# dnbaker/dashing

Measured on AMD Instinct MI355X. Metric: genome-pairs/sec, all-pairs HLL Jaccard (Ertl-MLE), N=10000 p=14, higher is better.
Workload: dtype u8/u32 popcount + f64 estimator; 1 GPU; BASELINE configs[2]: 10000 synthetic sketches, p=14 (16384 B each), all-pairs dist on MI355X; n_sketches=10000, p=14, k=31, estimator=ERTL_MLE

## Files before the change

### dashing_amd/csrc/abi.hip

```cpp
#include <algorithm>
#include <cstdlib>
#include <cstring>
#include <new>

#include "ctx.h"

using namespace dsh;

extern "C" {

const char *dsh_backend_name(void) { return "hip:gfx950"; }

int dsh_abi_version(void) { return DSH_ABI_VERSION; }

int dsh_device_count(void)
{
    int n = 0;
    if (hipGetDeviceCount(&n) != hipSuccess) return 0;
    return n;
}

static void release_ctx(dsh_ctx *c)
{
    (void)hipSetDevice(c->device);
// ... 787 lines not shown
{
    if (!c) return DSH_EINVAL;
    if (pair_ms) *pair_ms = c->pair_ms;
    if (fin_ms) *fin_ms = c->fin_ms;
    if (prep_ms) *prep_ms = c->prep_ms;
    if (launches) *launches = c->pair_launches;
    return DSH_OK;
}

int dsh_last_part_info(dsh_ctx *c, double *ready_ms, uint64_t *floats, uint32_t cap, uint32_t *nparts_out)
{
    if (!c || !nparts_out) return DSH_EINVAL;
    const uint32_t k = (uint32_t)c->part_ready_ms.size();
    *nparts_out = k;
    if (k > cap && (ready_ms || floats)) return DSH_EINVAL;
    for (uint32_t q = 0; q < k; ++q) {
        if (ready_ms) ready_ms[q] = c->part_ready_ms[q];
        if (floats) floats[q] = c->part_floats[q];
    }
    return DSH_OK;
}

int dsh_finalize_phase_cycles(dsh_ctx *c, uint64_t *out16)
{
    if (!c || !out16) return DSH_EINVAL;
    int rc = bind(c);
    if (rc) return rc;
    if (!c->phase_cyc.ptr) return fail(c, DSH_ESTATE, "no call with the option finalize_timing yet");
    HIPCHK(c, hipStreamSynchronize(c->stream));
    HIPCHK(c, hipMemcpy(out16, c->phase_cyc.ptr, 16 * sizeof(uint64_t), hipMemcpyDeviceToHost));
    return DSH_OK;
}

int dsh_get_info(dsh_ctx *c, const char *name, int64_t *out)
{
    if (!c || !name || !out) return DSH_EINVAL;
    if (!std::strcmp(name, "planes")) *out = c->lay.P;
    else if (!std::strcmp(name, "vlo")) *out = c->lay.vlo;
    else if (!std::strcmp(name, "vhi")) *out = c->lay.vhi;
    else if (!std::strcmp(name, "threshold")) *out = c->lay.pbase + (int64_t)c->lay.P;
    else if (!std::strcmp(name, "pbase")) *out = c->lay.pbase;
    else if (!std::strcmp(name, "host_layout_us")) *out = (int64_t)c->host_layout_us;
    else if (!std::strcmp(name, "host_lists_us")) *out = (int64_t)c->host_lists_us;
    else if (!std::strcmp(name, "host_keys_wait_us")) *out = (int64_t)c->host_keys_wait_us;
    else if (!std::strcmp(name, "emax")) *out = c->emax;
    else if (!std::strcmp(name, "elow")) *out = c->elow;
    else if (!std::strcmp(name, "kc")) *out = c->kc;
    else if (!std::strcmp(name, "pair_groups")) *out = c->pair_groups;
    else if (!std::strcmp(name, "pair_round")) *out = c->pp.band_round.empty() ? 0 : c->pp.band_round[0];
    else if (!std::strcmp(name, "tile")) *out = kTile;
    else if (!std::strcmp(name, "parts_done")) *out = c->parts_done;
    else if (!std::strcmp(name, "parts_signalled")) *out = c->parts_signalled ? 1 : 0;
    else if (!std::strcmp(name, "sketch_kernel_us")) *out = (int64_t)(c->sketch_ms * 1000.0);
    else if (!std::strcmp(name, "fastx_decode_us")) *out = (int64_t)(c->fastx_ms * 1000.0);
    else if (!std::strcmp(name, "xch_recv_gated")) *out = c->xch.recv_gated ? 1 : 0;
    else if (!std::strcmp(name, "stats_route")) *out = c->gs.route_last;
    else if (!std::strcmp(name, "linkage_route")) *out = c->lk.route_last;
    else if (!std::strcmp(name, "mst_rounds")) *out = c->mst.rounds_last;
    else if (!std::strcmp(name, "mst_band_us")) *out = (int64_t)(c->mst.band_ms * 1000.0);
    else if (!std::strcmp(name, "place_kernel_us")) *out = (int64_t)(c->xch.place_ms * 1000.0);
    else if (!std::strcmp(name, "whatif_mfma")) {
#ifdef DSH_WHATIF_MFMA
        *out = 1;
#else
        *out = 0;
#endif
    }
    else if (!std::strcmp(name, "npad")) *out = c->lay.Npad;
    else if (!std::strcmp(name, "kpad")) *out = c->Kpad;
    else if (!std::strcmp(name, "cum_bytes")) *out = c->cum_bytes;
    else if (!std::strcmp(name, "sorted")) *out = c->lay.sorted;
    else if (!std::strcmp(name, "ncols")) *out = (int64_t)c->lay.ncols;
    else if (!std::strcmp(name, "lockstep")) *out = c->planes_valid && use_lockstep(c) ? 1 : 0;
    else if (!std::strcmp(name, "tiles")) *out = (int64_t)c->pp.T.size();
    else if (!std::strcmp(name, "bands")) *out = (int64_t)c->last_bands;
    else if (!std::strcmp(name, "items")) *out = (int64_t)c->pp.items.size();
    else if (!std::strcmp(name, "frag_items")) {
        uint64_t f = 0;
        for (uint32_t x : c->pp.band_frags) f += x;
        *out = (int64_t)f;
    }
    else if (!std::strcmp(name, "sparse_items")) *out = (int64_t)c->pp.sp_items.size();
    else if (!std::strcmp(name, "sparse_plane_us")) *out = (int64_t)(c->sparse_ms * 1000.0);
    else if (!std::strcmp(name, "sparse_planes")) *out = c->sparse_planes;
    else if (!std::strcmp(name, "sparse_cap")) *out = c->sparse_cap;
    else if (!std::strcmp(name, "words_per_plane")) *out = c->W;
    else if (!std::strcmp(name, "avg_tile_planes_x100")) {
        uint64_t tot = 0;
        for (const auto &t : c->pp.T) tot += t.w - t.z;
        *out = c->pp.T.empty() ? 0 : (int64_t)(tot * 100 / c->pp.T.size());
    }
    else return fail(c, DSH_EINVAL, "unknown info %s", name);
    return DSH_OK;
}

int dsh_set_option(dsh_ctx *c, const char *name, int64_t v)
{
    if (!c || !name) return DSH_EINVAL;
    if (!std::strcmp(name, "kc")) {
        if (v != 0 && v != 16 && v != 32) return fail(c, DSH_EINVAL, "kc must be 0 (auto), 16 or 32");
        c->kc_opt = (int)v;
        c->planes_valid = false;
        return DSH_OK;
    }
    if (!std::strcmp(name, "pair_groups")) {
        if (v != 0 && v != 2 && v != 3) return fail(c, DSH_EINVAL, "pair_groups must be 0 (auto), 2 or 3");
        c->pair_groups_opt = (int)v;
        c->planes_valid = false;
        return DSH_OK;
    }
    if (!std::strcmp(name, "cum_budget_bytes")) {
        if (v < (1 << 20)) return fail(c, DSH_EINVAL, "cum_budget_bytes too small");
        c->cum_budget = (uint64_t)v;
        return DSH_OK;
    }
    if (!std::strcmp(name, "knn_square_budget_bytes")) {
        if (v < 0) return fail(c, DSH_EINVAL, "knn_square_budget_bytes must be >= 0");
        c->knn_square_budget = (uint64_t)v;
        return DSH_OK;
    }
    if (!std::strcmp(name, "threshold_band_bytes")) {
        if (v < 4) return fail(c, DSH_EINVAL, "threshold_band_bytes must be at least 4");
        c->threshold_band_bytes = (uint64_t)v;
        return DSH_OK;
    }
    if (!std::strcmp(name, "pairs_chunk")) {
        if (v < 1 || v > (1 << 24)) return fail(c, DSH_EINVAL, "pairs_chunk must be in [1, 2^24]");
        c->pairs.chunk = (uint64_t)v;
        return DSH_OK;
    }
    if (!std::strcmp(name, "cluster_chunk")) {
        if (v < 1 || v > (1 << 26)) return fail(c, DSH_EINVAL, "cluster_chunk must be in [1, 2^26]");
        c->cc.chunk = (uint64_t)v;
        return DSH_OK;
    }
    if (!std::strcmp(name, "stats_route")) {
        if (v < -1 || v > 1) return fail(c, DSH_EINVAL, "stats_route must be -1 (auto), 0 (dense) or 1 (pairs)");
        c->gs.route = (int)v;
        return DSH_OK;
    }
    if (!std::strcmp(name, "linkage_route")) {
        if (v < -1 || v > 1) return fail(c, DSH_EINVAL, "linkage_route must be -1 (auto), 0 (dense) or 1 (pairs)");
        c->lk.route = (int)v;
        return DSH_OK;
    }
    if (!std::strcmp(name, "linkage_partition")) {
        if (v < 0 || v > 1) return fail(c, DSH_EINVAL, "linkage_partition must be 0 or 1");
        c->lk.partition = (int)v;
        return DSH_OK;
    }
    if (!std::strcmp(name, "linkage_budget_bytes")) {
        if (v < 64) return fail(c, DSH_EINVAL, "linkage_budget_bytes must be at least 64");
        c->lk.budget = (uint64_t)v;
        return DSH_OK;
    }
    if (!std::strcmp(name, "linkage_lds_max")) {
        if (v < 0 || v > 6144) return fail(c, DSH_EINVAL, "linkage_lds_max must be in [0, 6144]");
        c->lk.lds_max = (uint32_t)v;
        return DSH_OK;
    }
    if (!std::strcmp(name, "greedy_band_rows")) {
        if (v < 1 || v > (long long)kGreedyMaxRows) return fail(c, DSH_EINVAL, "greedy_band_rows must be in [1, %u]", kGreedyMaxRows);
        c->gr.band_rows = (uint64_t)v;
        return DSH_OK;
    }
    if (!std::strcmp(name, "derive_chunk_bytes")) {
        if (v < 1) return fail(c, DSH_EINVAL, "derive_chunk_bytes must be at least 1");
        c->derive.chunk_bytes = (uint64_t)v;
        return DSH_OK;
    }
    if (!std::strcmp(name, "sort")) {
        if (v < -1 || v > 1) return fail(c, DSH_EINVAL, "sort must be -1, 0 or 1");
        c->sort_mode = (int)v;
        return DSH_OK;
    }
    if (!std::strcmp(name, "range_sort_min_rows")) {
        if (v < 1) return fail(c, DSH_EINVAL, "range_sort_min_rows must be >= 1");
        c->range_sort_min_rows = (int)std::min<int64_t>(v, 1 << 30);
        return DSH_OK;
    }
#ifdef DSH_WHATIF_MFMA
    if (!std::strcmp(name, "pair_mfma")) {
        c->pair_mfma = v != 0;
        return DSH_OK;
    }
#endif
    if (!std::strcmp(name, "finalize_stop")) {
        if (v < 0 || v > 4) return fail(c, DSH_EINVAL, "finalize_stop must be in [0,4]");
        if (v && !c->profiling) return fail(c, DSH_ESTATE, "finalize_stop needs dsh_set_profiling(ctx, 1)");
        c->finalize_stop = (int)v;
        return DSH_OK;
    }
    if (!std::strcmp(name, "finalize_timing")) {
        if (v && !c->profiling) return fail(c, DSH_ESTATE, "finalize_timing needs dsh_set_profiling(ctx, 1)");
        c->finalize_timing = v != 0;
        return DSH_OK;
    }
    if (!std::strcmp(name, "nsplit")) {
        if (v < 0 || v > 64) return fail(c, DSH_EINVAL, "nsplit must be in [0,64]");
        c->nsplit = (int)v;
        return DSH_OK;
    }
    if (!std::strcmp(name, "emax") || !std::strcmp(name, "elow")) {
        if (v < -1 || v > (int64_t)kMaxListSide) return fail(c, DSH_EINVAL, "%s must be in [-1,%u]", name, kMaxListSide);
        (name[1] == 'm' ? c->emax_opt : c->elow_opt) = (int)v;
        return DSH_OK;
    }
    if (!std::strcmp(name, "part_band_tiles")) {
        if (v < 1 || v > (1 << 30)) return fail(c, DSH_EINVAL, "part_band_tiles out of range");
        c->part_band_tiles = (int)v;
        return DSH_OK;
    }
    if (!std::strcmp(name, "xch_tail_bands")) {
        if (v < 0 || v > 8) return fail(c, DSH_EINVAL, "xch_tail_bands out of range");
        c->tail_bands = (int)v;
        return DSH_OK;
    }
    if (!std::strcmp(name, "overflow_frag_permille")) {
        if (v < 0 || v > 1000) return fail(c, DSH_EINVAL, "overflow_frag_permille out of range");
        c->overflow_frag_permille = (int)v;
        return DSH_OK;
    }
    if (!std::strcmp(name, "sparse_planes")) {
        if (v < -1 || v > 2) return fail(c, DSH_EINVAL, "sparse_planes is -1 (auto), 0 (off), 1 or 2");
        c->sparse_planes = (int)v;
        return DSH_OK;
    }
    if (!std::strcmp(name, "sparse_lds")) {
        if (v < 0 || v > 1) return fail(c, DSH_EINVAL, "sparse_lds must be 0 or 1");
        c->sparse_lds = (int)v;
        return DSH_OK;
    }
    if (!std::strcmp(name, "sparse_cap")) {
        if (v < 0 || v > (int64_t)plan::kSparseCapMax) return fail(c, DSH_EINVAL, "sparse_cap must be in [0, %u]", plan::kSparseCapMax);
        c->sparse_cap = (int)v;
        return DSH_OK;
    }
    if (!std::strcmp(name, "xch_recv_gate")) {
        if (v < -1 || v > 1) return fail(c, DSH_EINVAL, "xch_recv_gate is -1 (auto), 0 or 1");
        c->xch.recv_gate = (int)v;
        return DSH_OK;
    }
    if (!std::strcmp(name, "finalize_signal")) {
        if (v < -1 || v > 1) return fail(c, DSH_EINVAL, "finalize_signal is -1 (auto), 0 or 1");
        c->finalize_signal = (int)v;
        return DSH_OK;
    }
    return fail(c, DSH_EINVAL, "unknown option %s", name);
}

}
```

### dashing_amd/csrc/ctx.h

```cpp
#pragma once
#include <hip/hip_runtime.h>
#include <rccl/rccl.h>

#include <cstdarg>
#include <cstdio>
#include <cstdlib>
#include <deque>
#include <string>
#include <vector>

#include "../../include/dashing_hip.h"
#include "kernels.h"
#include "plan.h"

struct NoCopy {
    NoCopy() = default;
    NoCopy(const NoCopy &) = delete;
    NoCopy &operator=(const NoCopy &) = delete;
};

struct DevBuf : NoCopy {
    void *ptr = nullptr;
    size_t cap = 0;
    ~DevBuf() { release(); }
// ... 65 lines not shown
        if (hipDeviceGetStreamPriorityRange(&least, &greatest) != hipSuccess) greatest = 0;
        if (const char *e = std::getenv("DSH_COPY_STREAM_PRIORITY")) greatest = std::atoi(e);
        return hipStreamCreateWithPriority(&st, hipStreamNonBlocking, greatest);
    }
    operator hipStream_t() const { return st; }
};

struct Staging : NoCopy {
    PinBuf buf;
    Event sent_ev;
    bool in_flight = false;
    hipError_t wait()
    {
        if (!in_flight) return hipSuccess;
        const hipError_t e = hipEventSynchronize(sent_ev);
        if (e == hipSuccess) in_flight = false;
        return e;
    }
    hipError_t room(size_t bytes)
    {
        const hipError_t e = wait();
        return e == hipSuccess ? buf.ensure(bytes) : e;
    }
    hipError_t sent(hipStream_t st)
    {
        hipError_t e = sent_ev.ensure();
        if (e == hipSuccess) e = hipEventRecord(sent_ev, st);
        if (e == hipSuccess) in_flight = true;
        return e;
    }
    void *ptr() const { return buf.ptr; }
};

struct dsh_ctx {
    int device = 0;
    Stream stream;
    Stream copy_stream;
    Stream aux_stream;
    Stream place_stream;
    Stream spin_stream;
    std::string err;
    DevBuf regs_own;
    const uint8_t *regs = nullptr;
    uint64_t n = 0;
    int p = 0;
    bool have_sketches = false;
    bool planes_valid = false;
    int card_estim = -1;
    uint64_t card_from = 0;
    uint64_t pass_gen = 0, lay_gen = 0;
    DevBuf card, planes, cum, tiles, items, outbuf, exc, excv, exc_n, keys, perm, tailhist;
    Event ev_aux_fork, ev_aux_join;
    bool aux_join_pending = false;
    DevBuf outbuf2[2];
    Event ev_filled[2];
    Event ev_drained[2];
    bool drained_pending[2] = {false, false};
    unsigned out_turn = 0;
    std::deque<Event> tickets;
    uint64_t ticket_next = 0;
    Event ev_first_tiles;
    bool pass_from_zero = false;
    DevBuf hist;
    Event ev_keys;
    DevBuf cidx_rec, cidx_ent;
    uint32_t nbuckets = 0, ent_stride = 0;
    DevBuf colS_n, colS_key, colS_card, colS_th, colS_rl;
    uint32_t rl_stride = 0;
    dsh::plan::Layout lay;
    bool lay_built = false;
    dsh::plan::PairPlan pp;
    std::deque<Event> ev_part;
    uint32_t parts_done = 0;
    DevBuf sig;
    Staging st_sig;
    uint32_t sig_gen = 0;
    bool parts_signalled = false;
    int finalize_signal = -1;
    int can_wait_value = -1;
    int wall_clock_khz = 0;
    PinBuf pin_keys;
    const uint32_t *hk32 = nullptr;
    const uint32_t *hg32 = nullptr;
    bool hk32_valid = false;
    double host_layout_us = 0, host_lists_us = 0, host_keys_wait_us = 0;
    Staging st_perm;
    DevBuf rowoff;
    Staging st_lists;
    uint32_t W = 0, Kpad = 0;
    int emax = 0, elow = 0, cum_bytes = 4;
    int kc = 16;
    int kc_opt = 0;
    int pair_groups = 3;
    int pair_groups_opt = 0;
    int emax_opt = -1;
    int elow_opt = -1;
    int part_band_tiles = 2048;
    int overflow_frag_permille = 500;
    int sparse_planes = -1;
    int sparse_cap = (int)dsh::plan::kSparseCapDefault;
    int sparse_lds = 1;
    DevBuf sp_tab, sp_lists, sp_len, sp_slabs, sp_items;
    Staging st_sparse;
    std::vector<dsh::plan::U2> sp_have;
    uint64_t sp_serial = 0, lay_serial = 0;
    uint32_t sp_cap_have = 0;
    double sparse_ms = 0;
    std::vector<std::pair<hipEvent_t, hipEvent_t>> ev_sparse;
    int tail_bands = 2;
    std::vector<double> part_ready_ms;
    std::vector<uint64_t> part_floats;
    size_t last_bands = 0;
    uint64_t cum_budget = 8ull << 30;
    int sort_mode = -1;
    int range_sort_min_rows = 1024;
    DevBuf thr_vals;
    uint64_t threshold_band_bytes = (uint64_t)1 << 30;
    uint64_t knn_square_budget = (uint64_t)96 << 30;
    int pair_mfma = 0;
    int finalize_stop = 0;
    int finalize_timing = 0;
    DevBuf phase_cyc;
    int nsplit = 0;
    bool profiling = false;
    double pair_ms = 0, fin_ms = 0, prep_ms = 0, sketch_ms = 0, fastx_ms = 0;
    uint32_t pair_launches = 0;
    std::deque<Event> ev_pool;
    size_t ev_used = 0;

    struct {
        DevBuf seqbuf, workbuf, recbuf;
        Staging work, rec;
        DevBuf rawbuf, fx_tab, fx_summ, fx_state, fx_declen, fx_status;
        Staging fx;
    } sketch;
    struct {
        DevBuf cnt, off, total, col, val, rowptr;
    } thr;
    struct {
        DevBuf card, hist, lhs, rhs, out, err;
        Staging list;
        int card_estim = -1;
        uint64_t chunk = 1u << 18;
    } pairs;
    struct {
        DevBuf parent, state, lhs, rhs, rowptr, seed, labels;
        uint64_t chunk = 1u << 20;
    } cc;
    struct {
        DevBuf assign, state, labels;
        DevBuf best;
        uint64_t band_rows = 4096;
    } gr;
    struct {
        DevBuf labels, acc, grp, out, csr;
        int route = -1;
        int route_last = -1;
    } gs;
    struct {
        DevBuf edges, labels, counts;
        int cus = 0;
    } hs;
    struct {
        DevBuf tab, cells, nodes, labels, state;
        uint64_t budget = 8ull << 30;
        uint32_t lds_max = 4096;
        int partition = 1;
        int route = -1;
        int route_last = -1;
    } lk;
    struct {
        DevBuf best, ckey, cedge, elhs, erhs, ekey, state;
        int rounds_last = 0;
        double band_ms = 0;
    } mst;
    struct {
        DevBuf degree, best, kind, state;
    } db;
    struct {
        DevBuf err, stage, ptr, mem, dst, part[2], out;
        uint64_t chunk_bytes = (uint64_t)256 << 20;
    } derive;
    struct {
// ... 194 lines not shown
```

### dashing_amd/csrc/engine.hip

```cpp
#include <algorithm>
#include <chrono>
#include <cstring>

#include "ctx.h"

namespace dsh {

int prepare(dsh_ctx *c, int estim, int want_sorted, bool card_only, uint64_t want_rb, uint64_t want_re, uint32_t nparts,
            int rowsorted, const std::vector<uint64_t> *extra_in)
{
    static const std::vector<uint64_t> kNoExtra;
    std::vector<uint64_t> extra_cached;
    const std::vector<uint64_t> *extra = extra_in ? extra_in : &kNoExtra;
    if (!c->have_sketches) return fail(c, DSH_ESTATE, "no sketches loaded");
    if (estim < 0 || estim > 2) return fail(c, DSH_EINVAL, "bad estimator %d", estim);
    if (want_sorted < 0) {
        want_sorted = c->lay.sorted;
        want_rb = c->lay.rb;
        want_re = c->lay.re;
        rowsorted = 0;
        extra_cached = c->lay.extra;
        extra = &extra_cached;
    }
    if (!want_sorted) rowsorted = 0, extra = &kNoExtra;
    if (want_re > c->n) want_re = c->n;
    if (!want_sorted) want_rb = 0, want_re = c->n;
    if (want_rb > want_re) want_rb = want_re;
    const uint64_t n = c->n;
    std::vector<uint64_t> parts, rs_pos;
    if (want_rb >= want_re) extra = &kNoExtra;
    if (want_sorted && !rowsorted) {
        if (extra->empty()) plan::range_parts(n, want_rb, want_re, std::max<uint32_t>(nparts, 1), parts);
        else parts = {want_rb, want_re};
    }
    if (rowsorted) plan::rowsorted_part_positions(n, want_rb, want_re, std::max<uint32_t>(nparts, 1), rs_pos, extra);
    const int emax_new = c->emax_opt >= 0 ? std::min<int>(c->emax_opt, (int)kMaxListSide) : plan::auto_list_cap(c->p, true);
    const int elow_new = c->elow_opt >= 0 ? std::min<int>(c->elow_opt, (int)kMaxListSide) : plan::auto_list_cap(c->p, false);
    if (emax_new != c->emax || elow_new != c->elow) {
        c->planes_valid = false;
        c->card_estim = -1;
    }
    c->emax = emax_new;
    c->elow = elow_new;
    const bool same_layout = c->planes_valid && c->lay_gen == c->pass_gen && c->lay.sorted == want_sorted &&
                             (!want_sorted || (c->lay.rb == want_rb && c->lay.re == want_re && c->lay.rowsorted == rowsorted &&
                                               c->lay.extra == *extra && (rowsorted ? c->lay.part_w == rs_pos : c->lay.parts == parts)));
    const uint64_t need_from = (card_only || !want_sorted || c->pass_from_zero) ? 0 : want_rb;
    const bool have_pass = c->card_estim == estim && c->card_from <= need_from;
    if (have_pass && (card_only || same_layout)) return DSH_OK;
    const bool keep_layout = same_layout && have_pass;
    DeviceTimer timer(c, c->stream);
    if (!have_pass) {
        HIPCHK(c, c->card.ensure(std::max<uint64_t>(n, 1) * sizeof(double)));
        HIPCHK(c, c->exc.ensure(std::max<uint64_t>(n, 1) * kListCap * (c->p <= 15 ? 2 : 4)));
        HIPCHK(c, c->excv.ensure(std::max<uint64_t>(n, 1) * kListCap));
        HIPCHK(c, c->exc_n.ensure(std::max<uint64_t>(n, 1) * sizeof(uint32_t)));
        HIPCHK(c, c->keys.ensure(std::max<uint64_t>(n, 1) * 2 * sizeof(uint32_t)));
        HIPCHK(c, c->tailhist.ensure(std::max<uint64_t>(n, 1) * 64));
        HIPCHK(c, c->hist.ensure(std::max<uint64_t>(n, 1) * 64 * sizeof(uint32_t)));
        HIPCHK(c, launch_selfhist_card(c->stream, c->regs, need_from, n, c->p, estim, c->emax, c->elow,
                                       (uint32_t *)c->hist.ptr, c->exc.ptr, (uint8_t *)c->excv.ptr,
                                       (uint32_t *)c->exc_n.ptr, (uint32_t *)c->keys.ptr,
                                       (uint8_t *)c->tailhist.ptr, (uint32_t *)c->keys.ptr + n));
        HIPCHK(c, c->pin_keys.ensure(std::max<uint64_t>(n, 1) * 2 * sizeof(uint32_t)));
        c->hk32 = (const uint32_t *)c->pin_keys.ptr;
        c->hg32 = c->hk32 + n;
        if (n > need_from)
            HIPCHK(c, hipMemcpyAsync((uint32_t *)c->pin_keys.ptr + need_from, (const uint32_t *)c->keys.ptr + need_from,
                                     (2 * n - need_from) * sizeof(uint32_t), hipMemcpyDeviceToHost, c->stream));
        HIPCHK(c, c->ev_keys.ensure());
        HIPCHK(c, hipEventRecord(c->ev_keys, c->stream));
        HIPCHK(c, launch_card_from_hist(c->stream, (const uint32_t *)c->hist.ptr, (const uint32_t *)c->keys.ptr, need_from, n,
                                        c->p, estim, (double *)c->card.ptr));
        c->card_estim = estim;
        c->card_from = need_from;
        c->hk32_valid = false;
        ++c->pass_gen;
    }
    if (card_only) {
        timer.stop(c->prep_ms, true);
        return DSH_OK;
    }
#ifdef DSH_EXPERIMENT_REUSE_LAYOUT
    const bool reuse_host_layout = !keep_layout && c->lay_built && c->lay.n == n && c->lay.sorted == want_sorted &&
                                   (!want_sorted || (c->lay.rb == want_rb && c->lay.re == want_re && c->lay.rowsorted == rowsorted &&
                                                     c->lay.extra == *extra && (rowsorted ? c->lay.part_w == rs_pos : c->lay.parts == parts)));
#else
    constexpr bool reuse_host_layout = false;
#endif
    if (!keep_layout) {
        if (c->p > kMaxPCompare)
            return fail(c, DSH_EINVAL, "the compare path takes p <= %d (p=%d: sketching and cardinalities only)", kMaxPCompare, c->p);
        if (c->pair_groups_opt == 3 && c->kc_opt == 32)
            return fail(c, DSH_EINVAL, "pair_groups = 3 needs kc = 16 (or kc = 0, auto)");
        const auto t_h0 = std::chrono::steady_clock::now();
        if (!c->hk32_valid && !reuse_host_layout) {
            HIPCHK(c, hipEventSynchronize(c->ev_keys));
            c->hk32_valid = true;
        }
        const auto t_h1 = std::chrono::steady_clock::now();
        c->host_keys_wait_us = std::chrono::duration<double, std::micro>(t_h1 - t_h0).count();
        const uint32_t *k32 = c->hk32;
        for (uint64_t i = c->card_from; i < n && !reuse_host_layout; ++i)
            if (plan::key_bad(k32[i]))
                return fail(c, DSH_EINVAL, "sketch %llu holds a register value above %d (= 64 - p + 1): not an HLL of precision %d (corrupt or foreign .hll?)",
                            (unsigned long long)i, 64 - c->p + 1, c->p);
        c->planes_valid = false;
        plan::Layout &L = c->lay;
        if (!reuse_host_layout)
            plan::build_layout(k32, n, want_sorted, want_rb, want_re, parts, L, rowsorted ? std::max<uint32_t>(nparts, 1) : 0,
                               extra->empty() ? nullptr : extra, c->hg32);
        ++c->lay_serial;
        c->lay_built = true;
        c->cum_bytes = c->p <= 15 ? 2 : 4;
        const uint64_t m = 1ull << c->p;
        c->W = (uint32_t)std::max<uint64_t>(1, m / 32);
        c->pair_groups = c->pair_groups_opt ? c->pair_groups_opt : (c->kc_opt == 32 ? 2 : 3);
        c->kc = c->pair_groups == 3 ? 16 : c->kc_opt ? c->kc_opt : (c->W >= 32 ? 32 : 16);
        if (want_sorted && !reuse_host_layout) {
            const uint64_t nperm = L.perm.size();
            HIPCHK(c, c->perm.ensure(std::max<uint64_t>(nperm, 1) * sizeof(uint32_t)));
            if (nperm) {
                const size_t pb_ = (nperm * sizeof(uint32_t) + 15) & ~(size_t)15;
                const size_t rb_ = L.rowsorted ? L.rowoff.size() * sizeof(uint64_t) : 0;
                HIPCHK(c, c->st_perm.room(pb_ + rb_));
                uint8_t *h = (uint8_t *)c->st_perm.ptr();
                std::memcpy(h, L.perm.data(), nperm * sizeof(uint32_t));
                HIPCHK(c, launch_upload(c->stream, c->perm.ptr, h, nperm * sizeof(uint32_t)));
                if (L.rowsorted) {
                    HIPCHK(c, c->rowoff.ensure(rb_));
                    std::memcpy(h + pb_, L.rowoff.data(), rb_);
                    HIPCHK(c, launch_upload(c->stream, c->rowoff.ptr, h + pb_, rb_));
                }
                HIPCHK(c, c->st_perm.sent(c->stream));
            }
        }
        const uint32_t NT = L.Npad / kTile;
        c->nbuckets = (uint32_t)std::min<uint64_t>(2 * m, kMaxBuckets);
        c->ent_stride = std::max<uint32_t>(1, kTile * (uint32_t)(c->emax + c->elow));
        c->rl_stride = std::max<uint32_t>(1, (uint32_t)(c->emax + c->elow));
        const size_t nbk = std::max<size_t>(NT, 1);
        HIPCHK(c, c->cidx_rec.ensure(nbk * c->nbuckets * (size_t)(colindex_inline(c->p, c->rl_stride) + 1) * sizeof(uint32_t)));
        HIPCHK(c, c->cidx_ent.ensure(nbk * c->ent_stride * sizeof(uint32_t)));
        HIPCHK(c, c->colS_n.ensure(nbk * kTile * sizeof(uint32_t)));
        HIPCHK(c, c->colS_key.ensure(nbk * kTile * sizeof(uint32_t)));
        HIPCHK(c, c->colS_card.ensure(nbk * kTile * sizeof(double)));
        HIPCHK(c, c->colS_th.ensure(nbk * kTile * 64));
        HIPCHK(c, c->colS_rl.ensure(nbk * kTile * (size_t)c->rl_stride * sizeof(uint32_t)));
        c->host_layout_us = std::chrono::duration<double, std::micro>(std::chrono::steady_clock::now() - t_h1).count();
        HIPCHK(c, hipEventRecord(c->ev_aux_fork, c->stream));
        HIPCHK(c, hipStreamWaitEvent(c->aux_stream, c->ev_aux_fork, 0));
        {
            ColIndexLaunch ci;
            ci.exc = c->exc.ptr;
            ci.excv = (const uint8_t *)c->excv.ptr;
            ci.exc_n = (const uint32_t *)c->exc_n.ptr;
            ci.keys = (const uint32_t *)c->keys.ptr;
            ci.card = (const double *)c->card.ptr;
            ci.tailhist = (const uint8_t *)c->tailhist.ptr;
            ci.perm = want_sorted ? (const uint32_t *)c->perm.ptr : nullptr;
            ci.ncols = L.ncols;
            ci.p = c->p;
            ci.nblocks = NT;
            ci.nbuckets = c->nbuckets;
            ci.ent_stride = c->ent_stride;
            ci.E = c->rl_stride;
            ci.rec = (uint32_t *)c->cidx_rec.ptr;
            ci.ent = (uint32_t *)c->cidx_ent.ptr;
            ci.nS = (uint32_t *)c->colS_n.ptr;
            ci.keyS = (uint32_t *)c->colS_key.ptr;
            ci.cardS = (double *)c->colS_card.ptr;
            ci.thS = (uint8_t *)c->colS_th.ptr;
            ci.rl = (uint32_t *)c->colS_rl.ptr;
            HIPCHK(c, launch_build_colindex(c->aux_stream, ci));
        }
        HIPCHK(c, hipEventRecord(c->ev_aux_join, c->aux_stream));
        const uint64_t K = (uint64_t)L.P * c->W;
        c->Kpad = (uint32_t)((K + c->kc - 1) / c->kc * c->kc);
        if (c->Kpad) {
            const size_t bytes = (size_t)c->Kpad * L.Npad * sizeof(uint32_t);
            HIPCHK(c, c->planes.ensure(bytes));
            if (c->Kpad > K)
                HIPCHK(c, hipMemsetAsync((uint32_t *)c->planes.ptr + K * L.Npad, 0,
                                         (size_t)(c->Kpad - K) * L.Npad * sizeof(uint32_t),
                                         c->stream));
            HIPCHK(c, launch_transform(c->stream, c->regs, L.ncols, c->p, L.pbase, L.P, c->W, L.Npad,
                                       (uint32_t *)c->planes.ptr,
                                       want_sorted ? (const uint32_t *)c->perm.ptr : nullptr));
        }
        c->aux_join_pending = true;
        c->lay_gen = c->pass_gen;
        c->planes_valid = true;
    }
    timer.stop(c->prep_ms, true);
    return DSH_OK;
}

namespace {

struct JobLayout {
    int want_sorted = 0;
    uint64_t lrb = 0, lre = 0;
    bool with_parts = false;
    bool with_extra = false;
};

struct PairRun {
    plan::Tuning tu;
    std::vector<uint64_t> item_off;
    plan::U4 *pinT = nullptr, *pinF = nullptr, *pinI = nullptr;
    bool signal = false;
    bool sig_upload = false;
    FinalizeLaunch fin{};
    hipEvent_t e_call0 = nullptr;
    std::vector<std::pair<size_t, hipEvent_t>> ev_part_t;
    std::vector<std::pair<hipEvent_t, hipEvent_t>> evp, evf;
};

JobLayout choose_layout(const dsh_ctx *c, const PairJob &job)
{
    JobLayout jl;
    const uint64_t jre = std::min<uint64_t>(job.row_end, c->n);
    const bool full_tri = !job.rect && job.row_begin == 0 && jre >= c->n;
    jl.with_parts = job.nparts > 0 && !job.rect && !job.sorted_rows;
    jl.lre = c->n;
    if (job.sorted_rows) jl.want_sorted = 1;
    else if (!job.rect && jre > job.row_begin &&
             (jl.with_parts || (c->sort_mode != 0 && (full_tri || jre - job.row_begin >= (uint64_t)c->range_sort_min_rows)))) {
        jl.want_sorted = 1;
        jl.lrb = job.row_begin;
        jl.lre = jre;
    }
    jl.with_extra = jl.want_sorted && jl.with_parts && !job.extra.empty() && jl.lre > jl.lrb;
    return jl;
}

constexpr uint64_t kSparseSlabBudget = 2ull << 30;
uint32_t sparse_list_stride(const dsh_ctx *c)
{
    return std::max<uint32_t>(8, (std::min<uint32_t>((uint32_t)c->sparse_cap, plan::kSparseCapMax) + 7) / 8 * 8);
}
int sparse_wordmajor(const dsh_ctx *c) { return c->sparse_lds && c->p <= 15 ? 1 : 0; }
uint64_t sparse_slab_bytes(const dsh_ctx *c)
{
    return ((uint64_t)16 << c->p) + (uint64_t)kTile * sparse_list_stride(c) * sizeof(uint16_t) + kTile * sizeof(uint32_t);
}

plan::Tuning tuning_of(const dsh_ctx *c)
{
    plan::Tuning tu;
    tu.W = c->W;
    tu.kc = c->kc;
    tu.cum_bytes = c->cum_bytes;
    tu.cum_budget = c->cum_budget;
    tu.nsplit = c->nsplit;
    tu.lockstep = use_lockstep(c);
    tu.round_items = 256u * (uint32_t)c->pair_groups;
    tu.small_round_items = c->pair_groups_opt == 0 && c->pair_groups == 3 ? 512u : 0u;
    tu.part_band_tiles = (uint32_t)c->part_band_tiles;
    tu.overflow_frag_max_permille = (uint32_t)c->overflow_frag_permille;
    tu.tail_bands = (uint32_t)c->tail_bands;
    tu.p = c->p;
    tu.sparse_planes = c->sparse_planes;
    tu.sparse_cap = (uint32_t)c->sparse_cap;
    tu.sparse_max_slabs = (uint32_t)std::min<uint64_t>(1u << 16, kSparseSlabBudget / sparse_slab_bytes(c));
    return tu;
}

int reserve_lists(dsh_ctx *c, PairRun &r)
{
    plan::PairPlan &pp = c->pp;
    const std::vector<plan::U4> &T = pp.T;
    r.item_off.assign(pp.bands.size() + 1, 0);
    for (size_t bi = 0; bi < pp.bands.size(); ++bi) r.item_off[bi + 1] = r.item_off[bi] + plan::band_item_count(r.tu, pp, bi);
    const uint64_t nitems_total = r.item_off.back();
    pp.items.reserve(nitems_total);
    static_assert(sizeof(plan::U4) == sizeof(uint4), "plan::U4 must have the layout of uint4");
    HIPCHK(c, c->st_lists.room((2 * T.size() + std::max<uint64_t>(nitems_total, 1)) * sizeof(uint4)));
    r.pinT = (plan::U4 *)c->st_lists.ptr(), r.pinF = r.pinT + T.size(), r.pinI = r.pinF + T.size();
    HIPCHK(c, c->tiles.ensure(2 * T.size() * sizeof(uint4)));
    HIPCHK(c, c->items.ensure(std::max<uint64_t>(nitems_total, 1) * sizeof(uint4)));
    HIPCHK(c, c->cum.ensure(std::max<uint64_t>(pp.per_tile_bytes * pp.max_band, 256)));
    return DSH_OK;
}

int stage_signal_block(dsh_ctx *c, PairRun &r)
{
    ++c->sig_gen;
    if (c->sig_gen == 0) c->sig_gen = 1;
    HIPCHK(c, c->st_sig.room((2 * kSigMaxParts + 2) * sizeof(uint32_t)));
    static_assert(kSigPartTotal == kSigPartCnt + kSigMaxParts && kSigGen == kSigPartTotal + kSigMaxParts && kSigStamp == kSigGen + 1, "signal block layout");
    uint32_t *blk = (uint32_t *)c->st_sig.ptr(), *tot = blk + kSigMaxParts;
    for (uint32_t qd = 0; qd < kSigMaxParts; ++qd) blk[qd] = 0u;
    for (uint32_t qd = 0; qd < kSigMaxParts; ++qd) tot[qd] = qd < c->pp.part_tiles.size() ? c->pp.part_tiles[qd] : 0u;
    tot[kSigMaxParts] = c->sig_gen;
    tot[kSigMaxParts + 1] = c->profiling ? 1u : 0u;
    r.sig_upload = true;
    return DSH_OK;
}

FinalizeLaunch finalize_invariants(const dsh_ctx *c, const PairJob &job, bool with_extra)
{
    const plan::Layout &L = c->lay;
    FinalizeLaunch f{};
    f.cum_bytes = c->cum_bytes;
    FinalizeArgs &a = f.a;
    a.cum = c->cum.ptr;
    a.perm = L.sorted ? (const uint32_t *)c->perm.ptr : nullptr;
    a.rowoff = L.rowsorted ? (const uint64_t *)c->rowoff.ptr : nullptr;
    a.pbase = L.pbase;
    a.p = c->p;
    a.estim = job.estim;
    a.result_type = job.result_type;
    a.ksinv = job.ksinv_double ? 1. / (double)job.k : (double)(float)(1. / (double)job.k);
    a.nS = (const uint32_t *)c->colS_n.ptr;
    a.keyS = (const uint32_t *)c->colS_key.ptr;
    a.cardS = (const double *)c->colS_card.ptr;
    a.thS = (const uint8_t *)c->colS_th.ptr;
    a.rl = (const uint32_t *)c->colS_rl.ptr;
    a.E = c->rl_stride;
    a.cidx_rec = (const uint32_t *)c->cidx_rec.ptr;
    a.cidx_ent = (const uint32_t *)c->cidx_ent.ptr;
    a.nbuckets = c->nbuckets;
    a.ent_stride = c->ent_stride;
    a.n = c->n;
    a.ncols = L.ncols;
    a.rect = job.rect;
    a.sorted_out = job.sorted_rows;
    a.square = job.square;
    a.knn = job.knn;
    a.out2 = job.d_out2;
    a.knn_ld = job.knn_ld;
    a.knn_rows = job.knn_rows;
    a.stop = c->finalize_stop;
    a.phase_cyc = c->finalize_timing ? (unsigned long long *)c->phase_cyc.ptr : nullptr;
    a.row_begin = job.row_begin;
    a.row_end = with_extra ? c->n : job.row_end;
    a.col_begin = job.col_begin;
    a.col_end = job.col_end;
    a.base_index = job.base_index;
    a.out = job.d_out;
    return f;
}

int upload_band(dsh_ctx *c, PairRun &r, size_t bi)
{
    plan::PairPlan &pp = c->pp;
// ... 282 lines not shown
```

### dashing_amd/csrc/host/plan_capi.cpp

```cpp
#include <algorithm>
#include <cstdarg>
#include <cstdio>
#include <cstring>
#include <vector>

#include "../linkage.h"
#include "../mst.h"
#include "../plan.h"
#include "../uf.h"

using namespace dsh;
using namespace dsh::plan;

namespace {

struct SparseCheck {
    const uint32_t *gcnt = nullptr;
    int planes = 0;
    uint32_t cap = 0;
    uint32_t *routes = nullptr;
    uint64_t routes_cap = 0;
};

struct Err {
    char *buf;
    size_t cap;
    int fail(const char *fmt, ...)
    {
        if (buf && cap) {
            va_list ap;
            va_start(ap, fmt);
            vsnprintf(buf, cap, fmt, ap);
            va_end(ap);
        }
        return -1;
    }
};

}

static int plan_check(uint64_t n, const uint32_t *keys, int mode, int want_sorted, uint64_t rb, uint64_t re, uint64_t cb,
                      uint64_t ce, uint32_t nparts, int want_parts, int p, uint64_t cum_budget, int lockstep, int nsplit,
                      int ls_item_chunks, const std::vector<uint64_t> &extra, uint64_t *stats, char *err, size_t cap,
                      uint32_t round_items = 0, const SparseCheck *sc = nullptr)
{
    Err E{err, cap};
    if (re > n) re = n;
    const bool rowsorted = mode == 3;
    if (rowsorted) mode = 0, want_sorted = 1, want_parts = 1;
    if (mode == 1 || !want_sorted) want_sorted = mode == 2 ? 1 : 0;
    if (mode == 2) want_sorted = 1;
    std::vector<uint64_t> parts;
    uint64_t lrb = 0, lre = n;
    if (want_sorted && mode == 0) lrb = rb, lre = re;
    if (want_sorted && !rowsorted) range_parts(n, lrb, lre, std::max<uint32_t>(want_parts ? nparts : 1, 1), parts);
    if (!extra.empty() && !(want_sorted && mode == 0)) return E.fail("extra segments need a sorted triangle layout");
    Layout L;
    build_layout(keys, n, want_sorted, lrb, lre, parts, L, rowsorted ? std::max<uint32_t>(nparts, 1) : 0, extra.empty() ? nullptr : &extra,
                 sc ? sc->gcnt : nullptr);
    std::vector<std::pair<uint64_t, uint64_t>> wsegs;
    wanted_order(n, lrb, lre, &extra, wsegs, rowsorted);
    auto in_rows = [&](uint64_t i) {
        for (auto &w : wsegs)
            if (i >= w.first && i < w.second) return true;
        return false;
    };
    uint64_t nw = 0, wspan = 0;
    for (auto &w : wsegs) nw += w.second - w.first, wspan += tri_span(n, w.first, w.second);
    if (want_sorted && mode == 0 && L.nwanted != nw) return E.fail("nwanted %llu != %llu", (unsigned long long)L.nwanted, (unsigned long long)nw);
    if (rowsorted) {
        auto skey = [&](uint32_t g) { return ((uint32_t)key_T(keys[g]) << 12) | ((uint32_t)key_L(keys[g]) << 6) | (uint32_t)key_hi(keys[g]); };
        for (auto &w : wsegs)
            for (uint64_t s = w.first - lrb + 1; s < w.second - lrb; ++s)
                if (skey(L.perm[s - 1]) > skey(L.perm[s])) return E.fail("row-sorted: a wanted segment is not one key-ordered run at %llu", (unsigned long long)s);
        if (L.part_w.empty() || L.part_w.front() != 0 || L.part_w.back() != nw) return E.fail("row-sorted: part cuts do not span the wanted rows");
        for (size_t q = 1; q + 1 < L.part_w.size(); ++q) {
            if (L.part_w[q] <= L.part_w[q - 1]) return E.fail("row-sorted: cut %zu at %llu", q, (unsigned long long)L.part_w[q]);
            uint64_t w0 = 0;
            bool ok = false;
            for (auto &w : wsegs) {
                if (L.part_w[q] >= w0 && L.part_w[q] < w0 + (w.second - w.first)) ok = (L.part_w[q] - w0) % kTile == 0;
                w0 += w.second - w.first;
            }
            if (!ok) return E.fail("row-sorted: cut %zu at %llu is not at a tile row of the wanted order", q, (unsigned long long)L.part_w[q]);
        }
        if (L.part_w.size() - 1 > std::max<uint32_t>(nparts, 1)) return E.fail("row-sorted: more parts than asked for");
        uint64_t acc = 0, w_ = 0;
        if (L.rowoff_w.size() != nw + 1) return E.fail("row-sorted: rowoff_w size");
        for (auto &w : wsegs)
            for (uint64_t s = w.first - lrb; s < w.second - lrb; ++s, ++w_) {
                if (s >= L.rowoff.size() || L.rowoff[s] != acc || L.rowoff_w[w_] != acc) return E.fail("row-sorted: rowoff[%llu]", (unsigned long long)s);
                acc += n - 1 - L.perm[s];
            }
        if (L.rowoff_w.back() != acc || acc != wspan) return E.fail("row-sorted: the rows do not add up to the span");
    }
    const uint64_t col0 = want_sorted ? lrb : 0;
    if (L.ncols != n - col0) return E.fail("ncols %llu != %llu", (unsigned long long)L.ncols, (unsigned long long)(n - col0));
    if (L.Npad % kTile || L.Npad < L.ncols || L.Npad >= L.ncols + kTile) return E.fail("bad Npad %u", L.Npad);
    std::vector<uint8_t> seen(n, 0);
    for (uint64_t s = 0; s < L.ncols; ++s) {
        const uint32_t g = L.perm[s];
        if (g < col0 || g >= n || seen[g]) return E.fail("perm[%llu] = %u is out of range or repeated", (unsigned long long)s, g);
        seen[g] = 1;
    }
    if (want_sorted) {
        uint64_t s = 0;
        for (size_t q = 0; q + 1 < L.parts.size(); ++q)
            for (uint64_t r = L.parts[q]; r < L.parts[q + 1]; ++r, ++s)
                if (L.perm[s] < L.parts[q] || L.perm[s] >= L.parts[q + 1])
                    return E.fail("column %llu holds sketch %u, not a row of part %zu", (unsigned long long)s, L.perm[s], q);
        if (!rowsorted && extra.empty()) {
            if (L.part_pos.size() != L.parts.size()) return E.fail("part positions and parts differ in number");
            for (size_t q = 0; q < L.parts.size(); ++q)
                if (L.part_pos[q] != L.parts[q] - lrb) return E.fail("part position %zu", q);
        }
        for (; s < L.ncols; ++s)
            if (L.perm[s] < lre) return E.fail("column %llu (after the wanted rows) holds wanted row %u", (unsigned long long)s, L.perm[s]);
        for (auto &w : wsegs)
            for (uint64_t s2 = w.first - lrb; s2 < w.second - lrb; ++s2)
                if (L.perm[s2] < w.first || L.perm[s2] >= w.second) return E.fail("position %llu of a wanted segment holds row %u", (unsigned long long)s2, L.perm[s2]);
        if (!extra.empty())
            for (uint64_t s2 = 0; s2 < L.ncols; ++s2) {
                const uint64_t b = s2 / kTile * kTile;
                if (in_rows(L.perm[s2]) != in_rows(L.perm[b])) return E.fail("block %llu mixes wanted and other rows", (unsigned long long)(b / kTile));
            }
        if (L.whole)
            for (uint64_t i = 0; i < n; ++i)
                if (L.perm[n + L.perm[i]] != i) return E.fail("inverse permutation wrong at %llu", (unsigned long long)i);
    }
    Tuning tu;
    const uint64_t m = 1ull << p;
    tu.W = (uint32_t)std::max<uint64_t>(1, m / 32);
    tu.kc = tu.W >= 32 ? 32 : 16;
    tu.cum_bytes = p <= 15 ? 2 : 4;
    tu.cum_budget = cum_budget;
    tu.nsplit = nsplit;
    tu.lockstep = lockstep && tu.W >= (uint32_t)tu.kc;
    tu.ls_item_chunks = ls_item_chunks;
    if (round_items) tu.round_items = round_items;
    if (round_items > 512) tu.small_round_items = 512;
    tu.p = p;
    if (sc) tu.sparse_planes = sc->planes, tu.sparse_cap = sc->cap;
    PairQuery q;
    q.rect = mode == 1;
    q.sorted_rows = mode == 2;
    q.want_parts = want_parts && mode == 0 && want_sorted;
    q.row_begin = rb;
    q.row_end = re;
    q.col_begin = cb;
    q.col_end = ce;
    PairPlan pp;
    const bool any = build_pairs(L, q, tu, pp);
    for (int i = 0; i < 9; ++i) stats[i] = 0;
    stats[5] = L.Npad;
    stats[6] = L.P;
    std::vector<uint8_t> hit;
    uint64_t wanted = 0;
    auto orig = [&](uint64_t s) -> uint64_t { return L.perm[s]; };
    if (mode == 1) {
        const uint64_t nr = re > rb ? re - rb : 0, nc = ce > cb ? ce - cb : 0;
        wanted = nr * nc;
        hit.assign(wanted, 0);
    } else {
        hit.assign(n * n, 0);
        for (uint64_t i = rb; i < re; ++i) wanted += n - 1 - i;
        for (size_t x = 0; x + 1 < extra.size(); x += 2)
            for (uint64_t i = extra[x]; i < extra[x + 1]; ++i) wanted += n - 1 - i;
        if (mode == 2) {
            wanted = 0;
            for (uint64_t si = rb; si < re; ++si) wanted += n - 1 - si;
        }
    }
    if (!any) {
        if (wanted) return E.fail("nothing planned although %llu pairs are wanted", (unsigned long long)wanted);
        return 0;
    }
    const std::vector<U4> &T = pp.T;
    uint64_t got = 0, planes_sum = 0;
    for (const U4 &t : T) {
        if (t.z > t.w || t.w > L.P) return E.fail("tile (%u,%u) has the plane range [%u,%u) of %u", t.x, t.y, t.z, t.w, L.P);
        planes_sum += t.w - t.z;
        for (uint32_t a = 0; a < kTile; ++a)
            for (uint32_t b = 0; b < kTile; ++b) {
                const uint64_t si = (uint64_t)t.x * kTile + a, sj = (uint64_t)t.y * kTile + b;
                if (si >= L.ncols || sj >= L.ncols) continue;
                const uint64_t i = orig(si), j = orig(sj);
                bool active;
                uint64_t slot;
                if (mode == 1) {
                    active = i >= rb && i < re && j >= cb && j < ce;
                    slot = active ? (i - rb) * (ce - cb) + (j - cb) : 0;
                } else if (mode == 2) {
                    active = si < sj && si >= rb && si < re;
                    slot = si * n + sj;
                } else {
                    const uint64_t oi = std::min(i, j), oj = std::max(i, j);
                    active = si < sj && oi >= rb && oi < (extra.empty() ? re : n);
                    slot = oi * n + oj;
                    if (active && !extra.empty() && !in_rows(oi))
                        return E.fail("tile (%u,%u) computes the pair (%llu,%llu) of a row this rank does not hold", t.x, t.y, (unsigned long long)oi, (unsigned long long)oj);
                }
                if (!active) continue;
                if (hit[slot]++) return E.fail("pair slot %llu computed twice (tile %u,%u)", (unsigned long long)slot, t.x, t.y);
                ++got;
                const uint32_t ka = keys[i], kb = keys[j];
                const int Tp = L.pbase + (int)t.w, Lp = L.pbase + (int)t.z;
                if (Tp < std::max(key_T(ka), key_T(kb))) return E.fail("tile (%u,%u): T %d below a sketch's threshold", t.x, t.y, Tp);
                if (Lp > std::max(std::max(key_lo(ka), key_lo(kb)), std::min(key_L(ka), key_L(kb))))
                    return E.fail("tile (%u,%u): Lp %d above what the low lists cover", t.x, t.y, Lp);
            }
    }
    if (got != wanted) return E.fail("%llu of %llu wanted pairs are covered", (unsigned long long)got, (unsigned long long)wanted);
    size_t at = 0;
    if (pp.bands.size() != pp.segs.size() || pp.bands.size() != pp.band_items.size()) return E.fail("band bookkeeping sizes differ");
    std::vector<int> part_done(pp.nparts, 0);
    int last_part = -1;
    for (size_t bi = 0; bi < pp.bands.size(); ++bi) {
        const auto &bd = pp.bands[bi];
        if (bd.first != at || bd.second <= bd.first || bd.second > T.size()) return E.fail("band %zu = [%zu,%zu) does not follow %zu", bi, bd.first, bd.second, at);
        at = bd.second;
        if (bd.second - bd.first > 1 && (bd.second - bd.first) * pp.per_tile_bytes > cum_budget)
            return E.fail("band %zu needs %llu bytes of C(v), budget %llu", bi, (unsigned long long)((bd.second - bd.first) * pp.per_tile_bytes), (unsigned long long)cum_budget);
        size_t sa = bd.first;
        for (const Seg &sg : pp.segs[bi]) {
            if (sg.b != sa || sg.e <= sg.b || sg.e > bd.second) return E.fail("segment [%zu,%zu) of band %zu does not follow %zu", sg.b, sg.e, bi, sa);
            sa = sg.e;
            if (sg.part >= 0) {
                if ((uint32_t)sg.part >= pp.nparts || part_done[sg.part]++ || sg.part != last_part + 1)
                    return E.fail("part %d completed out of order or twice", sg.part);
                last_part = sg.part;
            }
            if (q.want_parts)
                for (size_t t = sg.b; t < sg.e; ++t) {
                    uint64_t pos0 = ~0ull;
                    for (size_t k = 0; k < L.wtr.size(); ++k)
                        if (T[t].x >= L.wtr[k].first && T[t].x < L.wtr[k].second) pos0 = L.wtr_w[k] + (uint64_t)(T[t].x - L.wtr[k].first) * kTile;
                    const int cur = last_part + (sg.part >= 0 ? 0 : 1);
                    if (cur < 0 || (size_t)cur + 1 >= L.part_w.size() || pos0 < L.part_w[cur] || pos0 >= L.part_w[cur + 1])
                        return E.fail("tile row %u is not in part %d", T[t].x, cur);
                }
        }
        if (sa != bd.second) return E.fail("segments of band %zu end at %zu, not %zu", bi, sa, bd.second);
        const auto &bi_ = pp.band_items[bi];
        if (band_item_count(tu, pp, bi) != bi_.second - bi_.first) return E.fail("band %zu: band_item_count disagrees with the items built", bi);
        std::vector<uint32_t> next(bd.second - bd.first);
        for (size_t t = bd.first; t < bd.second; ++t) next[t - bd.first] = pp.chunks[t].x;
        std::vector<std::vector<std::pair<uint32_t, uint32_t>>> per(bd.second - bd.first);
        const uint32_t cpp_ = tu.W >= (uint32_t)tu.kc ? tu.W / tu.kc : 1;
        const uint32_t nfr = bi < pp.band_frags.size() ? pp.band_frags[bi] : 0u;
        const uint32_t bri = bi < pp.band_round.size() ? pp.band_round[bi] : 0u;
        if (bri != tu.round_items && !(tu.small_round_items && bri == tu.small_round_items)) return E.fail("band %zu: round of %u items", bi, bri);
        if (bi == 0 && round_items) stats[9] = bri;
        if (nfr > bi_.second - bi_.first || nfr > bri) return E.fail("band %zu: %u fragments", bi, nfr);
        if (nfr && (!tu.lockstep || (bi_.second - bi_.first - nfr) % bri)) return E.fail("band %zu: fragments behind %zu whole items", bi, bi_.second - bi_.first - nfr);
        stats[8] += nfr;
        for (size_t it = bi_.first; it < bi_.second; ++it) {
            const U4 &I = pp.items[it];
            if (I.x >= per.size() || I.y >= I.z) return E.fail("item %zu is malformed", it);
            const bool frag = it >= bi_.second - nfr;
            if ((I.w != 0) != frag) return E.fail("item %zu: fragment flag %u at the wrong place", it, I.w);
            if (frag && (I.y / cpp_ != (I.z - 1) / cpp_ || I.z - I.y != pp.items[bi_.second - 1].z - pp.items[bi_.second - 1].y))
                return E.fail("fragment %zu spans two planes or differs in length", it);
            per[I.x].emplace_back(I.y, I.z | (frag ? 0x80000000u : 0u));
        }
        for (size_t t = 0; t < per.size(); ++t) {
            std::sort(per[t].begin(), per[t].end());
            uint32_t x = pp.chunks[bd.first + t].x;
            for (size_t k = 0; k < per[t].size(); ++k) {
                auto &pr = per[t][k];
                const bool frag = (pr.second & 0x80000000u) != 0;
                pr.second &= 0x7FFFFFFFu;
                if (pr.first != x) return E.fail("items of tile %zu leave a gap or overlap at chunk %u", t, x);
                if (!frag && tu.W >= (uint32_t)tu.kc && ((pr.first % cpp_) || (pr.second % cpp_))) return E.fail("an item of tile %zu is not whole planes", t);
                if (frag && (pr.first % cpp_) && !(k > 0 && (per[t][k - 1].second & 0x7FFFFFFFu) == pr.first))
                    return E.fail("a fragment of tile %zu starts inside a plane that fragments do not cover from its start", t);
                x = pr.second;
            }
            if (x != pp.chunks[bd.first + t].y) return E.fail("items of tile %zu end at chunk %u, not %u", t, x, pp.chunks[bd.first + t].y);
        }
    }
    if (at != T.size()) return E.fail("bands end at %zu of %zu tiles", at, T.size());
    if (pp.sp.size() != T.size() || pp.band_sp_items.size() != pp.bands.size()) return E.fail("sparse bookkeeping sizes differ");
    {
        const uint32_t cpp_ = tu.W >= (uint32_t)tu.kc ? tu.W / tu.kc : 1;
        std::vector<uint8_t> seen_pl;
        size_t sat = 0;
        for (size_t bi = 0; bi < pp.bands.size(); ++bi) {
            const auto &bd = pp.bands[bi];
            const auto &rg = pp.band_sp_items[bi];
            if (rg.first != sat || rg.second < rg.first || rg.second > pp.sp_items.size()) return E.fail("sparse items of band %zu do not follow %zu", bi, sat);
            sat = rg.second;
            seen_pl.assign((bd.second - bd.first) * 2, 0);
            for (size_t k = rg.first; k < rg.second; ++k) {
                const U4 &I = pp.sp_items[k];
                if (I.x >= bd.second - bd.first) return E.fail("sparse item %zu names tile %u of band %zu", k, I.x, bi);
                const size_t t = bd.first + I.x;
                const uint32_t sp = pp.sp[t];
                if (I.y >= T[t].w || I.y + sp < T[t].w) return E.fail("sparse item %zu: plane %u is not one of the top %u of tile %zu", k, I.y, sp, t);
                if (seen_pl[I.x * 2 + (T[t].w - 1 - I.y)]++) return E.fail("plane %u of tile %zu has two sparse items", I.y, t);
                if (I.z >= pp.slabs.size() || I.w >= pp.slabs.size() || pp.slabs[I.z].x != T[t].x || pp.slabs[I.z].y != I.y ||
                    pp.slabs[I.w].x != T[t].y || pp.slabs[I.w].y != I.y)
                    return E.fail("sparse item %zu names the wrong slabs", k);
                const int v = L.pbase + 1 + (int)I.y;
                if (sparse_bound(L, T[t].x, v) > tu.sparse_cap || sparse_bound(L, T[t].y, v) > tu.sparse_cap) return E.fail("sparse item %zu: a set may exceed the cap", k);
                if (sc && sc->gcnt)
                    for (int side = 0; side < 2; ++side)
                        for (uint32_t a = 0; a < kTile; ++a) {
                            const uint64_t sx = (uint64_t)(side ? T[t].y : T[t].x) * kTile + a;
                            if (sx >= L.ncols) continue;
                            const uint32_t key = keys[orig(sx)], g = sc->gcnt[orig(sx)];
                            const uint32_t own = v >= key_T(key) ? (g & 0xFFFFu) : v == key_T(key) - 1 ? g >> 16 : 65535u;
                            if (own > tu.sparse_cap) return E.fail("sparse item %zu: sketch %llu may hold %u positions", k, (unsigned long long)orig(sx), own);
                        }
            }
            for (size_t t = bd.first; t < bd.second; ++t) {
                const uint32_t sp = pp.sp[t];
                if (sp > 2 || sp > T[t].w - T[t].z) return E.fail("tile %zu routes %u planes of %u", t, sp, T[t].w - T[t].z);
                for (uint32_t x = 0; x < sp; ++x)
                    if (!seen_pl[(t - bd.first) * 2 + x]) return E.fail("routed plane %u of tile %zu has no sparse item", T[t].w - 1 - x, t);
                if (tu.W >= (uint32_t)tu.kc && (pp.chunks[t].x != T[t].z * cpp_ || pp.chunks[t].y != (T[t].w - sp) * cpp_))
                    return E.fail("tile %zu: the dense chunk range is not the planes left over", t);
            }
        }
        if (sat != pp.sp_items.size()) return E.fail("sparse items end at %zu of %zu", sat, pp.sp_items.size());
        if (sc && sc->routes) {
            if (T.size() > sc->routes_cap) return E.fail("%zu tiles, room for %llu routes", T.size(), (unsigned long long)sc->routes_cap);
            for (size_t t = 0; t < T.size(); ++t) {
                uint32_t *o = sc->routes + 5 * t;
                o[0] = T[t].x, o[1] = T[t].y, o[2] = T[t].z, o[3] = T[t].w, o[4] = pp.sp[t];
            }
        }
    }
    for (uint32_t qd = 0; qd < pp.nparts; ++qd)
        if (part_done[qd] != 1) return E.fail("part %u never completes", qd);
    if (pp.nparts) {
        uint64_t tsum = 0;
        if (pp.part_tiles.size() != pp.nparts) return E.fail("part_tiles has %zu entries for %u parts", pp.part_tiles.size(), pp.nparts);
        for (uint32_t c : pp.part_tiles) tsum += c;
        if (tsum != T.size()) return E.fail("the parts hold %llu tiles of %zu", (unsigned long long)tsum, T.size());
    }
    if (q.want_parts && pp.nparts + 1 != L.part_w.size()) return E.fail("%u parts planned, layout has %zu", pp.nparts, L.part_w.size() - 1);
    std::vector<U4> dt(T.size()), df(T.size());
    emit_tile_lists(L, pp, dt.data(), df.data());
    for (size_t bi = 0; bi < pp.bands.size(); ++bi)
        for (const Seg &sg : pp.segs[bi]) {
            std::vector<uint8_t> used(pp.bands[bi].second - pp.bands[bi].first, 0);
            for (size_t t = sg.b; t < sg.e; ++t) {
                const U4 &f = df[t];
                const uint32_t fw = f.w & 0xFFFFu, fpart = f.w >> 16;
                const size_t src = pp.bands[bi].first + fw;
                if (fw >= used.size() || src < sg.b || src >= sg.e || used[fw]++) return E.fail("finalize list names a C(v) block twice or outside its segment");
                if (pp.nparts) {
                    if (fpart >= pp.nparts || src < pp.part_first[fpart] || src >= pp.part_first[fpart + 1])
                        return E.fail("finalize list entry %zu carries part %u, which does not hold tile %zu", t, fpart, src);
                } else if (fpart) {
                    return E.fail("finalize list entry %zu carries a part without parts", t);
                }
                if (f.x != T[src].x || f.y != T[src].y || (f.z & 0xFFu) != T[src].z || ((f.z >> 8) & 0xFFu) != T[src].w)
                    return E.fail("finalize list entry %zu does not match tile %zu", t, src);
                if (dt[src].x != T[src].x || dt[src].y != T[src].y || dt[src].z != (T[src].z | (T[src].w << 8)))
                    return E.fail("tile list entry %zu is wrong", src);
                const int lo = (int)((f.z >> 16) & 0xFFu), hi = (int)(f.z >> 24);
                if (hi - lo + 1 > sg.hist_bins) return E.fail("segment hist_bins %d too small for tile %zu", sg.hist_bins, src);
            }
            {
                std::vector<uint32_t> rows_seen;
                for (size_t t = sg.b + 1; t < sg.e; ++t) {
                    if (df[t - 1].x == df[t].x) {
                        if (df[t - 1].y >= df[t].y) return E.fail("finalize list of a segment is not row-major at %zu", t);
                    } else {
                        rows_seen.push_back(df[t - 1].x);
                        if (std::find(rows_seen.begin(), rows_seen.end(), df[t].x) != rows_seen.end())
                            return E.fail("finalize list of a segment returns to tile row %u at %zu", df[t].x, t);
                    }
                }
            }
        }
    stats[0] = T.size();
    stats[1] = pp.bands.size();
    stats[2] = pp.items.size();
    stats[3] = pp.nparts;
    stats[4] = T.empty() ? 0 : planes_sum * 100 / T.size();
    if (sc) stats[10] = pp.sp_items.size(), stats[11] = pp.slabs.size();
    stats[7] = 0;
    for (size_t b = 0; b < pp.band_items.size(); ++b) {
        const uint32_t nfr = b < pp.band_frags.size() ? pp.band_frags[b] : 0u;
        const uint32_t bri = pp.band_round[b];
        stats[7] += (pp.band_items[b].second - pp.band_items[b].first - nfr + bri - 1) / bri + (nfr ? 1 : 0);
    }
    return 0;
}

extern "C" {

int dshh_plan_check(uint64_t n, const uint32_t *keys, int mode, int want_sorted, uint64_t rb, uint64_t re, uint64_t cb,
                    uint64_t ce, uint32_t nparts, int want_parts, int p, uint64_t cum_budget, int lockstep, int nsplit,
                    int ls_item_chunks, uint64_t *stats, char *err, size_t cap)
{
    return plan_check(n, keys, mode, want_sorted, rb, re, cb, ce, nparts, want_parts, p, cum_budget, lockstep, nsplit, ls_item_chunks,
                      std::vector<uint64_t>(), stats, err, cap);
}

int dshh_plan_check_ri(uint64_t n, const uint32_t *keys, int mode, int want_sorted, uint64_t rb, uint64_t re, uint64_t cb,
                       uint64_t ce, uint32_t nparts, int want_parts, int p, uint64_t cum_budget, int lockstep, int nsplit,
                       int ls_item_chunks, uint32_t round_items, uint64_t *stats, char *err, size_t cap)
{
    Err E{err, cap};
    if (round_items == 0 || round_items % 256) return E.fail("round_items %u is not a positive multiple of 256", round_items);
    return plan_check(n, keys, mode, want_sorted, rb, re, cb, ce, nparts, want_parts, p, cum_budget, lockstep, nsplit, ls_item_chunks,
                      std::vector<uint64_t>(), stats, err, cap, round_items);
}

int dshh_plan_check_sparse(uint64_t n, const uint32_t *keys, const uint32_t *gcnt, int mode, int want_sorted, uint64_t rb, uint64_t re,
                           uint32_t nparts, int want_parts, int p, uint64_t cum_budget, uint32_t round_items, int sparse_planes,
                           uint32_t sparse_cap, uint64_t *stats, uint32_t *routes, uint64_t routes_cap, char *err, size_t cap)
{
    Err E{err, cap};
    if (round_items == 0 || round_items % 256) return E.fail("round_items %u is not a positive multiple of 256", round_items);
    SparseCheck sc;
    sc.gcnt = gcnt;
    sc.planes = sparse_planes;
    sc.cap = sparse_cap;
    sc.routes = routes;
    sc.routes_cap = routes_cap;
    stats[10] = stats[11] = 0;
    return plan_check(n, keys, mode, want_sorted, rb, re, 0, 0, nparts, want_parts, p, cum_budget, 1, 0, 64, std::vector<uint64_t>(), stats, err,
                      cap, round_items, &sc);
}

int dshh_plan_check_rowset(uint64_t n, const uint32_t *keys, const uint64_t *tab, uint32_t rank, int rowsorted, uint32_t nparts, int p,
                           uint64_t cum_budget, uint64_t *stats, char *err, size_t cap)
{
    Err E{err, cap};
    RowSets rs;
    if (const char *why = parse_rowsets(tab, n, rs)) return E.fail("%s", why);
    if (rank >= rs.world) return E.fail("rank %u of %u", rank, rs.world);
    uint64_t rb, re;
    std::vector<uint64_t> extra;
    rs.rank_rows(rank, rb, re, extra);
    for (int i = 0; i < 9; ++i) stats[i] = 0;
    if (rb >= re) return 0;
    return plan_check(n, keys, rowsorted ? 3 : 0, 1, rb, re, 0, 0, rowsorted ? nparts : 1, 1, p, cum_budget, 1, 0, 64, extra, stats, err, cap);
}

uint64_t dshh_rowsorted_split(uint64_t n, uint64_t rb, uint64_t re) { return rowsorted_split(n, rb, re); }

int64_t dshh_threshold_bands(uint64_t n, uint64_t rb, uint64_t re, uint64_t ncols, uint64_t band_bytes, uint64_t row_cap,
                             uint64_t *bounds, uint64_t cap)
{
    const uint64_t band_floats = std::max<uint64_t>(band_bytes / sizeof(float), 1);
    if (!ncols && re > n) re = n;
    uint64_t nb = 0;
    if (cap) bounds[0] = rb;
    for (uint64_t b0 = rb; b0 < re;) {
        b0 = ncols ? std::min<uint64_t>(re, b0 + rect_band_rows(ncols, band_floats)) : tri_band_end(n, b0, re, band_floats, row_cap);
        if (++nb >= cap) return -1;
        bounds[nb] = b0;
    }
    return (int64_t)nb;
}

uint64_t dshh_hist_grid(uint64_t units, uint64_t lds_bytes, uint32_t cus, uint64_t *iters)
{
    const uint64_t grid = hist_grid(units, lds_bytes, cus);
    if (iters) *iters = units / (4 * grid) + (units % (4 * grid) ? 1 : 0);
    return grid;
}

int64_t dshh_greedy_bands(uint64_t n, uint64_t band_bytes, uint64_t row_cap, uint64_t *bounds, uint64_t cap)
{
    const uint64_t band_floats = std::max<uint64_t>(band_bytes / sizeof(float), 1);
    uint64_t nb = 0;
    if (cap) bounds[0] = 0;
    for (uint64_t b0 = 0; b0 + 1 < n;) {
        b0 = tri_band_end(n, b0, n, band_floats, row_cap);
        if (++nb >= cap) return -1;
        bounds[nb] = b0;
    }
    return (int64_t)nb;
}

int64_t dshh_greedy_extend_bands(const uint32_t *labels_in, uint64_t m, uint64_t n, uint64_t band_bytes, uint64_t *bounds, uint64_t cap)
{
    if (m > n) return -1;
    const uint64_t band_floats = std::max<uint64_t>(band_bytes / sizeof(float), 1);
    uint64_t nb = 0, b0 = 0, b1 = 0;
    for (uint64_t from = 0; greedy_old_band(labels_in, m, n - m, from, band_floats, b0, b1); from = b1) {
        if (2 * nb + 2 > cap) return -1;
        bounds[2 * nb] = b0;
        bounds[2 * nb + 1] = b1;
        ++nb;
    }
    return (int64_t)nb;
}

int dsh_plan_uf_labels(uint64_t n, const uint32_t *lhs, const uint32_t *rhs, uint64_t n_edges, uint32_t step_cap, uint32_t *labels_out)
{
    if (n > 0xFFFFFFFFull) return -1;
    std::vector<uint32_t> parent(n);
    for (uint64_t x = 0; x < n; ++x) parent[x] = (uint32_t)x;
    for (uint64_t e = 0; e < n_edges; ++e) {
        if (lhs[e] >= n || rhs[e] >= n) return -1;
        uint32_t why = 0;
        if (uf_unite<UfPlain>(parent.data(), lhs[e], rhs[e], step_cap, &why) == kUfOverrun) return (int)why;
    }
    for (uint64_t x = 0; x < n; ++x) {
        const uint32_t l = uf_find<UfPlain>(parent.data(), (uint32_t)x, step_cap);
        if (l == kUfOverrun) return (int)kUfErrFind;
        labels_out[x] = l;
    }
    return 0;
}
// ... 66 lines not shown
```

### dashing_amd/csrc/kernels.h

```cpp
#pragma once
#include <hip/hip_runtime.h>
#include <stdint.h>

#include "consts.h"

namespace dsh {

hipError_t launch_selfhist_card(hipStream_t st, const uint8_t *regs, uint64_t first, uint64_t n, int p, int estim,
                                int emax, int elow, uint32_t *hist, void *exc, uint8_t *excv, uint32_t *exc_n,
                                uint32_t *keys, uint8_t *tailhist, uint32_t *gcnt);
hipError_t launch_card_from_hist(hipStream_t st, const uint32_t *hist, const uint32_t *keys, uint64_t first, uint64_t n, int p,
                                 int estim, double *card);
inline int colindex_inline(int p, uint32_t E) { return p <= 12 && E <= 256 ? 7 : 3; }
struct ColIndexLaunch {
    const void *exc;
    const uint8_t *excv;
    const uint32_t *exc_n, *keys;
    const double *card;
    const uint8_t *tailhist;
    const uint32_t *perm;
    uint64_t ncols;
    int p;
    uint32_t nblocks, nbuckets, ent_stride, E;
    uint32_t *rec;
    uint32_t *ent;
    uint32_t *nS, *keyS;
    double *cardS;
    uint8_t *thS;
    uint32_t *rl;
};
hipError_t launch_build_colindex(hipStream_t st, const ColIndexLaunch &c);
hipError_t launch_transform(hipStream_t st, const uint8_t *regs, uint64_t n, int p, int vlo,
                            uint32_t P, uint32_t W, uint32_t Npad, uint32_t *planes,
                            const uint32_t *perm);
hipError_t launch_pair_counts(hipStream_t st, int kc, int cum_bytes, const uint32_t *planes,
                              uint32_t Npad, uint32_t Kpad, uint32_t W, uint32_t P,
                              const uint4 *tiles, const uint4 *items, uint32_t nitems, void *cum,
                              uint64_t nslots);

hipError_t launch_sparse_build(hipStream_t st, const uint32_t *planes, uint32_t Npad, uint32_t W, uint64_t ncols, const uint2 *slabs,
                               uint32_t nslabs, uint32_t cap, int wordmajor, uint32_t *tab, uint16_t *lists, uint32_t *len);
hipError_t launch_sparse_count(hipStream_t st, int cum_bytes, const uint4 *items, uint32_t nitems, int wordmajor, const uint32_t *tab,
                               const uint16_t *lists, const uint32_t *len, uint32_t cap, uint32_t m, void *cum, uint64_t nslots);

hipError_t launch_pair_counts_lockstep(hipStream_t st, int kc, int groups, int cum_bytes, const uint32_t *planes,
                                       uint32_t Npad, uint32_t Kpad, uint32_t W, uint32_t P, const uint4 *tiles,
                                       const uint4 *items, uint32_t nitems, uint32_t nfrag, void *cum, uint64_t nslots);
hipError_t launch_pair_counts_mfma(hipStream_t st, int kc, int cum_bytes, const uint32_t *planes,
                                   uint32_t Npad, uint32_t Kpad, uint32_t W, uint32_t P,
                                   const uint4 *tiles, const uint4 *items, uint32_t nitems, void *cum,
                                   uint64_t nslots);

struct FinalizeArgs {
    const void *cum;
    uint64_t nslots;
    const uint4 *tiles;
    const uint32_t *perm;
    const uint64_t *rowoff;
    int hist_bins;
    int pbase;
    int p;
    int estim;
    int result_type;
    double ksinv;
    const uint32_t *nS;
    const uint32_t *keyS;
    const double *cardS;
    const uint8_t *thS;
    const uint32_t *rl;
    uint32_t E;
    const uint32_t *cidx_rec;
    const uint32_t *cidx_ent;
    uint32_t nbuckets, ent_stride;
    uint64_t n;
    uint64_t ncols;
    int rect;
    int sorted_out;
    int square;
    int knn;
    float *out2;
    uint64_t knn_ld, knn_rows;
    int stop;
    uint32_t ntiles;
    unsigned long long *phase_cyc;
    uint64_t row_begin, row_end, col_begin, col_end;
    uint64_t base_index;
    float *out;
    uint32_t *sig;
};
static_assert(sizeof(FinalizeArgs) == 272, "the kernel argument of k_finalize changed its layout");
struct FinalizeLaunch {
    FinalizeArgs a;
    int cum_bytes;
// ... 213 lines not shown
```

### dashing_amd/csrc/kernels_compare.hip

```cpp
#include <hip/hip_runtime.h>
#include <stdint.h>

#include <algorithm>

#include "estimators.h"
#include "kernels.h"

namespace dsh {

template <typename PT>
__global__ __launch_bounds__(256, 4) void k_selfhist_card(const uint8_t *__restrict__ regs, uint64_t first,
                                                        uint64_t n, int p, int estim, int emax, int elow,
                                                        uint32_t *__restrict__ hist_out,
                                                        PT *__restrict__ exc,
                                                        uint8_t *__restrict__ excv,
                                                        uint32_t *__restrict__ exc_n,
                                                        uint32_t *__restrict__ keys,
                                                        uint8_t *__restrict__ tailhist,
                                                        uint32_t *__restrict__ gcnt)
{
    __shared__ uint32_t hist[4][64];
    __shared__ uint32_t sub[4][8][72];
    __shared__ int thr[4], thrL[4];
    const int tid = threadIdx.x, lane = tid & 63, wave = tid >> 6;
    const uint64_t s = first + (uint64_t)blockIdx.x * 4 + wave;
#pragma unroll
    for (int k = 0; k < 8; ++k) sub[wave][k][lane] = 0;
    __syncthreads();
    const uint64_t m = 1ull << p;
    const uint4 *src = reinterpret_cast<const uint4 *>(regs + (s < n ? s : 0) * m);
    const uint64_t nch = m >> 4;
    constexpr int kRegCache = 16;
    uint4 cache[kRegCache];
#pragma unroll
    for (int k = 0; k < kRegCache; ++k) {
        const uint64_t c = (uint64_t)k * 64 + lane;
        cache[k] = src[c < nch ? c : nch - 1];
    }
#pragma unroll
    for (int k = 0; k < kRegCache; ++k)
        if (!(s < n && (uint64_t)k * 64 + lane < nch)) cache[k] = make_uint4(0, 0, 0, 0);
    uint32_t bad = 0;
    const uint32_t limrep = (uint32_t)(64 - p + 2) * 0x01010101u;
    if (s < n) {
        uint32_t *mysub = sub[wave][lane & 7];
        auto count16 = [mysub, limrep, &bad](const uint4 x) {
            const uint32_t w[4] = {x.x, x.y, x.z, x.w};
#pragma unroll
            for (int k = 0; k < 4; ++k) {
                bad |= (w[k] | (((w[k] & 0x7F7F7F7Fu) | 0x80808080u) - limrep)) & 0x80808080u;
                atomicAdd(&mysub[w[k] & 63], 1u);
                atomicAdd(&mysub[(w[k] >> 8) & 63], 1u);
                atomicAdd(&mysub[(w[k] >> 16) & 63], 1u);
                atomicAdd(&mysub[(w[k] >> 24) & 63], 1u);
            }
        };
#pragma unroll
        for (int k = 0; k < kRegCache; ++k)
            if ((uint64_t)k * 64 + lane < nch) count16(cache[k]);
        for (uint64_t c = (uint64_t)kRegCache * 64 + lane; c < nch; c += 64) count16(src[c]);
    }
    __syncthreads();
    {
        uint32_t t = 0;
#pragma unroll
        for (int k = 0; k < 8; ++k) t += sub[wave][k][lane];
        hist[wave][lane] = t;
    }
    __syncthreads();
    if (s < n && lane == 0) {
        const uint32_t *h = hist[wave];
        int lo = 0, hi = 63;
        while (lo < 63 && h[lo] == 0) ++lo;
        while (hi > 0 && h[hi] == 0) --hi;
        int T = hi;
        uint32_t cnt = 0;
        while (T > lo && cnt + h[T] <= (uint32_t)emax) {
            cnt += h[T];
            --T;
        }
        int L = lo;
        uint32_t cntl = 0;
        while (L < T && cntl + h[L] <= (uint32_t)elow) {
            cntl += h[L];
            ++L;
        }
        thr[wave] = T;
        thrL[wave] = L;
        exc_n[s] = cnt + cntl;
        keys[s] = ((uint32_t)hi << 18) | ((uint32_t)T << 12) | ((uint32_t)L << 6) | (uint32_t)lo;
        const uint32_t g0 = cnt + h[T], g1 = g0 + (T > 0 ? h[T - 1] : 0u);
        gcnt[s] = (g0 < 65535u ? g0 : 65535u) | ((g1 < 65535u ? g1 : 65535u) << 16);
    }
    if (s < n && __any(bad != 0) && lane == 0) atomicOr(&keys[s], 0x80000000u);
    __syncthreads();
    if (s >= n) return;
    const uint32_t T = (uint32_t)thr[wave], L = (uint32_t)thrL[wave];
    tailhist[s * 64 + lane] = (uint32_t)lane > T ? (uint8_t)hist[wave][lane] : (uint8_t)0;
    hist_out[s * 64 + lane] = hist[wave][lane];
    if (emax == 0 && elow == 0) return;
    PT *dstp = exc + s * kListCap;
    uint8_t *dstv = excv + s * kListCap;
    const uint32_t trep = (T + 1) * 0x01010101u, lrep = L * 0x01010101u;
    auto hits = [trep, lrep](uint32_t x) -> uint32_t {
        const uint32_t ge = ((x | 0x80808080u) - trep) & 0x80808080u;
        const uint32_t lt = ~((x | 0x80808080u) - lrep) & 0x80808080u;
        return ge | lt;
    };
    uint32_t mine = 0;
#pragma unroll
    for (int k = 0; k < kRegCache; ++k)
        if ((uint64_t)k * 64 + lane < nch) {
            const uint32_t w[4] = {cache[k].x, cache[k].y, cache[k].z, cache[k].w};
#pragma unroll
            for (int q = 0; q < 4; ++q) mine += (uint32_t)__popc(hits(w[q]));
        }
    for (uint64_t c = (uint64_t)kRegCache * 64 + lane; c < nch; c += 64) {
        const uint4 x = src[c];
        mine += (uint32_t)(__popc(hits(x.x)) + __popc(hits(x.y)) + __popc(hits(x.z)) + __popc(hits(x.w)));
    }
    uint32_t slot = mine;
#pragma unroll
    for (int d = 1; d < 64; d <<= 1) {
        const uint32_t o = __shfl_up(slot, d, 64);
        if (lane >= d) slot += o;
    }
    slot -= mine;
    auto emit4 = [&](uint32_t x, uint32_t pos0) {
        uint32_t h = hits(x);
        while (h) {
            const uint32_t b = (uint32_t)__builtin_ctz(h) >> 3;
            h &= h - 1;
            if (slot < kListCap) {
                dstp[slot] = (PT)(pos0 + b);
                dstv[slot] = (uint8_t)((x >> (8 * b)) & 0xFFu);
            }
            ++slot;
        }
    };
#pragma unroll
    for (int k = 0; k < kRegCache; ++k) {
        const uint64_t c = (uint64_t)k * 64 + lane;
        if (c < nch) {
            const uint32_t w[4] = {cache[k].x, cache[k].y, cache[k].z, cache[k].w};
#pragma unroll
            for (int q = 0; q < 4; ++q) emit4(w[q], (uint32_t)(c * 16 + q * 4));
        }
    }
    for (uint64_t c = (uint64_t)kRegCache * 64 + lane; c < nch; c += 64) {
        const uint4 x = src[c];
        emit4(x.x, (uint32_t)(c * 16));
        emit4(x.y, (uint32_t)(c * 16 + 4));
        emit4(x.z, (uint32_t)(c * 16 + 8));
        emit4(x.w, (uint32_t)(c * 16 + 12));
    }
}

__global__ __launch_bounds__(64) void k_card_from_hist(const uint32_t *__restrict__ hist, const uint32_t *__restrict__ keys,
                                                       uint64_t first, uint64_t n, int p, int estim, double *__restrict__ card)
{
    const uint64_t s = first + (uint64_t)blockIdx.x * 64 + threadIdx.x;
    if (s >= n) return;
    const uint32_t *h = hist + s * 64;
    struct Bins {
        const uint32_t *h;
        enum { stride = 1 };
        __device__ uint32_t operator()(int v) const { return h[v & 63]; }
        __device__ const uint32_t *at(int v) const { return h + v; }
    };
    const Bins c{h};
    const uint32_t key = keys[s];
    card[s] = estimate(c, c, p, estim, (int)(key & 63u), (int)((key >> 18) & 63u));
}

template <typename PT, int RK>
// ... 1031 lines not shown
            atomicAdd(&a.phase_cyc[12], (unsigned long long)mx_bins);
            atomicAdd(&a.phase_cyc[13], (unsigned long long)(mx_it * mx_bins));
        }
    }
}

template <typename CT, int RK, bool TIMED, bool GENERAL>
__global__ __launch_bounds__(128) __attribute__((amdgpu_waves_per_eu(8, 8), amdgpu_num_sgpr(96))) void k_finalize(FinalizeArgs a)
{
    finalize_block<CT, RK, TIMED, GENERAL>(a);
}

template <typename CT, int RK>
__global__ __launch_bounds__(128) __attribute__((amdgpu_waves_per_eu(8, 8), amdgpu_num_sgpr(96))) void k_finalize_signal(FinalizeArgs a)
{
    finalize_block<CT, RK, false, false>(a);
    if (a.sig == nullptr) return;
    const uint32_t tidx = finalize_row_of_block().tidx;
    if (tidx >= a.ntiles) return;
    asm volatile("s_waitcnt vmcnt(0)" ::: "memory");
    __builtin_amdgcn_fence(__ATOMIC_RELEASE, "workgroup");
    __syncthreads();
    if (threadIdx.x == 0) {
        uint32_t *sig = a.sig;
        if (atomicAdd(sig + kSigTileCnt + tidx, 1u) == kTile - 1) {
            atomicExch(sig + kSigTileCnt + tidx, 0u);
            const uint32_t q = a.tiles[tidx].w >> 16;
            if (atomicAdd(sig + kSigPartCnt + q, 1u) + 1u == sig[kSigPartTotal + q]) {
                if (sig[kSigStamp]) reinterpret_cast<unsigned long long *>(sig + kSigPartTime)[q] = wall_clock64();
                __hip_atomic_store(sig + kSigPartFlag + q, sig[kSigGen], __ATOMIC_RELEASE, __HIP_MEMORY_SCOPE_SYSTEM);
            }
        }
    }
}

__global__ void k_wall_stamp(unsigned long long *out) { *out = wall_clock64(); }

hipError_t launch_wall_stamp(hipStream_t st, unsigned long long *out)
{
    hipLaunchKernelGGL(k_wall_stamp, dim3(1), dim3(1), 0, st, out);
    return hipGetLastError();
}

hipError_t preload_compare_kernels()
{
    hipFuncAttributes fa;
    return hipFuncGetAttributes(&fa, reinterpret_cast<const void *>(k_wall_stamp));
}

__global__ __launch_bounds__(256) void k_upload(uint32_t *__restrict__ dst, const uint32_t *__restrict__ src, uint64_t nwords)
{
    const uint64_t stride = (uint64_t)gridDim.x * 256;
    for (uint64_t w = (uint64_t)blockIdx.x * 256 + threadIdx.x; w < nwords; w += stride) dst[w] = src[w];
}

__global__ __launch_bounds__(256) void k_upload_segs(UploadSegs u)
{
    const UploadSeg g = u.s[blockIdx.y];
    const uint64_t stride = (uint64_t)gridDim.x * 256;
    for (uint64_t w = (uint64_t)blockIdx.x * 256 + threadIdx.x; w < g.nwords; w += stride) g.dst[w] = g.src[w];
}

hipError_t launch_upload_segs(hipStream_t st, const UploadSegs &u, uint32_t nseg)
{
    uint64_t most = 0;
    for (uint32_t i = 0; i < nseg; ++i) most = std::max(most, u.s[i].nwords);
    if (!nseg || !most) return hipSuccess;
    const uint32_t blocks = (uint32_t)std::min<uint64_t>(256, (most + 255) / 256);
    hipLaunchKernelGGL(k_upload_segs, dim3(blocks, nseg), dim3(256), 0, st, u);
    return hipGetLastError();
}

hipError_t launch_upload(hipStream_t st, void *dst, const void *src_pinned, size_t bytes)
{
    if (bytes == 0) return hipSuccess;
    const uint64_t nwords = (bytes + 3) / 4;
    const uint32_t blocks = (uint32_t)std::min<uint64_t>(256, (nwords + 255) / 256);
    hipLaunchKernelGGL(k_upload, dim3(blocks), dim3(256), 0, st, (uint32_t *)dst, (const uint32_t *)src_pinned, nwords);
    return hipGetLastError();
}

hipError_t launch_selfhist_card(hipStream_t st, const uint8_t *regs, uint64_t first, uint64_t n, int p, int estim,
                                int emax, int elow, uint32_t *hist, void *exc, uint8_t *excv, uint32_t *exc_n,
                                uint32_t *keys, uint8_t *tailhist, uint32_t *gcnt)
{
    if (n <= first) return hipSuccess;
    const uint32_t blocks = (uint32_t)((n - first + 3) / 4);
    if (p <= 15)
        hipLaunchKernelGGL(k_selfhist_card<uint16_t>, dim3(blocks), dim3(256), 0, st, regs, first, n, p, estim, emax, elow,
                           hist, (uint16_t *)exc, excv, exc_n, keys, tailhist, gcnt);
    else
        hipLaunchKernelGGL(k_selfhist_card<uint32_t>, dim3(blocks), dim3(256), 0, st, regs, first, n, p, estim, emax, elow,
                           hist, (uint32_t *)exc, excv, exc_n, keys, tailhist, gcnt);
    return hipGetLastError();
}

hipError_t launch_card_from_hist(hipStream_t st, const uint32_t *hist, const uint32_t *keys, uint64_t first, uint64_t n, int p,
                                 int estim, double *card)
{
    if (n <= first) return hipSuccess;
    hipLaunchKernelGGL(k_card_from_hist, dim3((uint32_t)((n - first + 63) / 64)), dim3(64), 0, st, hist, keys, first, n, p, estim, card);
    return hipGetLastError();
}

hipError_t launch_build_colindex(hipStream_t st, const ColIndexLaunch &c)
{
    if (c.nblocks == 0) return hipSuccess;
    uint32_t G = 1;
    while (G < 4 && c.nblocks * G < 256 && c.nbuckets / (2 * G) >= 4096) G *= 2;
    const size_t lds = (size_t)(c.nbuckets / G) * sizeof(uint32_t);
#define DSH_COLINDEX(PT, RK)                                                                                                  \
    do {                                                                                                                      \
        hipError_t e = ensure_dynamic_lds(reinterpret_cast<const void *>(k_build_colindex<PT, RK>), lds);                     \
        if (e != hipSuccess) return e;                                                                                        \
        hipLaunchKernelGGL((k_build_colindex<PT, RK>), dim3(c.nblocks, G), dim3(1024), lds, st, (const PT *)c.exc, c.excv,    \
                           c.exc_n, c.keys, c.card, c.tailhist, c.perm, c.ncols, c.p, c.nbuckets, c.ent_stride, c.E, c.rec,    \
                           c.ent, c.nS, c.keyS, c.cardS, c.thS, c.rl);                                                         \
    } while (0)
    if (c.p > 15) DSH_COLINDEX(uint32_t, 3);
    else if (colindex_inline(c.p, c.E) == 3) DSH_COLINDEX(uint16_t, 3);
    else DSH_COLINDEX(uint16_t, 7);
#undef DSH_COLINDEX
    return hipGetLastError();
}

hipError_t launch_transform(hipStream_t st, const uint8_t *regs, uint64_t n, int p, int vlo,
                            uint32_t P, uint32_t W, uint32_t Npad, uint32_t *planes,
                            const uint32_t *perm)
{
    if (P == 0) return hipSuccess;
    if (p >= 8 && ((uint64_t)1 << p) / 256 <= 65535) {
        hipLaunchKernelGGL(k_transform_t, dim3(Npad / 64, (uint32_t)(((uint64_t)1 << p) / 256)), dim3(256), 0, st, regs,
                           n, p, vlo, P, W, Npad, planes, perm);
        return hipGetLastError();
    }
    const uint64_t threads = (uint64_t)Npad * W;
    const uint32_t blocks = (uint32_t)((threads + 255) / 256);
    hipLaunchKernelGGL(k_transform, dim3(blocks), dim3(256), 0, st, regs, n, p, vlo, P, W, Npad,
                       planes, perm);
    return hipGetLastError();
}

template <int KC, int U, typename CT>
static hipError_t launch_pc(hipStream_t st, const uint32_t *planes, uint32_t Npad, uint32_t Kpad,
                            uint32_t W, uint32_t P, const uint4 *tiles, const uint4 *items,
                            uint32_t nitems, void *cum, uint64_t nslots)
{
    const size_t lds = (size_t)KC * 2048;
    hipError_t e = ensure_dynamic_lds(reinterpret_cast<const void *>(k_pair_counts<KC, U, CT>), lds);
    if (e != hipSuccess) return e;
    hipLaunchKernelGGL((k_pair_counts<KC, U, CT>), dim3(nitems), dim3(256), lds, st, planes, Npad,
                       Kpad, W, P, tiles, items, reinterpret_cast<CT *>(cum), nslots);
    return hipGetLastError();
}

template <int KC, typename CT>
static hipError_t launch_pc_u(hipStream_t st, const uint32_t *planes, uint32_t Npad,
                              uint32_t Kpad, uint32_t W, uint32_t P, const uint4 *tiles,
                              const uint4 *items, uint32_t nitems, void *cum, uint64_t nslots)
{
    if (W >= 8) return launch_pc<KC, 8, CT>(st, planes, Npad, Kpad, W, P, tiles, items, nitems, cum, nslots);
    if (W == 4) return launch_pc<KC, 4, CT>(st, planes, Npad, Kpad, W, P, tiles, items, nitems, cum, nslots);
    if (W == 2) return launch_pc<KC, 2, CT>(st, planes, Npad, Kpad, W, P, tiles, items, nitems, cum, nslots);
    return launch_pc<KC, 1, CT>(st, planes, Npad, Kpad, W, P, tiles, items, nitems, cum, nslots);
}

hipError_t launch_pair_counts(hipStream_t st, int kc, int cum_bytes, const uint32_t *planes,
                              uint32_t Npad, uint32_t Kpad, uint32_t W, uint32_t P,
                              const uint4 *tiles, const uint4 *items, uint32_t nitems, void *cum,
                              uint64_t nslots)
{
    if (nitems == 0 || Kpad == 0) return hipSuccess;
    if (cum_bytes == 2) {
        switch (kc) {
        case 16: return launch_pc_u<16, uint16_t>(st, planes, Npad, Kpad, W, P, tiles, items, nitems, cum, nslots);
        case 32: return launch_pc_u<32, uint16_t>(st, planes, Npad, Kpad, W, P, tiles, items, nitems, cum, nslots);
// ... 84 lines not shown
```

### dashing_amd/csrc/kernels_sparseplane.hip

```cpp
#include <hip/hip_runtime.h>
#include <stdint.h>

#include "kernels.h"

namespace dsh {

namespace {

constexpr int kSpChunk = 16;
constexpr int kSpCounters = 11;

__global__ __launch_bounds__(256) void k_sparse_build(const uint32_t *__restrict__ planes, uint32_t Npad, uint32_t W, uint64_t ncols,
                                                      const uint2 *__restrict__ slabs, uint32_t nslabs, uint32_t cap, int wordmajor,
                                                      uint32_t *__restrict__ tab, uint16_t *__restrict__ lists, uint32_t *__restrict__ len)
{
    const uint32_t lane = threadIdx.x & 63u;
    const uint32_t nch = W / kSpChunk;
    const uint64_t unit = (uint64_t)blockIdx.x * 4 + (threadIdx.x >> 6);
    if (unit >= (uint64_t)nslabs * 2 * nch) return;
    const uint32_t ch = (uint32_t)(unit % nch), h = (uint32_t)(unit / nch) & 1u, s = (uint32_t)(unit / (2 * (uint64_t)nch));
    const uint2 sl = slabs[s];
    const uint32_t row = h * 64 + lane;
    const uint64_t col = (uint64_t)sl.x * kTile + row;
    const uint32_t w0 = ch * kSpChunk;
    const uint32_t *src = planes + ((uint64_t)sl.y * W + w0) * Npad + col;
    const uint32_t real = col < ncols ? 0xFFFFFFFFu : 0u;
    uint32_t x[kSpChunk];
#pragma unroll
    for (int k = 0; k < kSpChunk; ++k) x[k] = ~src[(uint64_t)k * Npad] & real;
    const uint64_t m = (uint64_t)W * 32;
    uint32_t *trow = tab + ((uint64_t)s * m + (uint64_t)w0 * 32 + lane) * 4 + 2 * h;
    uint32_t *tcol = tab + ((uint64_t)s * 4 + 2 * h) * m + (uint64_t)w0 * 32 + (lane & 31u);
#pragma unroll
    for (int k = 0; k < kSpChunk; ++k) {
        const uint32_t xx = x[k];
        uint32_t lo = 0, hi = 0;
#pragma unroll
        for (uint32_t b = 0; b < 32; ++b) {
            const unsigned long long bal = __ballot((xx >> b) & 1u);
            if (lane == b) {
                lo = (uint32_t)bal;
                hi = (uint32_t)(bal >> 32);
            }
        }
        if (wordmajor) {
            const uint32_t hi2 = __shfl(hi, (int)(lane & 31u), 64);
            tcol[(lane >> 5) * m + (uint64_t)k * 32] = lane < 32 ? lo : hi2;
        } else if (lane < 32) {
            *reinterpret_cast<uint2 *>(trow + (uint64_t)k * 32 * 4) = make_uint2(lo, hi);
        }
    }
    uint32_t mine = 0;
#pragma unroll
    for (int k = 0; k < kSpChunk; ++k) mine += (uint32_t)__popc(x[k]);
    if (!mine) return;
    uint32_t slot = atomicAdd(&len[(uint64_t)s * kTile + row], mine);
    uint16_t *dst = lists + ((uint64_t)s * kTile + row) * cap;
#pragma unroll
    for (int k = 0; k < kSpChunk; ++k) {
        uint32_t xx = x[k];
        while (xx) {
            const uint32_t b = (uint32_t)__builtin_ctz(xx);
            xx &= xx - 1;
            if (slot < cap) dst[slot] = (uint16_t)((w0 + k) * 32 + b);
            ++slot;
        }
    }
}

__device__ __forceinline__ void csa(uint32_t &h, uint32_t &l, uint32_t a, uint32_t b, uint32_t c)
{
    const uint32_t u = a ^ b;
    h = (a & b) | (u & c);
    l = u ^ c;
}

__device__ __forceinline__ void put32(uint16_t *dst, const uint32_t (&v)[32])
{
#pragma unroll
    for (int q = 0; q < 4; ++q)
        reinterpret_cast<uint4 *>(dst)[q] = make_uint4(v[8 * q] | (v[8 * q + 1] << 16), v[8 * q + 2] | (v[8 * q + 3] << 16),
                                                       v[8 * q + 4] | (v[8 * q + 5] << 16), v[8 * q + 6] | (v[8 * q + 7] << 16));
}
__device__ __forceinline__ void put32(uint32_t *dst, const uint32_t (&v)[32])
{
#pragma unroll
    for (int q = 0; q < 8; ++q) reinterpret_cast<uint4 *>(dst)[q] = make_uint4(v[4 * q], v[4 * q + 1], v[4 * q + 2], v[4 * q + 3]);
}

template <typename CT>
__global__ __launch_bounds__(512) void k_sparse_count(const uint4 *__restrict__ items, const uint32_t *__restrict__ tab,
                                                      const uint16_t *__restrict__ lists, const uint32_t *__restrict__ len, uint32_t cap,
                                                      uint32_t m, CT *__restrict__ cum, uint64_t nslots)
{
    __shared__ uint32_t lenj[kTile];
    const uint4 it = items[blockIdx.x];
    const uint32_t tid = threadIdx.x, r = tid >> 2, w = tid & 3u;
    if (tid < kTile) lenj[tid] = len[(uint64_t)it.w * kTile + tid];
    __syncthreads();
    const uint32_t li_all = len[(uint64_t)it.z * kTile + r];
    const uint32_t li = li_all < cap ? li_all : cap;
    const uint16_t *lp = lists + ((uint64_t)it.z * kTile + r) * cap;
    const uint32_t *tb = tab + (uint64_t)it.w * m * 4 + w;
    uint32_t c[kSpCounters];
#pragma unroll
    for (int b = 0; b < kSpCounters; ++b) c[b] = 0;
    for (uint32_t k0 = 0; k0 < li; k0 += 8) {
        const uint4 pk = *reinterpret_cast<const uint4 *>(lp + k0);
        const uint32_t pw[4] = {pk.x, pk.y, pk.z, pk.w};
        uint32_t x[8];
#pragma unroll
        for (int q = 0; q < 8; ++q) {
            const bool valid = k0 + q < li;
            const uint32_t pos = valid ? (pw[q >> 1] >> (16 * (q & 1))) & 0xFFFFu : 0u;
            const uint32_t v = tb[(uint64_t)pos * 4];
            x[q] = valid ? v : 0u;
        }
        uint32_t t0, t1, t2, t3, f0, f1, e;
        csa(t0, c[0], c[0], x[0], x[1]);
        csa(t1, c[0], c[0], x[2], x[3]);
        csa(f0, c[1], c[1], t0, t1);
        csa(t2, c[0], c[0], x[4], x[5]);
        csa(t3, c[0], c[0], x[6], x[7]);
        csa(f1, c[1], c[1], t2, t3);
        csa(e, c[2], c[2], f0, f1);
#pragma unroll
        for (int b = 3; b < kSpCounters; ++b) {
            const uint32_t carry = c[b] & e;
            c[b] ^= e;
            e = carry;
        }
    }
    const uint32_t base = m - li_all;
    uint32_t out[32];
#pragma unroll
    for (int cc = 0; cc < 32; ++cc) {
        uint32_t cnt = 0;
#pragma unroll
        for (int b = 0; b < kSpCounters; ++b) cnt |= ((c[b] >> cc) & 1u) << b;
        out[cc] = (base - lenj[w * 32 + cc] + cnt) & (sizeof(CT) == 2 ? 0xFFFFu : 0xFFFFFFFFu);
    }
    put32(cum + (uint64_t)it.y * nslots + (uint64_t)it.x * (kTile * kTile) + (uint64_t)r * kTile + w * 32, out);
}

template <typename CT>
__global__ __launch_bounds__(512) void k_sparse_count_lds(const uint4 *__restrict__ items, uint32_t nitems, const uint32_t *__restrict__ tabw,
                                                          const uint16_t *__restrict__ lists, const uint32_t *__restrict__ len, uint32_t cap,
                                                          uint32_t m, CT *__restrict__ cum, uint64_t nslots)
{
    extern __shared__ __attribute__((aligned(16))) uint32_t sp_lds[];
    const uint32_t g = blockIdx.x, item = (g >> 5) * 8 + (g & 7u), w = (g >> 3) & 3u;
    if (item >= nitems) return;
    const uint4 it = items[item];
    const uint32_t tid = threadIdx.x, r = tid >> 2, q = tid & 3u;
    const uint4 *src = reinterpret_cast<const uint4 *>(tabw + ((uint64_t)it.w * 4 + w) * m);
    for (uint32_t i = tid; i < m / 4; i += 512) reinterpret_cast<uint4 *>(sp_lds)[i] = src[i];
    if (tid < 32) sp_lds[m + tid] = len[(uint64_t)it.w * kTile + w * 32 + tid];
    __syncthreads();
    const uint32_t li_all = len[(uint64_t)it.z * kTile + r];
    const uint32_t li = li_all < cap ? li_all : cap;
    const uint16_t *lp = lists + ((uint64_t)it.z * kTile + r) * cap;
    uint32_t c[kSpCounters];
#pragma unroll
    for (int b = 0; b < kSpCounters; ++b) c[b] = 0;
    for (uint32_t k0 = 8 * q; k0 < li; k0 += 32) {
        const uint4 pk = *reinterpret_cast<const uint4 *>(lp + k0);
        const uint32_t pw[4] = {pk.x, pk.y, pk.z, pk.w};
        uint32_t x[8];
#pragma unroll
        for (int j = 0; j < 8; ++j) {
            const bool valid = k0 + j < li;
            const uint32_t pos = valid ? (pw[j >> 1] >> (16 * (j & 1))) & 0xFFFFu : 0u;
            const uint32_t v = sp_lds[pos];
            x[j] = valid ? v : 0u;
        }
        uint32_t t0, t1, t2, t3, f0, f1, e;
        csa(t0, c[0], c[0], x[0], x[1]);
        csa(t1, c[0], c[0], x[2], x[3]);
        csa(f0, c[1], c[1], t0, t1);
        csa(t2, c[0], c[0], x[4], x[5]);
        csa(t3, c[0], c[0], x[6], x[7]);
        csa(f1, c[1], c[1], t2, t3);
        csa(e, c[2], c[2], f0, f1);
#pragma unroll
        for (int b = 3; b < kSpCounters; ++b) {
            const uint32_t carry = c[b] & e;
            c[b] ^= e;
            e = carry;
        }
    }
#pragma unroll
    for (int d = 1; d <= 2; d <<= 1) {
        uint32_t carry = 0;
#pragma unroll
        for (int b = 0; b < kSpCounters; ++b) {
            const uint32_t o = __shfl_xor(c[b], d, 64);
            const uint32_t u = c[b] ^ o;
            const uint32_t sum = u ^ carry;
            carry = (c[b] & o) | (u & carry);
            c[b] = sum;
        }
    }
    if (q != 0) return;
    const uint32_t base = m - li_all;
    uint32_t out[32];
#pragma unroll
    for (int cc = 0; cc < 32; ++cc) {
        uint32_t cnt = 0;
#pragma unroll
        for (int b = 0; b < kSpCounters; ++b) cnt |= ((c[b] >> cc) & 1u) << b;
        out[cc] = (base - sp_lds[m + cc] + cnt) & (sizeof(CT) == 2 ? 0xFFFFu : 0xFFFFFFFFu);
    }
    put32(cum + (uint64_t)it.y * nslots + (uint64_t)it.x * (kTile * kTile) + (uint64_t)r * kTile + w * 32, out);
}

}

hipError_t launch_sparse_build(hipStream_t st, const uint32_t *planes, uint32_t Npad, uint32_t W, uint64_t ncols, const uint2 *slabs,
                               uint32_t nslabs, uint32_t cap, int wordmajor, uint32_t *tab, uint16_t *lists, uint32_t *len)
{
    if (nslabs == 0) return hipSuccess;
    if (W < kSpChunk || W % kSpChunk || cap % 8) return hipErrorInvalidValue;
    hipError_t e = hipMemsetAsync(len, 0, (size_t)nslabs * kTile * sizeof(uint32_t), st);
    if (e != hipSuccess) return e;
    const uint64_t units = (uint64_t)nslabs * 2 * (W / kSpChunk);
    hipLaunchKernelGGL(k_sparse_build, dim3((uint32_t)((units + 3) / 4)), dim3(256), 0, st, planes, Npad, W, ncols, slabs, nslabs, cap,
                       wordmajor, tab, lists, len);
    return hipGetLastError();
}

hipError_t launch_sparse_count(hipStream_t st, int cum_bytes, const uint4 *items, uint32_t nitems, int wordmajor, const uint32_t *tab,
                               const uint16_t *lists, const uint32_t *len, uint32_t cap, uint32_t m, void *cum, uint64_t nslots)
{
    if (nitems == 0) return hipSuccess;
    if (cap % 8 || cap > 2047) return hipErrorInvalidValue;
    if (wordmajor) {
        if (m < 512 || m > (1u << 15)) return hipErrorInvalidValue;
        const size_t lds = (size_t)m * 4 + 32 * 4;
        const uint32_t grid = (nitems + 7) / 8 * 32;
#define DSH_SPL(CT)                                                                                                                   \
    do {                                                                                                                              \
        const hipError_t e = ensure_dynamic_lds(reinterpret_cast<const void *>(k_sparse_count_lds<CT>), lds);                          \
        if (e != hipSuccess) return e;                                                                                                \
        hipLaunchKernelGGL(k_sparse_count_lds<CT>, dim3(grid), dim3(512), lds, st, items, nitems, tab, lists, len, cap, m, (CT *)cum, nslots); \
    } while (0)
        if (cum_bytes == 2) DSH_SPL(uint16_t);
        else DSH_SPL(uint32_t);
#undef DSH_SPL
        return hipGetLastError();
    }
    if (cum_bytes == 2)
        hipLaunchKernelGGL(k_sparse_count<uint16_t>, dim3(nitems), dim3(512), 0, st, items, tab, lists, len, cap, m, (uint16_t *)cum, nslots);
    else
        hipLaunchKernelGGL(k_sparse_count<uint32_t>, dim3(nitems), dim3(512), 0, st, items, tab, lists, len, cap, m, (uint32_t *)cum, nslots);
    return hipGetLastError();
}

hipError_t preload_sparseplane_kernels()
{
    hipFuncAttributes fa;
    return hipFuncGetAttributes(&fa, reinterpret_cast<const void *>(k_sparse_build));
}

}
```

### dashing_amd/csrc/plan.cpp

```cpp
#include "plan.h"

#include <algorithm>
#include <cstring>

namespace dsh {
namespace plan {

uint64_t tri_index(uint64_t n, uint64_t i, uint64_t j) { return i * (2 * n - i - 1) / 2 + j - (i + 1); }

uint64_t tri_span(uint64_t n, uint64_t rb, uint64_t re)
{
    if (re > n) re = n;
    if (rb >= re) return 0;
    const uint64_t cnt = re - rb;
    return cnt * (n - 1) - (rb + re - 1) * cnt / 2;
}

uint64_t tri_band_end(uint64_t n, uint64_t b0, uint64_t re, uint64_t band_floats, uint64_t row_cap)
{
    const uint64_t max_rows = std::min<uint64_t>(std::max<uint64_t>(row_cap, 1), kBandMaxRows);
    uint64_t b1 = b0, span = 0;
    do {
        span += n - 1 - b1;
        ++b1;
// ... 331 lines not shown
            }
            for (; u < NT; ++u) {
                uint32_t to = 0;
                for (uint32_t r = 1; r < world; ++r)
                    if (cost[r] < cost[to]) to = r;
                cost[to] += (double)(NT - u);
                deal[u - t_pool] = to;
            }
            double mx = 0;
            for (uint32_t r = 0; r < world; ++r) mx = std::max(mx, cost[r]);
            size_t segs = 0;
            for (size_t d = 0; d < deal.size(); ++d) segs += d == 0 || deal[d] != deal[d - 1];
            if (sweep == 0) {
                if (best_max < 0 || mx < best_max) best_max = mx;
            } else if (mx <= accept && (best_t == NT + 1 || segs < best_segs)) {
                best_t = t_pool;
                best_segs = segs;
                best_deal = deal;
                best_start = start;
                best_stop = stop;
            }
        }
    }
    if (best_t >= NT && bonus == 0.0) return;
    if (best_t > NT) return;
    rs.seg.clear();
    rs.owner.clear();
    rs.seg.push_back(0);
    auto push = [&](uint64_t end_row, uint32_t who) {
        if (end_row <= rs.seg.back()) return;
        if (!rs.owner.empty() && rs.owner.back() == who) rs.seg.back() = end_row;
        else rs.seg.push_back(end_row), rs.owner.push_back(who);
    };
    for (uint32_t r = 0; r < world; ++r) push(std::min<uint64_t>(n, best_stop[r] * kTile), r);
    for (uint64_t u = best_t; u < NT; ++u) push(std::min<uint64_t>(n, (u + 1) * kTile), best_deal[u - best_t]);
    if (rs.owner.empty()) rs.owner.push_back(0), rs.seg.push_back(n);
    rs.seg.back() = n;
}

void sort_rows_by_key(const uint32_t *k32, uint64_t lo, uint64_t hi, uint32_t *dst, std::vector<uint32_t> &a)
{
    auto skey = [&](uint64_t i) -> uint32_t {
        const uint32_t key = k32[i];
        return ((uint32_t)key_T(key) << 12) | ((uint32_t)key_L(key) << 6) | (uint32_t)key_hi(key);
    };
    const uint64_t cnt_ = hi - lo;
    if (a.size() < 2 * cnt_) a.resize(2 * cnt_);
    uint32_t *const ks = a.data() + cnt_;
    uint32_t c0[513], c1[513];
    std::memset(c0, 0, sizeof c0);
    std::memset(c1, 0, sizeof c1);
    for (uint64_t i = 0; i < cnt_; ++i) {
        const uint32_t k = skey(lo + i);
        ks[i] = k;
        c0[(k & 511u) + 1u]++;
        c1[(k >> 9) + 1u]++;
    }
    for (int k = 1; k < 513; ++k) c0[k] += c0[k - 1], c1[k] += c1[k - 1];
    for (uint64_t i = 0; i < cnt_; ++i) a[c0[ks[i] & 511u]++] = (uint32_t)i;
    for (uint64_t i = 0; i < cnt_; ++i) dst[c1[ks[a[i]] >> 9]++] = (uint32_t)(lo + a[i]);
}

void rowsorted_offsets(uint64_t n, const uint32_t *order, uint64_t cnt, std::vector<uint64_t> &rowoff)
{
    rowoff.resize(cnt + 1);
    uint64_t acc = 0;
    for (uint64_t s = 0; s < cnt; ++s) {
        rowoff[s] = acc;
        acc += n - 1 - order[s];
    }
    rowoff[cnt] = acc;
}

void tile_planes(const Layout &L, uint32_t ti, uint32_t tj, int &pb, int &pe)
{
    const int lo_t = std::max<int>(std::max<int>(L.blk_lo[ti], L.blk_lo[tj]), std::min<int>(L.blk_L[ti], L.blk_L[tj]));
    const int T_t = std::max<int>(L.blk_T[ti], L.blk_T[tj]);
    pb = std::max(0, lo_t - L.pbase);
    pe = std::max(pb, T_t - L.pbase);
}

void build_layout(const uint32_t *k32, uint64_t n, int want_sorted, uint64_t rb, uint64_t re,
                  const std::vector<uint64_t> &parts, Layout &L, uint32_t rowsorted_nparts, const std::vector<uint64_t> *extra_in,
                  const uint32_t *gcnt)
{
    if (re > n) re = n;
    if (!want_sorted) rb = 0, re = n;
    if (rb > re) rb = re;
    static const std::vector<uint64_t> kNoExtra;
    const std::vector<uint64_t> &extra = (want_sorted && extra_in && rb < re) ? *extra_in : kNoExtra;
    const uint64_t col0 = want_sorted ? rb : 0;
    const uint64_t ncols = n - col0;
    int vr[3] = {63, 0, 0};
    for (uint64_t i = col0; i < n; ++i) {
        const uint32_t key = k32[i];
        vr[0] = std::min<int>(vr[0], key_lo(key));
        vr[1] = std::max<int>(vr[1], key_hi(key));
        vr[2] = std::max<int>(vr[2], key_T(key));
    }
    if (ncols == 0) vr[0] = vr[1] = vr[2] = 0;
    L.sorted = want_sorted;
    L.rb = rb;
    L.re = re;
    L.rowsorted = want_sorted && rowsorted_nparts > 0;
    L.extra = extra;
    if (L.rowsorted) {
        const uint64_t x = rowsorted_split(n, rb, re);
        if (x > rb && x < re) L.parts = {rb, x, re};
        else L.parts = {rb, re};
    } else if (!extra.empty()) {
        L.parts = {rb, re};
    } else {
        L.parts = want_sorted ? parts : std::vector<uint64_t>();
    }
    L.n = n;
    L.vlo = vr[0];
    L.vhi = vr[1];
    L.ncols = ncols;
    L.Npad = (uint32_t)((ncols + kTile - 1) / kTile * kTile);
    L.whole = want_sorted && rb == 0 && re == n;
    L.perm.resize(ncols);
    L.part_pos.clear();
    L.part_w.clear();
    L.rowoff.clear();
    L.rowoff_w.clear();
    L.wtr.clear();
    L.wtr_w.clear();
    L.nwanted = want_sorted ? rowset_rows(rb, re, extra) : n;
    if (want_sorted) {
        for (size_t q = 0; q + 1 < L.parts.size(); ++q)
            sort_rows_by_key(k32, L.parts[q], L.parts[q + 1], L.perm.data() + (L.parts[q] - rb), L.sort_a);
        uint64_t at = re;
        for (size_t x = 0; x + 1 < extra.size(); x += 2) {
            if (extra[x] > at) sort_rows_by_key(k32, at, extra[x], L.perm.data() + (at - rb), L.sort_a);
            sort_rows_by_key(k32, extra[x], extra[x + 1], L.perm.data() + (extra[x] - rb), L.sort_a);
            at = extra[x + 1];
        }
        if (at < n) sort_rows_by_key(k32, at, n, L.perm.data() + (at - rb), L.sort_a);
        std::vector<std::pair<uint64_t, uint64_t>> wsegs;
        wanted_order(n, rb, re, &extra, wsegs, L.rowsorted);
        uint64_t wrows = 0;
        for (auto &sg : wsegs) {
            L.wtr.emplace_back((uint32_t)((sg.first - rb) / kTile), (uint32_t)((sg.second - rb + kTile - 1) / kTile));
            L.wtr_w.push_back(wrows);
            wrows += sg.second - sg.first;
        }
        const uint64_t wend = extra.empty() ? re - rb : extra.back() - rb;
        if (L.rowsorted) {
            rowsorted_part_positions(n, rb, re, rowsorted_nparts, L.part_w, &extra);
            L.rowoff_w.resize(L.nwanted + 1);
            L.rowoff.assign(wend + 1, 0);
            uint64_t acc = 0, w = 0;
            for (auto &sg : wsegs)
                for (uint64_t s = sg.first - rb; s < sg.second - rb; ++s, ++w) {
                    L.rowoff_w[w] = L.rowoff[s] = acc;
                    acc += n - 1 - L.perm[s];
                }
            L.rowoff_w[L.nwanted] = acc;
        } else if (!extra.empty()) {
            L.part_w = {0, L.nwanted};
        } else {
            for (uint64_t r : L.parts) L.part_w.push_back(r - rb);
        }
        if (extra.empty()) L.part_pos = L.part_w;
        else L.part_pos = {0, wend};
        if (L.whole) {
            L.perm.resize(2 * n);
            for (uint64_t s = 0; s < n; ++s) L.perm[n + L.perm[s]] = (uint32_t)s;
        }
    } else {
        for (uint64_t i = 0; i < n; ++i) L.perm[i] = (uint32_t)i;
    }
    const uint32_t NT = L.Npad / kTile;
    L.blk_T.assign(NT, 0);
    L.blk_lo.assign(NT, 255);
    L.blk_L.assign(NT, 255);
    L.blk_hi.assign(NT, 0);
    L.blk_g0.assign(gcnt ? NT : 0, 0);
    L.blk_g1.assign(gcnt ? NT : 0, 0);
    int pbase = vr[2];
    const uint32_t *perm = L.perm.data();
    for (uint32_t b = 0; b < NT; ++b) {
        const uint64_t s0 = (uint64_t)b * kTile, s1 = std::min<uint64_t>(ncols, s0 + kTile);
        int bt = 0, blo = 255, bl = 255, bhi = 0;
        for (uint64_t s = s0; s < s1; ++s) {
            const uint32_t key = k32[perm[s]];
            bt = std::max(bt, key_T(key));
            blo = std::min(blo, key_lo(key));
            bl = std::min(bl, key_L(key));
            bhi = std::max(bhi, key_hi(key));
        }
        L.blk_T[b] = (uint8_t)bt;
        L.blk_lo[b] = (uint8_t)blo;
        L.blk_L[b] = (uint8_t)bl;
        L.blk_hi[b] = (uint8_t)bhi;
        pbase = std::min(pbase, bl);
        if (gcnt) {
            uint32_t g0 = 0, g1 = 0;
            for (uint64_t s = s0; s < s1; ++s) {
                const uint32_t g = gcnt[perm[s]];
                g0 = std::max(g0, g & 0xFFFFu);
                g1 = std::max(g1, key_T(k32[perm[s]]) == bt ? g >> 16 : g & 0xFFFFu);
            }
            L.blk_g0[b] = (uint16_t)g0;
            L.blk_g1[b] = (uint16_t)g1;
        }
    }
    L.pbase = pbase;
    L.P = (uint32_t)(vr[2] - pbase);
}

static void xcd_order(std::vector<U4> &t, std::vector<uint32_t> &rank, size_t b, size_t e, size_t group)
{
    const size_t cnt = e - b;
    if (cnt < 16) return;
    std::vector<U4> tmp(cnt);
    std::vector<uint32_t> rtmp(cnt);
    const size_t nx = 8, per = (cnt + nx - 1) / nx;
    size_t q = 0;
    for (size_t r = 0; r < per; r += group)
        for (size_t x = 0; x < nx; ++x)
            for (size_t u = 0; u < group && r + u < per; ++u) {
                const size_t src = x * per + r + u;
                if (src < cnt) {
                    rtmp[q] = rank[b + src];
                    tmp[q++] = t[b + src];
                }
            }
    std::copy(tmp.begin(), tmp.begin() + q, t.begin() + b);
    std::copy(rtmp.begin(), rtmp.begin() + q, rank.begin() + b);
}

uint32_t sparse_bound(const Layout &L, uint32_t b, int v)
{
    if (b >= L.blk_g0.size()) return 65535u;
    const int Tb = L.blk_T[b];
    return v >= Tb ? L.blk_g0[b] : v == Tb - 1 ? L.blk_g1[b] : 65535u;
}

static uint32_t sparse_route(const Layout &L, uint32_t cap, int nplanes, const U4 &t)
{
    uint32_t k = 0;
    for (; (int)k < nplanes && t.w - k > t.z; ++k) {
        const int v = L.pbase + (int)(t.w - k);
        if (std::max(sparse_bound(L, t.x, v), sparse_bound(L, t.y, v)) > cap) break;
    }
    return k;
}

static void tile_vrange(const Layout &L, const U4 &t, int &lo, int &hi)
{
    lo = std::min<int>(L.blk_lo[t.x], L.blk_lo[t.y]);
    hi = std::max<int>(L.blk_hi[t.x], L.blk_hi[t.y]);
    if (hi < lo) hi = lo;
}

bool build_tiles(const Layout &L, const PairQuery &job, const Tuning &tu, PairPlan &pp)
{
    std::vector<U4> &T = pp.T;
    T.clear();
    pp.bands.clear();
    pp.band_items.clear();
    pp.segs.clear();
    pp.items.clear();
    pp.band_frags.clear();
    pp.band_round.clear();
    pp.sp.clear();
    pp.sp_items.clear();
    pp.band_sp_items.clear();
    pp.slabs.clear();
    pp.nparts = 0;
    pp.max_band = 0;
    const uint32_t NT = L.Npad / kTile;
    const uint8_t *bLo = L.blk_lo.data(), *bL = L.blk_L.data(), *bT = L.blk_T.data();
    const int pbase = L.pbase;
    auto tile_row = [&](uint32_t ti, uint32_t c0, uint32_t c1) {
        const size_t at = T.size();
        T.resize(at + (c1 - c0));
        U4 *out = T.data() + at;
        const int lo_i = bLo[ti], L_i = bL[ti], T_i = bT[ti];
        for (uint32_t tj = c0; tj < c1; ++tj) {
            const int lo_t = std::max(std::max<int>(lo_i, bLo[tj]), std::min<int>(L_i, bL[tj]));
            const int pb = std::max(0, lo_t - pbase), pe = std::max(pb, std::max<int>(T_i, bT[tj]) - pbase);
            *out++ = U4{ti, tj, (uint32_t)pb, (uint32_t)pe};
        }
    };
    std::vector<size_t> trow_first;
    std::vector<uint64_t> trow_w;
    if (job.rect) {
        if (job.row_begin >= job.row_end || job.col_begin >= job.col_end) return false;
        const uint32_t r0 = (uint32_t)(job.row_begin / kTile), r1 = (uint32_t)((job.row_end + kTile - 1) / kTile);
        const uint32_t c0 = (uint32_t)(job.col_begin / kTile), c1 = (uint32_t)((job.col_end + kTile - 1) / kTile);
        T.reserve((size_t)(r1 - r0) * (c1 - c0));
        for (uint32_t ti = r0; ti < r1; ++ti) tile_row(ti, c0, c1);
    } else {
        if (job.row_begin >= job.row_end) return false;
        if (!L.sorted || job.sorted_rows) {
            const uint32_t r0 = (uint32_t)(job.row_begin / kTile);
            const uint32_t r1 = std::min<uint32_t>(NT, (uint32_t)((job.row_end + kTile - 1) / kTile));
            if (r1 > r0) T.reserve((size_t)(r1 - r0) * (NT - r0) - (size_t)(r1 - r0) * (r1 - r0 - 1) / 2);
            for (uint32_t ti = r0; ti < r1; ++ti) tile_row(ti, ti, NT);
        } else {
            size_t cnt = 0;
            for (const auto &w : L.wtr)
                for (uint32_t ti = w.first; ti < std::min(w.second, NT); ++ti) cnt += NT - ti;
            T.reserve(cnt);
            for (size_t k = 0; k < L.wtr.size(); ++k)
                for (uint32_t ti = L.wtr[k].first; ti < std::min(L.wtr[k].second, NT); ++ti) {
                    trow_first.push_back(T.size());
                    trow_w.push_back(L.wtr_w[k] + (uint64_t)(ti - L.wtr[k].first) * kTile);
                    tile_row(ti, ti, NT);
                }
        }
    }
    if (T.empty()) return false;
    const uint32_t sp_cap = std::min(tu.sparse_cap, kSparseCapMax);
    const bool sp_can = tu.sparse_planes != 0 && !job.rect && !job.sorted_rows && L.sorted && !L.blk_g0.empty() && tu.lockstep &&
                        tu.nsplit == 0 && tu.W >= (uint32_t)tu.kc && tu.p >= 9 && tu.p <= 16 && (tu.sparse_planes > 0 || tu.p >= 13);
    const int sp_planes = !sp_can ? 0 : tu.sparse_planes < 0 ? kSparseAutoPlanes : std::min(tu.sparse_planes, 2);
    const uint64_t sp_min_planes = tu.sparse_planes < 0 ? std::max<uint64_t>(tu.small_round_items, 512) : 0;
    uint64_t job_planes = 0;
    for (const U4 &t : T) job_planes += t.w - t.z;
    const int sp_planes_job = job_planes > sp_min_planes ? sp_planes : 0;
    pp.per_tile_bytes = (uint64_t)kTile * kTile * tu.cum_bytes * std::max<uint32_t>(L.P, 1);
    const uint64_t max_tiles = std::min<uint64_t>(65536, std::max<uint64_t>(1, tu.cum_budget / pp.per_tile_bytes));
    const size_t kPartBandTiles = tu.part_band_tiles;
    const bool parts_on = job.want_parts && !job.rect && !job.sorted_rows && L.sorted && L.part_w.size() >= 2;
    std::vector<size_t> pstart{0};
    if (parts_on) {
        size_t q = 0;
        for (size_t r = 0; r < trow_first.size(); ++r)
            while (q + 2 < L.part_w.size() && trow_w[r] >= L.part_w[q + 1]) {
                ++q;
                pstart.push_back(trow_first[r]);
            }
        pp.nparts = (uint32_t)pstart.size();
    }
    pstart.push_back(T.size());
    pp.part_first = pstart;
    pp.part_tiles.clear();
    if (parts_on)
        for (size_t q = 0; q + 1 < pstart.size(); ++q) pp.part_tiles.push_back((uint32_t)(pstart[q + 1] - pstart[q]));
    auto part_of_tile = [&](size_t t) -> size_t {
        return (size_t)(std::upper_bound(pstart.begin(), pstart.end() - 1, t) - pstart.begin()) - 1;
    };
    std::vector<size_t> cuts;
    if (parts_on && pp.nparts >= 2 && tu.tail_bands > 0 && tu.lockstep && tu.W >= (uint32_t)tu.kc && tu.nsplit == 0 && tu.round_items > 0) {
        const uint64_t RI = tu.round_items;
        auto dense_planes = [&](const U4 &t) -> uint64_t { return t.w - t.z - (sp_planes_job ? sparse_route(L, sp_cap, sp_planes_job, t) : 0u); };
        uint64_t items = 0;
        for (const U4 &t : T) items += dense_planes(t);
        const uint64_t R = (items + RI - 1) / RI;
        constexpr uint64_t kBandRounds = 16;
        for (uint32_t ntails = tu.tail_bands; ntails >= 1 && cuts.empty() && items <= 4 * kBandRounds * RI && R >= 3; --ntails) {
            std::vector<uint64_t> tails;
            uint64_t left = R;
            for (uint32_t b = 0; b < ntails; ++b) {
                const uint64_t pm = b == 0 ? tu.tail_permille : tu.tail_permille2;
                const uint64_t r = std::max<uint64_t>(1, (left * pm + 500) / 1000);
                if (left < r + 2 || (b > 0 && left < r + tu.tail_head_min_rounds)) break;
                tails.push_back(r);
                left -= r;
            }
            std::vector<uint64_t> quota;
            {
                const uint64_t nb = (left + kBandRounds - 1) / kBandRounds;
                for (uint64_t b = 0; b < nb; ++b) quota.push_back(left / nb + (b < left % nb ? 1 : 0));
            }
            for (size_t b = tails.size(); b-- > 0;) {
                const uint64_t nb = (tails[b] + kBandRounds - 1) / kBandRounds;
                for (uint64_t x = 0; x < nb; ++x) quota.push_back(tails[b] / nb + (x < tails[b] % nb ? 1 : 0));
            }
            uint64_t acc = 0, rounds = 0, band_items = 0;
            size_t t = 0;
            for (size_t b = 0; b + 1 < quota.size(); ++b) {
                while (t < T.size() && band_items + dense_planes(T[t]) <= quota[b] * RI) {
                    acc += dense_planes(T[t]);
                    band_items += dense_planes(T[t]);
                    ++t;
                }
                if (t == 0 || t >= T.size() || (!cuts.empty() && cuts.back() == t)) continue;
                cuts.push_back(t);
                rounds += (band_items + RI - 1) / RI;
                band_items = 0;
            }
            rounds += (items - acc + band_items + RI - 1) / RI;
            if (rounds != R && !(R > kBandRounds && rounds == R + 1)) cuts.clear();
        }
    }
    size_t next_cut = 0;
    for (size_t b = 0; b < T.size();) {
        size_t e = std::min<size_t>(T.size(), b + max_tiles);
        if (parts_on) {
            const size_t q = part_of_tile(b);
            if (pstart[q + 1] - pstart[q] >= kPartBandTiles) e = std::min(e, pstart[q + 1]);
        }
        while (next_cut < cuts.size() && cuts[next_cut] <= b) ++next_cut;
        if (next_cut < cuts.size()) e = std::min(e, cuts[next_cut]);
        pp.bands.emplace_back(b, e);
        b = e;
    }
    pp.segs.resize(pp.bands.size());
    for (size_t bi = 0; bi < pp.bands.size(); ++bi) {
        size_t b = pp.bands[bi].first;
        while (b < pp.bands[bi].second) {
            const size_t q = part_of_tile(b);
            const size_t e = std::min(pp.bands[bi].second, pstart[q + 1]);
            const bool last_of_part = e == pstart[q + 1];
            Seg sg{b, e, parts_on && last_of_part ? (int)q : -1, 1};
            for (size_t t = b; t < e; ++t) {
                int lo, hi;
                tile_vrange(L, T[t], lo, hi);
                sg.hist_bins = std::max(sg.hist_bins, hi - lo + 1);
            }
            pp.segs[bi].push_back(sg);
            b = e;
        }
    }
    std::vector<uint32_t> &rank = pp.rank;
    rank.resize(T.size());
    for (auto &sv : pp.segs)
        for (auto &sg : sv)
            for (size_t t = sg.b; t < sg.e; ++t) rank[t] = (uint32_t)(t - sg.b);
    for (auto &sv : pp.segs)
        for (auto &sg : sv) xcd_order(T, rank, sg.b, sg.e, tu.lockstep ? 2 : 1);
    pp.sp.assign(T.size(), 0);
    pp.band_sp_items.assign(pp.bands.size(), std::make_pair((size_t)0, (size_t)0));
    if (sp_planes) {
        pp.slab_of.assign((size_t)NT * std::max<uint32_t>(L.P, 1), -1);
        auto slab = [&](uint32_t b, uint32_t pl) -> uint32_t {
            int32_t &s = pp.slab_of[(size_t)b * L.P + pl];
            if (s < 0) {
                s = (int32_t)pp.slabs.size();
                pp.slabs.push_back(U2{b, pl});
            }
            return (uint32_t)s;
        };
        for (size_t bi = 0; bi < pp.bands.size(); ++bi) {
            const auto &bd = pp.bands[bi];
            const size_t i0 = pp.sp_items.size();
            uint64_t band_planes = 0;
            for (size_t t = bd.first; t < bd.second; ++t) band_planes += T[t].w - T[t].z;
            if (band_planes > sp_min_planes)
                for (size_t t = bd.first; t < bd.second; ++t) {
                    const uint32_t k = sparse_route(L, sp_cap, sp_planes, T[t]);
                    if (!k || pp.slabs.size() + 2 * k > tu.sparse_max_slabs) continue;
                    pp.sp[t] = (uint8_t)k;
                    for (uint32_t x = 0; x < k; ++x) {
                        const uint32_t pl = T[t].w - 1 - x;
                        pp.sp_items.push_back(U4{(uint32_t)(t - bd.first), pl, slab(T[t].x, pl), slab(T[t].y, pl)});
                    }
                }
            const size_t cnt = pp.sp_items.size() - i0;
            if (cnt > 1) {
                constexpr size_t nx = 8;
                std::vector<uint32_t> per_col(NT, 0), cols;
                for (size_t k = i0; k < pp.sp_items.size(); ++k) per_col[T[bd.first + pp.sp_items[k].x].y]++;
                for (uint32_t b = 0; b < NT; ++b)
                    if (per_col[b]) cols.push_back(b);
                std::stable_sort(cols.begin(), cols.end(), [&](uint32_t a, uint32_t b) { return per_col[a] > per_col[b]; });
                std::vector<uint32_t> xcd_of(NT, 0);
                size_t load[nx] = {0};
                for (uint32_t b : cols) {
                    size_t x = 0;
                    for (size_t y = 1; y < nx; ++y)
                        if (load[y] < load[x]) x = y;
                    xcd_of[b] = (uint32_t)x;
                    load[x] += per_col[b];
                }
                std::vector<U4> lists[nx];
                for (size_t k = i0; k < pp.sp_items.size(); ++k) lists[xcd_of[T[bd.first + pp.sp_items[k].x].y]].push_back(pp.sp_items[k]);
                for (auto &l : lists)
                    std::stable_sort(l.begin(), l.end(), [&](const U4 &a, const U4 &b) {
                        const U4 &ta = T[bd.first + a.x], &tb = T[bd.first + b.x];
                        return ta.y != tb.y ? ta.y < tb.y : a.y != b.y ? a.y > b.y : ta.x < tb.x;
                    });
                size_t q = i0;
                for (size_t r = 0; q < pp.sp_items.size(); ++r)
                    for (size_t x = 0; x < nx; ++x)
                        if (r < lists[x].size()) pp.sp_items[q++] = lists[x][r];
            }
            pp.band_sp_items[bi] = std::make_pair(i0, pp.sp_items.size());
        }
    }
    const uint32_t KC = (uint32_t)tu.kc;
    const uint32_t cpp = tu.W >= KC ? tu.W / KC : 1;
    std::vector<U2> &CR = pp.chunks;
    CR.resize(T.size());
    if (tu.W >= KC) {
        for (size_t t = 0; t < T.size(); ++t) CR[t] = U2{T[t].z * cpp, (T[t].w - pp.sp[t]) * cpp};
    } else {
        for (size_t t = 0; t < T.size(); ++t)
            CR[t] = U2{(uint32_t)(((uint64_t)T[t].z * tu.W) / KC), (uint32_t)(((uint64_t)T[t].w * tu.W + KC - 1) / KC)};
    }
    for (auto &bd : pp.bands) pp.max_band = std::max(pp.max_band, bd.second - bd.first);
    return true;
}

static void overflow_fragments(const Tuning &tu, uint64_t RI, uint32_t cpp, uint64_t piece, uint64_t ni, uint64_t &over, uint32_t &f)
{
    over = 0;
    f = 1;
    if (!tu.lockstep || tu.nsplit != 0 || RI == 0 || tu.overflow_frag_max_permille == 0 || piece != cpp || cpp < 2 || ni == 0) return;
    const uint64_t o = ni % RI;
    if (o == 0 || o * 1000 > RI * tu.overflow_frag_max_permille) return;
    uint32_t ff = 1;
    while (ff * 2 <= cpp && o * (ff * 2) <= RI) ff *= 2;
    if (ff < 2) return;
    over = o;
    f = ff;
}

static uint32_t band_round_items(const Tuning &tu, uint64_t ni)
{
    if (!tu.lockstep || tu.small_round_items == 0 || tu.small_round_items >= tu.round_items) return tu.round_items;
    return ni <= 2 * (uint64_t)tu.small_round_items ? tu.small_round_items : tu.round_items;
}

void build_band_items(const Tuning &tu, PairPlan &pp, size_t bi)
{
    const auto &bd = pp.bands[bi];
    const std::vector<U2> &CR = pp.chunks;
    std::vector<U4> &I = pp.items;
    const uint32_t KC = (uint32_t)tu.kc;
    const uint32_t cpp = tu.W >= KC ? tu.W / KC : 1;
    const size_t nt = bd.second - bd.first;
    uint64_t tot = 0;
    uint32_t maxlen = 0;
    for (size_t t = bd.first; t < bd.second; ++t) {
        const uint32_t len = CR[t].y - CR[t].x;
        tot += len;
        maxlen = std::max(maxlen, len);
    }
    uint64_t piece = tu.nsplit > 0 ? std::max<uint64_t>(1, (tot / std::max<size_t>(nt, 1) + tu.nsplit - 1) / tu.nsplit)
                                   : std::max<uint64_t>(1, tot / (16 * 512));
    if (tu.nsplit == 0 && tu.lockstep)
        piece = std::min<uint64_t>(piece, std::max<uint64_t>(cpp, (uint64_t)tu.ls_item_chunks));
    piece = (piece + cpp - 1) / cpp * cpp;
    const size_t i0 = I.size();
    const uint32_t maxpieces = (uint32_t)((maxlen + piece - 1) / piece);
    const bool by_length = tu.lockstep && piece <= 65536;
    std::vector<uint32_t> &first = pp.sort_first;
    for (uint32_t s = 0; s < maxpieces; ++s) {
        const size_t g0 = I.size();
        const uint64_t off = (uint64_t)s * piece;
        size_t cnt = 0;
        uint32_t lmin = ~0u, lmax = 0;
        if (by_length) first.assign((size_t)piece + 2, 0);
        for (size_t t = bd.first; t < bd.second; ++t) {
            const uint64_t b0 = CR[t].x + off;
            if (b0 >= CR[t].y) continue;
            const uint32_t len = (uint32_t)std::min<uint64_t>(CR[t].y - b0, piece);
            ++cnt;
            lmin = std::min(lmin, len);
            lmax = std::max(lmax, len);
            if (by_length) ++first[piece - len + 1];
        }
        I.resize(g0 + cnt);
        U4 *out = I.data() + g0;
        const bool place = by_length && lmin != lmax;
        if (place)
            for (size_t v = 1; v < first.size(); ++v) first[v] += first[v - 1];
        for (size_t t = bd.first; t < bd.second; ++t) {
            const uint64_t b0 = CR[t].x + off;
            if (b0 >= CR[t].y) continue;
            const uint32_t len = (uint32_t)std::min<uint64_t>(CR[t].y - b0, piece);
            const U4 it{(uint32_t)(t - bd.first), (uint32_t)b0, (uint32_t)b0 + len, 0};
            if (place) out[first[piece - len]++] = it;
            else *out++ = it;
        }
        if (!by_length && tu.lockstep && lmin != lmax)
            std::stable_sort(I.begin() + g0, I.end(), [](const U4 &x, const U4 &y) { return x.z - x.y > y.z - y.y; });
    }
// ... 156 lines not shown
```

### dashing_amd/csrc/plan.h

```cpp
#pragma once
#include <stddef.h>
#include <stdint.h>

#include <utility>
#include <vector>

#include "consts.h"

namespace dsh {
namespace plan {

struct U4 { uint32_t x, y, z, w; };
struct U2 { uint32_t x, y; };

inline int key_lo(uint32_t k) { return (int)(k & 63u); }
inline int key_L(uint32_t k) { return (int)((k >> 6) & 63u); }
inline int key_T(uint32_t k) { return (int)((k >> 12) & 63u); }
inline int key_hi(uint32_t k) { return (int)((k >> 18) & 63u); }
inline bool key_bad(uint32_t k) { return (k & 0x80000000u) != 0; }

uint64_t tri_index(uint64_t n, uint64_t i, uint64_t j);
uint64_t tri_span(uint64_t n, uint64_t rb, uint64_t re);
void partition_rows(uint64_t n, uint32_t nparts, uint32_t align, uint64_t *bounds);
void balance_rows(uint64_t n, uint32_t nparts, uint64_t *bounds);
void range_parts(uint64_t n, uint64_t rb, uint64_t re, uint32_t nparts, std::vector<uint64_t> &out);
uint64_t tri_band_end(uint64_t n, uint64_t b0, uint64_t re, uint64_t band_floats, uint64_t row_cap);
uint64_t rect_band_rows(uint64_t ncols, uint64_t band_floats);
bool greedy_old_band(const uint32_t *labels_in, uint64_t m, uint64_t ncols, uint64_t from, uint64_t band_floats, uint64_t &b0, uint64_t &b1);
constexpr uint64_t kHistMaxIters = (1u << 18) - 1;
constexpr uint64_t kHistLdsPerCu = 160u << 10;
constexpr uint64_t kHistMaxPerCu = 8;
static_assert(4 * kHistMaxIters * kThrChunk < (1ull << 32), "a workgroup's share of a band must fit its 32-bit counters");
uint64_t hist_grid(uint64_t units, uint64_t lds_bytes, uint32_t cus);

struct RowSets {
    uint32_t world = 0;
    std::vector<uint64_t> seg;
    std::vector<uint32_t> owner;
    size_t words() const { return 3 + 2 * owner.size(); }
    void write(uint64_t *tab) const;
    void rank_rows(uint32_t r, uint64_t &rb, uint64_t &re, std::vector<uint64_t> &extra) const;
};
const char *parse_rowsets(const uint64_t *tab, uint64_t n, RowSets &rs);
void rowsets_from_bounds(const uint64_t *bounds, uint32_t world, RowSets &rs);
constexpr uint64_t kTopupMaxRows = 32768;
void balance_rowsets(uint64_t n, uint32_t world, RowSets &rs, uint32_t prep_permille = ~0u, int dst = -1, uint32_t dst_bonus_permille = ~0u);
void wanted_order(uint64_t n, uint64_t rb, uint64_t re, const std::vector<uint64_t> *extra, std::vector<std::pair<uint64_t, uint64_t>> &segs,
                  bool rowsorted = false);
uint64_t rowsorted_split(uint64_t n, uint64_t rb, uint64_t re);
uint64_t rowset_tiles(uint64_t n, uint64_t rb, uint64_t re, const std::vector<uint64_t> &extra);
uint64_t rowset_rows(uint64_t rb, uint64_t re, const std::vector<uint64_t> &extra);
uint64_t rowset_span(uint64_t n, uint64_t rb, uint64_t re, const std::vector<uint64_t> &extra);

int auto_list_cap(int p, bool upper);

bool rowsorted_rule(uint64_t n, uint64_t rb, uint64_t re, uint32_t nparts);
void rowsorted_part_positions(uint64_t n, uint64_t rb, uint64_t re, uint32_t nparts, std::vector<uint64_t> &pos,
                              const std::vector<uint64_t> *extra = nullptr);
void sort_rows_by_key(const uint32_t *keys, uint64_t lo, uint64_t hi, uint32_t *dst, std::vector<uint32_t> &scratch);
void rowsorted_offsets(uint64_t n, const uint32_t *order, uint64_t cnt, std::vector<uint64_t> &rowoff);

struct Layout {
    int sorted = 0;
    uint64_t rb = 0, re = 0;
    std::vector<uint64_t> extra;
    std::vector<std::pair<uint32_t, uint32_t>> wtr;
    std::vector<uint64_t> wtr_w;
    uint64_t nwanted = 0;
    std::vector<uint64_t> part_w;
    std::vector<uint64_t> rowoff_w;
    std::vector<uint64_t> parts;
    int rowsorted = 0;
    std::vector<uint64_t> part_pos;
    std::vector<uint64_t> rowoff;
    uint64_t n = 0, ncols = 0;
    uint32_t Npad = 0;
    bool whole = false;
    std::vector<uint32_t> perm;
    std::vector<uint8_t> blk_T, blk_lo, blk_L, blk_hi;
    std::vector<uint16_t> blk_g0, blk_g1;
    int vlo = 0, vhi = 0;
    int pbase = 0;
    uint32_t P = 0;
    std::vector<uint32_t> sort_a;
};

void build_layout(const uint32_t *keys, uint64_t n, int want_sorted, uint64_t rb, uint64_t re,
                  const std::vector<uint64_t> &parts, Layout &L, uint32_t rowsorted_nparts = 0,
                  const std::vector<uint64_t> *extra = nullptr, const uint32_t *gcnt = nullptr);

void tile_planes(const Layout &L, uint32_t ti, uint32_t tj, int &pb, int &pe);

struct PairQuery {
    int rect = 0;
    int sorted_rows = 0;
    int want_parts = 0;
    uint64_t row_begin = 0, row_end = 0, col_begin = 0, col_end = 0;
};

constexpr uint32_t kSparseCapDefault = 1280, kSparseCapMax = 2040;
constexpr int kSparseAutoPlanes = 2;

struct Tuning {
    uint32_t W = 0;
    int kc = 32;
    int cum_bytes = 2;
    uint64_t cum_budget = 8ull << 30;
    int nsplit = 0;
    bool lockstep = true;
    int ls_item_chunks = 64;
    uint32_t part_band_tiles = 2048;
    uint32_t round_items = 512;
    uint32_t small_round_items = 0;
    uint32_t overflow_frag_max_permille = 500;
    uint32_t tail_bands = 2;
    uint32_t tail_permille = 100;
    uint32_t tail_permille2 = 350;
    uint32_t tail_head_min_rounds = 7;
    int sparse_planes = 0;
    uint32_t sparse_cap = kSparseCapDefault;
    uint32_t sparse_max_slabs = 1u << 16;
    int p = 0;
};

struct Seg {
    size_t b, e;
    int part;
    int hist_bins;
};

struct PairPlan {
    std::vector<U4> T;
    std::vector<std::pair<size_t, size_t>> bands;
    std::vector<std::pair<size_t, size_t>> band_items;
    std::vector<uint32_t> band_round;
    std::vector<std::vector<Seg>> segs;
    std::vector<U4> items;
    std::vector<uint32_t> band_frags;
    std::vector<uint32_t> rank;
    std::vector<U2> chunks;
    uint64_t per_tile_bytes = 0;
    size_t max_band = 0;
    uint32_t nparts = 0;
    std::vector<uint32_t> part_tiles;
    std::vector<size_t> part_first;
    std::vector<uint32_t> sort_first;
    std::vector<U4> sort_tmp;
    std::vector<uint8_t> sp;
    std::vector<U4> sp_items;
    std::vector<std::pair<size_t, size_t>> band_sp_items;
    std::vector<U2> slabs;
    std::vector<int32_t> slab_of;
};
uint32_t sparse_bound(const Layout &L, uint32_t b, int v);

bool build_pairs(const Layout &L, const PairQuery &q, const Tuning &t, PairPlan &pp);
bool build_tiles(const Layout &L, const PairQuery &q, const Tuning &t, PairPlan &pp);
void build_band_items(const Tuning &t, PairPlan &pp, size_t band);
void emit_tile_lists(const Layout &L, const PairPlan &pp, U4 *tiles_out, U4 *ftiles_out);
void emit_band_lists(const Layout &L, const PairPlan &pp, size_t band, U4 *tiles_out, U4 *ftiles_out);
uint64_t band_item_count(const Tuning &t, const PairPlan &pp, size_t band);

}
}
```

Measured before the change: 4.308 billion pairs/s.

## Add sided sparse routing of top and bottom planes with per-sketch thresholds

Extends sparse plane routing so that tiles can send both high and low register-value planes through the sparse list/table path. The selfhist kernel now also computes per-sketch thresholds, which are copied to the host and used when building the layout. Items may be transposed so the deeper block becomes the table side, and slabs carry polarity flags plus a table-only mark. The aim is to shrink the dense popcount chunk range per tile. The cost is extra planning work, more device-to-host key traffic, and a more complex item encoding.

```diff
diff --git a/dashing_amd/csrc/abi.hip b/dashing_amd/csrc/abi.hip
--- a/dashing_amd/csrc/abi.hip
+++ b/dashing_amd/csrc/abi.hip
@@ -893,7 +893,12 @@
     }
     else if (!std::strcmp(name, "sparse_items")) *out = (int64_t)c->pp.sp_items.size();
     else if (!std::strcmp(name, "sparse_plane_us")) *out = (int64_t)(c->sparse_ms * 1000.0);
+    else if (!std::strcmp(name, "sparse_sided_items")) *out = (int64_t)c->pp.sided_items;
+    else if (!std::strcmp(name, "sparse_transposed_items")) *out = (int64_t)c->pp.transposed_items;
+    else if (!std::strcmp(name, "sparse_slabs")) *out = (int64_t)c->pp.slabs.size();
+    else if (!std::strcmp(name, "sparse_table_slabs")) *out = (int64_t)c->pp.table_slabs;
     else if (!std::strcmp(name, "sparse_planes")) *out = c->sparse_planes;
+    else if (!std::strcmp(name, "sparse_sided")) *out = c->sparse_sided;
     else if (!std::strcmp(name, "sparse_cap")) *out = c->sparse_cap;
     else if (!std::strcmp(name, "words_per_plane")) *out = c->W;
     else if (!std::strcmp(name, "avg_tile_planes_x100")) {
@@ -1037,6 +1042,11 @@
         c->sparse_planes = (int)v;
         return DSH_OK;
     }
+    if (!std::strcmp(name, "sparse_sided")) {
+        if (v < -1 || v > 1) return fail(c, DSH_EINVAL, "sparse_sided is -1 (auto), 0 (off) or 1 (forced)");
+        c->sparse_sided = (int)v;
+        return DSH_OK;
+    }
     if (!std::strcmp(name, "sparse_lds")) {
         if (v < 0 || v > 1) return fail(c, DSH_EINVAL, "sparse_lds must be 0 or 1");
         c->sparse_lds = (int)v;
diff --git a/dashing_amd/csrc/ctx.h b/dashing_amd/csrc/ctx.h
--- a/dashing_amd/csrc/ctx.h
+++ b/dashing_amd/csrc/ctx.h
@@ -171,6 +171,8 @@
     PinBuf pin_keys;
     const uint32_t *hk32 = nullptr;
     const uint32_t *hg32 = nullptr;
+    const uint32_t *hv32 = nullptr;
+    uint32_t pass_sparse_cap = 0;
     bool hk32_valid = false;
     double host_layout_us = 0, host_lists_us = 0, host_keys_wait_us = 0;
     Staging st_perm;
@@ -188,6 +190,7 @@
     int overflow_frag_permille = 500;
     int sparse_planes = -1;
     int sparse_cap = (int)dsh::plan::kSparseCapDefault;
+    int sparse_sided = -1;
     int sparse_lds = 1;
     DevBuf sp_tab, sp_lists, sp_len, sp_slabs, sp_items;
     Staging st_sparse;
diff --git a/dashing_amd/csrc/engine.hip b/dashing_amd/csrc/engine.hip
--- a/dashing_amd/csrc/engine.hip
+++ b/dashing_amd/csrc/engine.hip
@@ -55,19 +55,22 @@
         HIPCHK(c, c->exc.ensure(std::max<uint64_t>(n, 1) * kListCap * (c->p <= 15 ? 2 : 4)));
         HIPCHK(c, c->excv.ensure(std::max<uint64_t>(n, 1) * kListCap));
         HIPCHK(c, c->exc_n.ensure(std::max<uint64_t>(n, 1) * sizeof(uint32_t)));
-        HIPCHK(c, c->keys.ensure(std::max<uint64_t>(n, 1) * 2 * sizeof(uint32_t)));
+        HIPCHK(c, c->keys.ensure(std::max<uint64_t>(n, 1) * 3 * sizeof(uint32_t)));
         HIPCHK(c, c->tailhist.ensure(std::max<uint64_t>(n, 1) * 64));
         HIPCHK(c, c->hist.ensure(std::max<uint64_t>(n, 1) * 64 * sizeof(uint32_t)));
         HIPCHK(c, launch_selfhist_card(c->stream, c->regs, need_from, n, c->p, estim, c->emax, c->elow,
                                        (uint32_t *)c->hist.ptr, c->exc.ptr, (uint8_t *)c->excv.ptr,
                                        (uint32_t *)c->exc_n.ptr, (uint32_t *)c->keys.ptr,
-                                       (uint8_t *)c->tailhist.ptr, (uint32_t *)c->keys.ptr + n));
-        HIPCHK(c, c->pin_keys.ensure(std::max<uint64_t>(n, 1) * 2 * sizeof(uint32_t)));
+                                       (uint8_t *)c->tailhist.ptr, (uint32_t *)c->keys.ptr + n, (uint32_t *)c->keys.ptr + 2 * n,
+                                       std::min<uint32_t>((uint32_t)c->sparse_cap, plan::kSparseCapMax)));
+        c->pass_sparse_cap = std::min<uint32_t>((uint32_t)c->sparse_cap, plan::kSparseCapMax);
+        HIPCHK(c, c->pin_keys.ensure(std::max<uint64_t>(n, 1) * 3 * sizeof(uint32_t)));
         c->hk32 = (const uint32_t *)c->pin_keys.ptr;
         c->hg32 = c->hk32 + n;
+        c->hv32 = c->hk32 + 2 * n;
         if (n > need_from)
             HIPCHK(c, hipMemcpyAsync((uint32_t *)c->pin_keys.ptr + need_from, (const uint32_t *)c->keys.ptr + need_from,
-                                     (2 * n - need_from) * sizeof(uint32_t), hipMemcpyDeviceToHost, c->stream));
+                                     (3 * n - need_from) * sizeof(uint32_t), hipMemcpyDeviceToHost, c->stream));
         HIPCHK(c, c->ev_keys.ensure());
         HIPCHK(c, hipEventRecord(c->ev_keys, c->stream));
         HIPCHK(c, launch_card_from_hist(c->stream, (const uint32_t *)c->hist.ptr, (const uint32_t *)c->keys.ptr, need_from, n,
@@ -109,7 +112,7 @@
         plan::Layout &L = c->lay;
         if (!reuse_host_layout)
             plan::build_layout(k32, n, want_sorted, want_rb, want_re, parts, L, rowsorted ? std::max<uint32_t>(nparts, 1) : 0,
-                               extra->empty() ? nullptr : extra, c->hg32);
+                               extra->empty() ? nullptr : extra, c->hg32, c->hv32, c->pass_sparse_cap);
         ++c->lay_serial;
         c->lay_built = true;
         c->cum_bytes = c->p <= 15 ? 2 : 4;
@@ -263,6 +266,7 @@
     tu.p = c->p;
     tu.sparse_planes = c->sparse_planes;
     tu.sparse_cap = (uint32_t)c->sparse_cap;
+    tu.sparse_sided = c->sparse_sided;
     tu.sparse_max_slabs = (uint32_t)std::min<uint64_t>(1u << 16, kSparseSlabBudget / sparse_slab_bytes(c));
     return tu;
 }
diff --git a/dashing_amd/csrc/host/plan_capi.cpp b/dashing_amd/csrc/host/plan_capi.cpp
--- a/dashing_amd/csrc/host/plan_capi.cpp
+++ b/dashing_amd/csrc/host/plan_capi.cpp
@@ -20,6 +20,11 @@
     uint32_t cap = 0;
     uint32_t *routes = nullptr;
     uint64_t routes_cap = 0;
+    const uint32_t *thr = nullptr;
+    uint32_t thr_cap = 0;
+    int sided = 0;
+    uint32_t *routes6 = nullptr, *items5 = nullptr, *slabs3 = nullptr;
+    uint64_t items_cap = 0, slabs_cap = 0;
 };
 
 struct Err {
@@ -57,7 +62,7 @@
     if (!extra.empty() && !(want_sorted && mode == 0)) return E.fail("extra segments need a sorted triangle layout");
     Layout L;
     build_layout(keys, n, want_sorted, lrb, lre, parts, L, rowsorted ? std::max<uint32_t>(nparts, 1) : 0, extra.empty() ? nullptr : &extra,
-                 sc ? sc->gcnt : nullptr);
+                 sc ? sc->gcnt : nullptr, sc ? sc->thr : nullptr, sc ? sc->thr_cap : 0);
     std::vector<std::pair<uint64_t, uint64_t>> wsegs;
     wanted_order(n, lrb, lre, &extra, wsegs, rowsorted);
     auto in_rows = [&](uint64_t i) {
@@ -140,7 +145,7 @@
     if (round_items) tu.round_items = round_items;
     if (round_items > 512) tu.small_round_items = 512;
     tu.p = p;
-    if (sc) tu.sparse_planes = sc->planes, tu.sparse_cap = sc->cap;
+    if (sc) tu.sparse_planes = sc->planes, tu.sparse_cap = sc->cap, tu.sparse_sided = sc->sided;
     PairQuery q;
     q.rect = mode == 1;
     q.sorted_rows = mode == 2;
@@ -280,7 +285,8 @@
         }
     }
     if (at != T.size()) return E.fail("bands end at %zu of %zu tiles", at, T.size());
-    if (pp.sp.size() != T.size() || pp.band_sp_items.size() != pp.bands.size()) return E.fail("sparse bookkeeping sizes differ");
+    if (pp.sp.size() != T.size() || pp.spb.size() != T.size() || pp.band_sp_items.size() != pp.bands.size()) return E.fail("sparse bookkeeping sizes differ");
+    const bool sided_chk = sc && sc->thr && sc->sided != 0 && pp.sided_items > 0;
     {
         const uint32_t cpp_ = tu.W >= (uint32_t)tu.kc ? tu.W / tu.kc : 1;
         std::vector<uint8_t> seen_pl;
@@ -290,18 +296,37 @@
             const auto &rg = pp.band_sp_items[bi];
             if (rg.first != sat || rg.second < rg.first || rg.second > pp.sp_items.size()) return E.fail("sparse items of band %zu do not follow %zu", bi, sat);
             sat = rg.second;
-            seen_pl.assign((bd.second - bd.first) * 2, 0);
+            seen_pl.assign((bd.second - bd.first) * 64, 0);
             for (size_t k = rg.first; k < rg.second; ++k) {
                 const U4 &I = pp.sp_items[k];
                 if (I.x >= bd.second - bd.first) return E.fail("sparse item %zu names tile %u of band %zu", k, I.x, bi);
                 const size_t t = bd.first + I.x;
-                const uint32_t sp = pp.sp[t];
-                if (I.y >= T[t].w || I.y + sp < T[t].w) return E.fail("sparse item %zu: plane %u is not one of the top %u of tile %zu", k, I.y, sp, t);
-                if (seen_pl[I.x * 2 + (T[t].w - 1 - I.y)]++) return E.fail("plane %u of tile %zu has two sparse items", I.y, t);
-                if (I.z >= pp.slabs.size() || I.w >= pp.slabs.size() || pp.slabs[I.z].x != T[t].x || pp.slabs[I.z].y != I.y ||
-                    pp.slabs[I.w].x != T[t].y || pp.slabs[I.w].y != I.y)
+                const uint32_t sp = pp.sp[t], spb = pp.spb[t], Ipl = I.y & kSpPlaneMask;
+                if (Ipl >= T[t].w || Ipl < T[t].z || (Ipl + sp < T[t].w && Ipl >= T[t].z + spb))
+                    return E.fail("sparse item %zu: plane %u is not one of the top %u or bottom %u of tile %zu", k, Ipl, sp, spb, t);
+                if (T[t].w - T[t].z > 64) return E.fail("tile %zu has %u planes: register values are below 64", t, T[t].w - T[t].z);
+                if (seen_pl[I.x * 64 + (Ipl - T[t].z)]++) return E.fail("plane %u of tile %zu has two sparse items", Ipl, t);
+                if (I.z >= pp.slabs.size() || I.w >= pp.slabs.size() || pp.slabs[I.z].x != T[t].x || (pp.slabs[I.z].y & kSpPlaneMask) != Ipl ||
+                    pp.slabs[I.w].x != T[t].y || (pp.slabs[I.w].y & kSpPlaneMask) != Ipl)
                     return E.fail("sparse item %zu names the wrong slabs", k);
-                const int v = L.pbase + 1 + (int)I.y;
+                const int v = L.pbase + 1 + (int)Ipl;
+                if (sided_chk) {
+                    const bool tr = (I.y & kSpItemTransposed) != 0, la = (I.y & kSpItemListA) != 0, ta = (I.y & kSpItemTabA) != 0;
+                    if (tr && T[t].x == T[t].y) return E.fail("sparse item %zu: a diagonal tile is transposed", k);
+                    const U2 &lsl = pp.slabs[tr ? I.w : I.z], &tsl = pp.slabs[tr ? I.z : I.w];
+                    if (((lsl.y & kSpSlabA) != 0) != la || ((tsl.y & kSpSlabA) != 0) != ta) return E.fail("sparse item %zu: polarities differ from its slabs'", k);
+                    if (lsl.y & kSpSlabTableOnly) return E.fail("sparse item %zu reads lists from a table-only slab", k);
+                    if (L.thr_cap != tu.sparse_cap) return E.fail("sparse item %zu planned on thresholds of cap %u at cap %u", k, L.thr_cap, tu.sparse_cap);
+                    for (uint32_t a = 0; a < kTile; ++a) {
+                        const uint64_t sx = (uint64_t)lsl.x * kTile + a;
+                        if (sx >= L.ncols) continue;
+                        const uint32_t th = sc->thr[orig(sx)];
+                        if (la ? v > (int)((th >> 8) & 0xFFu) : v < (int)(th & 0xFFu))
+                            return E.fail("sparse item %zu: sketch %llu of the list block is outside its bound at v = %d", k, (unsigned long long)orig(sx), v);
+                    }
+                    continue;
+                }
+                if (I.y != Ipl || pp.slabs[I.z].y != Ipl || pp.slabs[I.w].y != Ipl) return E.fail("sparse item %zu carries flags without the sided route", k);
                 if (sparse_bound(L, T[t].x, v) > tu.sparse_cap || sparse_bound(L, T[t].y, v) > tu.sparse_cap) return E.fail("sparse item %zu: a set may exceed the cap", k);
                 if (sc && sc->gcnt)
                     for (int side = 0; side < 2; ++side)
@@ -314,11 +339,13 @@
                         }
             }
             for (size_t t = bd.first; t < bd.second; ++t) {
-                const uint32_t sp = pp.sp[t];
-                if (sp > 2 || sp > T[t].w - T[t].z) return E.fail("tile %zu routes %u planes of %u", t, sp, T[t].w - T[t].z);
-                for (uint32_t x = 0; x < sp; ++x)
-                    if (!seen_pl[(t - bd.first) * 2 + x]) return E.fail("routed plane %u of tile %zu has no sparse item", T[t].w - 1 - x, t);
-                if (tu.W >= (uint32_t)tu.kc && (pp.chunks[t].x != T[t].z * cpp_ || pp.chunks[t].y != (T[t].w - sp) * cpp_))
+                const uint32_t sp = pp.sp[t], spb = pp.spb[t], np = T[t].w - T[t].z;
+                if ((!sided_chk && (sp > 2 || spb)) || sp + spb > np) return E.fail("tile %zu routes %u + %u planes of %u", t, spb, sp, np);
+                if (np > 64) return E.fail("tile %zu has %u planes: register values are below 64", t, np);
+                for (uint32_t x = 0; x < np; ++x)
+                    if ((seen_pl[(t - bd.first) * 64 + x] != 0) != (x < spb || x + sp >= np))
+                        return E.fail("plane %u of tile %zu: routed and sparse item disagree", T[t].z + x, t);
+                if (tu.W >= (uint32_t)tu.kc && (pp.chunks[t].x != (T[t].z + spb) * cpp_ || pp.chunks[t].y != (T[t].w - sp) * cpp_))
                     return E.fail("tile %zu: the dense chunk range is not the planes left over", t);
             }
         }
@@ -328,6 +355,24 @@
             for (size_t t = 0; t < T.size(); ++t) {
                 uint32_t *o = sc->routes + 5 * t;
                 o[0] = T[t].x, o[1] = T[t].y, o[2] = T[t].z, o[3] = T[t].w, o[4] = pp.sp[t];
+            }
+        }
+        if (sc && sc->routes6) {
+            if (T.size() > sc->routes_cap || pp.sp_items.size() > sc->items_cap || pp.slabs.size() > sc->slabs_cap)
+                return E.fail("%zu tiles, %zu items, %zu slabs: no room", T.size(), pp.sp_items.size(), pp.slabs.size());
+            for (size_t t = 0; t < T.size(); ++t) {
+                uint32_t *o = sc->routes6 + 6 * t;
+                o[0] = T[t].x, o[1] = T[t].y, o[2] = T[t].z, o[3] = T[t].w, o[4] = pp.spb[t], o[5] = pp.sp[t];
+            }
+            for (size_t bi = 0; bi < pp.bands.size(); ++bi)
+                for (size_t k = pp.band_sp_items[bi].first; k < pp.band_sp_items[bi].second; ++k) {
+                    const U4 &I = pp.sp_items[k];
+                    uint32_t *o = sc->items5 + 5 * k;
+                    o[0] = (uint32_t)(pp.bands[bi].first + I.x), o[1] = I.y & kSpPlaneMask, o[2] = I.y >> 8, o[3] = I.z, o[4] = I.w;
+                }
+            for (size_t k = 0; k < pp.slabs.size(); ++k) {
+                uint32_t *o = sc->slabs3 + 3 * k;
+                o[0] = pp.slabs[k].x, o[1] = pp.slabs[k].y & kSpPlaneMask, o[2] = pp.slabs[k].y >> 8;
             }
         }
     }
@@ -382,6 +427,7 @@
     stats[3] = pp.nparts;
     stats[4] = T.empty() ? 0 : planes_sum * 100 / T.size();
     if (sc) stats[10] = pp.sp_items.size(), stats[11] = pp.slabs.size();
+    if (sc && sc->routes6) stats[12] = pp.sided_items, stats[13] = pp.transposed_items, stats[14] = pp.table_slabs;
     stats[7] = 0;
     for (size_t b = 0; b < pp.band_items.size(); ++b) {
         const uint32_t nfr = b < pp.band_frags.size() ? pp.band_frags[b] : 0u;
@@ -428,6 +474,29 @@
                       cap, round_items, &sc);
 }
 
+int dshh_plan_check_sparse_sided(uint64_t n, const uint32_t *keys, const uint32_t *gcnt, const uint32_t *thr, uint32_t thr_cap, int mode,
+                                 int want_sorted, uint64_t rb, uint64_t re, uint32_t nparts, int want_parts, int p, uint64_t cum_budget,
+                                 uint32_t round_items, int sparse_planes, int sparse_sided, uint32_t sparse_cap, uint64_t *stats, uint32_t *routes,
+                                 uint64_t routes_cap, uint32_t *items, uint64_t items_cap, uint32_t *slabs, uint64_t slabs_cap, char *err, size_t cap)
+{
+    Err E{err, cap};
+    if (round_items == 0 || round_items % 256) return E.fail("round_items %u is not a positive multiple of 256", round_items);
+    if (!routes || !items || !slabs) return E.fail("routes, items and slabs are wanted");
+    SparseCheck sc;
+    sc.gcnt = gcnt;
+    sc.planes = sparse_planes;
+    sc.cap = sparse_cap;
+    sc.thr = thr;
+    sc.thr_cap = thr_cap;
+    sc.sided = sparse_sided;
+    sc.routes6 = routes, sc.routes_cap = routes_cap;
+    sc.items5 = items, sc.items_cap = items_cap;
+    sc.slabs3 = slabs, sc.slabs_cap = slabs_cap;
+    for (int i = 10; i < 15; ++i) stats[i] = 0;
+    return plan_check(n, keys, mode, want_sorted, rb, re, 0, 0, nparts, want_parts, p, cum_budget, 1, 0, 64, std::vector<uint64_t>(), stats, err,
+                      cap, round_items, &sc);
+}
+
 int dshh_plan_check_rowset(uint64_t n, const uint32_t *keys, const uint64_t *tab, uint32_t rank, int rowsorted, uint32_t nparts, int p,
                            uint64_t cum_budget, uint64_t *stats, char *err, size_t cap)
 {
diff --git a/dashing_amd/csrc/kernels.h b/dashing_amd/csrc/kernels.h
--- a/dashing_amd/csrc/kernels.h
+++ b/dashing_amd/csrc/kernels.h
@@ -8,7 +8,7 @@
 
 hipError_t launch_selfhist_card(hipStream_t st, const uint8_t *regs, uint64_t first, uint64_t n, int p, int estim,
                                 int emax, int elow, uint32_t *hist, void *exc, uint8_t *excv, uint32_t *exc_n,
-                                uint32_t *keys, uint8_t *tailhist, uint32_t *gcnt);
+                                uint32_t *keys, uint8_t *tailhist, uint32_t *gcnt, uint32_t *sthr, uint32_t scap);
 hipError_t launch_card_from_hist(hipStream_t st, const uint32_t *hist, const uint32_t *keys, uint64_t first, uint64_t n, int p,
                                  int estim, double *card);
 inline int colindex_inline(int p, uint32_t E) { return p <= 12 && E <= 256 ? 7 : 3; }
diff --git a/dashing_amd/csrc/kernels_compare.hip b/dashing_amd/csrc/kernels_compare.hip
--- a/dashing_amd/csrc/kernels_compare.hip
+++ b/dashing_amd/csrc/kernels_compare.hip
@@ -17,7 +17,8 @@
                                                         uint32_t *__restrict__ exc_n,
                                                         uint32_t *__restrict__ keys,
                                                         uint8_t *__restrict__ tailhist,
-                                                        uint32_t *__restrict__ gcnt)
+                                                        uint32_t *__restrict__ gcnt,
+                                                        uint32_t *__restrict__ sthr, uint32_t scap)
 {
     __shared__ uint32_t hist[4][64];
     __shared__ uint32_t sub[4][8][72];
@@ -91,6 +92,13 @@
         keys[s] = ((uint32_t)hi << 18) | ((uint32_t)T << 12) | ((uint32_t)L << 6) | (uint32_t)lo;
         const uint32_t g0 = cnt + h[T], g1 = g0 + (T > 0 ? h[T - 1] : 0u);
         gcnt[s] = (g0 < 65535u ? g0 : 65535u) | ((g1 < 65535u ? g1 : 65535u) << 16);
+        int vU = 64, vA = 0;
+        if (p >= 13) {
+            uint32_t up = 0, dn = 0;
+            while (vU > 0 && up + h[vU - 1] <= scap) up += h[--vU];
+            while (vA < 64 && dn + h[vA] <= scap) dn += h[vA++];
+        }
+        sthr[s] = (uint32_t)vU | ((uint32_t)vA << 8);
     }
     if (s < n && __any(bad != 0) && lane == 0) atomicOr(&keys[s], 0x80000000u);
     __syncthreads();
@@ -1288,16 +1296,16 @@
 
 hipError_t launch_selfhist_card(hipStream_t st, const uint8_t *regs, uint64_t first, uint64_t n, int p, int estim,
                                 int emax, int elow, uint32_t *hist, void *exc, uint8_t *excv, uint32_t *exc_n,
-                                uint32_t *keys, uint8_t *tailhist, uint32_t *gcnt)
+                                uint32_t *keys, uint8_t *tailhist, uint32_t *gcnt, uint32_t *sthr, uint32_t scap)
 {
     if (n <= first) return hipSuccess;
     const uint32_t blocks = (uint32_t)((n - first + 3) / 4);
     if (p <= 15)
         hipLaunchKernelGGL(k_selfhist_card<uint16_t>, dim3(blocks), dim3(256), 0, st, regs, first, n, p, estim, emax, elow,
-                           hist, (uint16_t *)exc, excv, exc_n, keys, tailhist, gcnt);
+                           hist, (uint16_t *)exc, excv, exc_n, keys, tailhist, gcnt, sthr, scap);
     else
         hipLaunchKernelGGL(k_selfhist_card<uint32_t>, dim3(blocks), dim3(256), 0, st, regs, first, n, p, estim, emax, elow,
-                           hist, (uint32_t *)exc, excv, exc_n, keys, tailhist, gcnt);
+                           hist, (uint32_t *)exc, excv, exc_n, keys, tailhist, gcnt, sthr, scap);
     return hipGetLastError();
 }
 
diff --git a/dashing_amd/csrc/kernels_sparseplane.hip b/dashing_amd/csrc/kernels_sparseplane.hip
--- a/dashing_amd/csrc/kernels_sparseplane.hip
+++ b/dashing_amd/csrc/kernels_sparseplane.hip
@@ -1,11 +1,21 @@
 #include <hip/hip_runtime.h>
 #include <stdint.h>
 
+#include <algorithm>
+
 #include "kernels.h"
+#include "plan.h"
 
 namespace dsh {
 
 namespace {
+
+using plan::kSpItemListA;
+using plan::kSpItemTabA;
+using plan::kSpItemTransposed;
+using plan::kSpPlaneMask;
+using plan::kSpSlabA;
+using plan::kSpSlabTableOnly;
 
 constexpr int kSpChunk = 16;
 constexpr int kSpCounters = 11;
@@ -20,41 +30,37 @@
     if (unit >= (uint64_t)nslabs * 2 * nch) return;
     const uint32_t ch = (uint32_t)(unit % nch), h = (uint32_t)(unit / nch) & 1u, s = (uint32_t)(unit / (2 * (uint64_t)nch));
     const uint2 sl = slabs[s];
+    const uint32_t plane = sl.y & kSpPlaneMask;
+    const uint32_t flip = sl.y & kSpSlabA ? 0u : 0xFFFFFFFFu;
     const uint32_t row = h * 64 + lane;
     const uint64_t col = (uint64_t)sl.x * kTile + row;
     const uint32_t w0 = ch * kSpChunk;
-    const uint32_t *src = planes + ((uint64_t)sl.y * W + w0) * Npad + col;
+    const uint32_t *src = planes + ((uint64_t)plane * W + w0) * Npad + col;
     const uint32_t real = col < ncols ? 0xFFFFFFFFu : 0u;
     uint32_t x[kSpChunk];
 #pragma unroll
-    for (int k = 0; k < kSpChunk; ++k) x[k] = ~src[(uint64_t)k * Npad] & real;
+    for (int k = 0; k < kSpChunk; ++k) x[k] = (src[(uint64_t)k * Npad] ^ flip) & real;
     const uint64_t m = (uint64_t)W * 32;
-    uint32_t *trow = tab + ((uint64_t)s * m + (uint64_t)w0 * 32 + lane) * 4 + 2 * h;
-    uint32_t *tcol = tab + ((uint64_t)s * 4 + 2 * h) * m + (uint64_t)w0 * 32 + (lane & 31u);
+    const uint32_t q = 2 * h + (lane >> 5), b5 = lane & 31u;
+    uint32_t *tpos = tab + ((uint64_t)s * m + (uint64_t)w0 * 32 + b5) * 4 + q;
+    uint32_t *tcol = tab + ((uint64_t)s * 4 + q) * m + (uint64_t)w0 * 32 + b5;
 #pragma unroll
     for (int k = 0; k < kSpChunk; ++k) {
-        const uint32_t xx = x[k];
-        uint32_t lo = 0, hi = 0;
-#pragma unroll
-        for (uint32_t b = 0; b < 32; ++b) {
-            const unsigned long long bal = __ballot((xx >> b) & 1u);
-            if (lane == b) {
-                lo = (uint32_t)bal;
-                hi = (uint32_t)(bal >> 32);
-            }
-        }
-        if (wordmajor) {
-            const uint32_t hi2 = __shfl(hi, (int)(lane & 31u), 64);
-            tcol[(lane >> 5) * m + (uint64_t)k * 32] = lane < 32 ? lo : hi2;
-        } else if (lane < 32) {
-            *reinterpret_cast<uint2 *>(trow + (uint64_t)k * 32 * 4) = make_uint2(lo, hi);
-        }
+        uint32_t t = x[k];
+#pragma unroll
+        for (uint32_t j = 16, mk = 0x0000FFFFu; j; j >>= 1, mk ^= mk << j) {
+            const uint32_t o = __shfl_xor(t, (int)j, 64);
+            t = lane & j ? (t & ~mk) | ((o >> j) & mk) : (t & mk) | ((o & mk) << j);
+        }
+        if (wordmajor) tcol[(uint64_t)k * 32] = t;
+        else tpos[(uint64_t)k * 32 * 4] = t;
     }
     uint32_t mine = 0;
 #pragma unroll
     for (int k = 0; k < kSpChunk; ++k) mine += (uint32_t)__popc(x[k]);
     if (!mine) return;
     uint32_t slot = atomicAdd(&len[(uint64_t)s * kTile + row], mine);
+    if (sl.y & kSpSlabTableOnly) return;
     uint16_t *dst = lists + ((uint64_t)s * kTile + row) * cap;
 #pragma unroll
     for (int k = 0; k < kSpChunk; ++k) {
@@ -89,19 +95,56 @@
 }
 
 template <typename CT>
+__device__ __forceinline__ void sp_values(uint32_t (&out)[32], const uint32_t (&c)[kSpCounters], uint32_t fl, uint32_t m, uint32_t ll,
+                                          const uint32_t *lt)
+{
+    const bool la = (fl & kSpItemListA) != 0, ta = (fl & kSpItemTabA) != 0;
+    const uint32_t kl = !la && !ta ? m - ll : la && !ta ? ll : 0u;
+    const uint32_t tsub = !la && !ta ? 0xFFFFFFFFu : 0u, tadd = !la && ta ? 0xFFFFFFFFu : 0u;
+    const uint32_t cneg = la != ta ? 0xFFFFFFFFu : 0u;
+#pragma unroll
+    for (int cc = 0; cc < 32; ++cc) {
+        uint32_t cnt = 0;
+#pragma unroll
+        for (int b = 0; b < kSpCounters; ++b) cnt |= ((c[b] >> cc) & 1u) << b;
+        const uint32_t t = lt[cc];
+        out[cc] = (kl + (t & tadd) - (t & tsub) + ((cnt ^ cneg) - cneg)) & (sizeof(CT) == 2 ? 0xFFFFu : 0xFFFFFFFFu);
+    }
+}
+
+template <typename CT>
+__device__ __forceinline__ void sp_store_rows(const uint32_t *st, CT *dst, uint32_t tid)
+{
+    if (sizeof(CT) == 2) {
+        const uint32_t at = (tid >> 4) * kTile + (tid & 15u) * 8;
+        const uint4 a = *reinterpret_cast<const uint4 *>(st + at), b = *reinterpret_cast<const uint4 *>(st + at + 4);
+        *reinterpret_cast<uint4 *>(dst + at) = make_uint4(a.x | (a.y << 16), a.z | (a.w << 16), b.x | (b.y << 16), b.z | (b.w << 16));
+    } else {
+#pragma unroll
+        for (uint32_t h = 0; h < 2; ++h) {
+            const uint32_t g = tid + 512 * h, at = (g >> 5) * kTile + (g & 31u) * 4;
+            *reinterpret_cast<uint4 *>(dst + at) = *reinterpret_cast<const uint4 *>(st + at);
+        }
+    }
+}
+
+template <typename CT>
 __global__ __launch_bounds__(512) void k_sparse_count(const uint4 *__restrict__ items, const uint32_t *__restrict__ tab,
                                                       const uint16_t *__restrict__ lists, const uint32_t *__restrict__ len, uint32_t cap,
                                                       uint32_t m, CT *__restrict__ cum, uint64_t nslots)
 {
     __shared__ uint32_t lenj[kTile];
+    __shared__ __attribute__((aligned(16))) uint32_t turn[32 * kTile];
     const uint4 it = items[blockIdx.x];
+    const bool tr = (it.y & kSpItemTransposed) != 0;
+    const uint32_t ls = tr ? it.w : it.z, ts = tr ? it.z : it.w, plane = it.y & kSpPlaneMask;
     const uint32_t tid = threadIdx.x, r = tid >> 2, w = tid & 3u;
-    if (tid < kTile) lenj[tid] = len[(uint64_t)it.w * kTile + tid];
+    if (tid < kTile) lenj[tid] = len[(uint64_t)ts * kTile + tid];
     __syncthreads();
-    const uint32_t li_all = len[(uint64_t)it.z * kTile + r];
+    const uint32_t li_all = len[(uint64_t)ls * kTile + r];
     const uint32_t li = li_all < cap ? li_all : cap;
-    const uint16_t *lp = lists + ((uint64_t)it.z * kTile + r) * cap;
-    const uint32_t *tb = tab + (uint64_t)it.w * m * 4 + w;
+    const uint16_t *lp = lists + ((uint64_t)ls * kTile + r) * cap;
+    const uint32_t *tb = tab + (uint64_t)ts * m * 4 + w;
     uint32_t c[kSpCounters];
 #pragma unroll
     for (int b = 0; b < kSpCounters; ++b) c[b] = 0;
@@ -131,16 +174,22 @@
             e = carry;
         }
     }
-    const uint32_t base = m - li_all;
     uint32_t out[32];
-#pragma unroll
-    for (int cc = 0; cc < 32; ++cc) {
-        uint32_t cnt = 0;
-#pragma unroll
-        for (int b = 0; b < kSpCounters; ++b) cnt |= ((c[b] >> cc) & 1u) << b;
-        out[cc] = (base - lenj[w * 32 + cc] + cnt) & (sizeof(CT) == 2 ? 0xFFFFu : 0xFFFFFFFFu);
-    }
-    put32(cum + (uint64_t)it.y * nslots + (uint64_t)it.x * (kTile * kTile) + (uint64_t)r * kTile + w * 32, out);
+    sp_values<CT>(out, c, it.y, m, li_all, lenj + w * 32);
+    CT *blk = cum + (uint64_t)plane * nslots + (uint64_t)it.x * (kTile * kTile);
+    if (!tr) {
+        put32(blk + (uint64_t)r * kTile + w * 32, out);
+        return;
+    }
+    for (uint32_t k = 0; k < 4; ++k) {
+        if (w == k) {
+#pragma unroll
+            for (int cc = 0; cc < 32; ++cc) turn[cc * kTile + r] = out[cc];
+        }
+        __syncthreads();
+        sp_store_rows<CT>(turn, blk + (uint64_t)k * 32 * kTile, tid);
+        __syncthreads();
+    }
 }
 
 template <typename CT>
@@ -152,14 +201,17 @@
     const uint32_t g = blockIdx.x, item = (g >> 5) * 8 + (g & 7u), w = (g >> 3) & 3u;
     if (item >= nitems) return;
     const uint4 it = items[item];
+    const bool tr = (it.y & kSpItemTransposed) != 0;
+    const uint32_t ls = tr ? it.w : it.z, ts = tr ? it.z : it.w, plane = it.y & kSpPlaneMask;
     const uint32_t tid = threadIdx.x, r = tid >> 2, q = tid & 3u;
-    const uint4 *src = reinterpret_cast<const uint4 *>(tabw + ((uint64_t)it.w * 4 + w) * m);
+    const uint32_t lenat = m < 32u * kTile ? 32u * kTile : m;
+    const uint4 *src = reinterpret_cast<const uint4 *>(tabw + ((uint64_t)ts * 4 + w) * m);
     for (uint32_t i = tid; i < m / 4; i += 512) reinterpret_cast<uint4 *>(sp_lds)[i] = src[i];
-    if (tid < 32) sp_lds[m + tid] = len[(uint64_t)it.w * kTile + w * 32 + tid];
+    if (tid < 32) sp_lds[lenat + tid] = len[(uint64_t)ts * kTile + w * 32 + tid];
     __syncthreads();
-    const uint32_t li_all = len[(uint64_t)it.z * kTile + r];
+    const uint32_t li_all = len[(uint64_t)ls * kTile + r];
     const uint32_t li = li_all < cap ? li_all : cap;
-    const uint16_t *lp = lists + ((uint64_t)it.z * kTile + r) * cap;
+    const uint16_t *lp = lists + ((uint64_t)ls * kTile + r) * cap;
     uint32_t c[kSpCounters];
 #pragma unroll
     for (int b = 0; b < kSpCounters; ++b) c[b] = 0;
@@ -201,17 +253,23 @@
             c[b] = sum;
         }
     }
-    if (q != 0) return;
-    const uint32_t base = m - li_all;
-    uint32_t out[32];
-#pragma unroll
-    for (int cc = 0; cc < 32; ++cc) {
-        uint32_t cnt = 0;
-#pragma unroll
-        for (int b = 0; b < kSpCounters; ++b) cnt |= ((c[b] >> cc) & 1u) << b;
-        out[cc] = (base - sp_lds[m + cc] + cnt) & (sizeof(CT) == 2 ? 0xFFFFu : 0xFFFFFFFFu);
-    }
-    put32(cum + (uint64_t)it.y * nslots + (uint64_t)it.x * (kTile * kTile) + (uint64_t)r * kTile + w * 32, out);
+    CT *blk = cum + (uint64_t)plane * nslots + (uint64_t)it.x * (kTile * kTile);
+    if (!tr) {
+        if (q != 0) return;
+        uint32_t out[32];
+        sp_values<CT>(out, c, it.y, m, li_all, sp_lds + lenat);
+        put32(blk + (uint64_t)r * kTile + w * 32, out);
+        return;
+    }
+    __syncthreads();
+    if (q == 0) {
+        uint32_t out[32];
+        sp_values<CT>(out, c, it.y, m, li_all, sp_lds + lenat);
+#pragma unroll
+        for (int cc = 0; cc < 32; ++cc) sp_lds[cc * kTile + r] = out[cc];
+    }
+    __syncthreads();
+    sp_store_rows<CT>(sp_lds, blk + (uint64_t)w * 32 * kTile, tid);
 }
 
 }
@@ -236,7 +294,7 @@
     if (cap % 8 || cap > 2047) return hipErrorInvalidValue;
     if (wordmajor) {
         if (m < 512 || m > (1u << 15)) return hipErrorInvalidValue;
-        const size_t lds = (size_t)m * 4 + 32 * 4;
+        const size_t lds = (size_t)std::max<uint32_t>(m, 32u * kTile) * 4 + 32 * 4;
         const uint32_t grid = (nitems + 7) / 8 * 32;
 #define DSH_SPL(CT)                                                                                                                   \
     do {                                                                                                                              \
diff --git a/dashing_amd/csrc/plan.cpp b/dashing_amd/csrc/plan.cpp
--- a/dashing_amd/csrc/plan.cpp
+++ b/dashing_amd/csrc/plan.cpp
@@ -437,7 +437,7 @@
 
 void build_layout(const uint32_t *k32, uint64_t n, int want_sorted, uint64_t rb, uint64_t re,
                   const std::vector<uint64_t> &parts, Layout &L, uint32_t rowsorted_nparts, const std::vector<uint64_t> *extra_in,
-                  const uint32_t *gcnt)
+                  const uint32_t *gcnt, const uint32_t *thr, uint32_t thr_cap)
 {
     if (re > n) re = n;
     if (!want_sorted) rb = 0, re = n;
@@ -533,6 +533,9 @@
     L.blk_hi.assign(NT, 0);
     L.blk_g0.assign(gcnt ? NT : 0, 0);
     L.blk_g1.assign(gcnt ? NT : 0, 0);
+    L.blk_vU.assign(thr ? NT : 0, 0);
+    L.blk_vA.assign(thr ? NT : 0, 64);
+    L.thr_cap = thr ? thr_cap : 0;
     int pbase = vr[2];
     const uint32_t *perm = L.perm.data();
     for (uint32_t b = 0; b < NT; ++b) {
@@ -559,6 +562,16 @@
             }
             L.blk_g0[b] = (uint16_t)g0;
             L.blk_g1[b] = (uint16_t)g1;
+        }
+        if (thr) {
+            uint32_t vU = 0, vA = 64;
+            for (uint64_t s = s0; s < s1; ++s) {
+                const uint32_t t = thr[perm[s]];
+                vU = std::max(vU, t & 0xFFu);
+                vA = std::min(vA, (t >> 8) & 0xFFu);
+            }
+            L.blk_vU[b] = (uint8_t)vU;
+            L.blk_vA[b] = (uint8_t)vA;
         }
     }
     L.pbase = pbase;
@@ -603,6 +616,30 @@
     return k;
 }
 
+int sided_depth(const Layout &L, uint32_t b, int v)
+{
+    if (b >= L.blk_vU.size()) return -1;
+    return std::max(v - (int)L.blk_vU[b], (int)L.blk_vA[b] - v);
+}
+
+int sided_polarity(const Layout &L, uint32_t b, int v)
+{
+    if (b >= L.blk_vU.size() || v >= (int)L.blk_vU[b]) return 0;
+    return v <= (int)L.blk_vA[b] ? 1 : 0;
+}
+
+static void sided_route(const Layout &L, const U4 &t, uint32_t &below, uint32_t &above)
+{
+    const uint32_t np = t.w - t.z;
+    auto routed = [&](uint32_t pl) {
+        const int v = L.pbase + 1 + (int)pl;
+        return sided_depth(L, t.x, v) >= 0 || sided_depth(L, t.y, v) >= 0;
+    };
+    above = below = 0;
+    while (above < np && routed(t.w - 1 - above)) ++above;
+    while (below + above < np && routed(t.z + below)) ++below;
+}
+
 static void tile_vrange(const Layout &L, const U4 &t, int &lo, int &hi)
 {
     lo = std::min<int>(L.blk_lo[t.x], L.blk_lo[t.y]);
@@ -621,6 +658,7 @@
     pp.band_frags.clear();
     pp.band_round.clear();
     pp.sp.clear();
+    pp.spb.clear();
     pp.sp_items.clear();
     pp.band_sp_items.clear();
     pp.slabs.clear();
@@ -677,6 +715,11 @@
     uint64_t job_planes = 0;
     for (const U4 &t : T) job_planes += t.w - t.z;
     const int sp_planes_job = job_planes > sp_min_planes ? sp_planes : 0;
+    const bool sd_can = !job.rect && !job.sorted_rows && L.sorted && !L.blk_vU.empty() && L.thr_cap == sp_cap && tu.lockstep && tu.nsplit == 0 &&
+                        tu.W >= (uint32_t)tu.kc && tu.p >= 13 && tu.p <= 16;
+    const bool sd_forced = sd_can && tu.sparse_sided > 0;
+    const bool sd_auto = sd_can && tu.sparse_sided < 0 && tu.sparse_planes < 0 && kSparseSidedAuto;
+    const bool sided_job = sd_forced || (sd_auto && job_planes > sp_min_planes);
     pp.per_tile_bytes = (uint64_t)kTile * kTile * tu.cum_bytes * std::max<uint32_t>(L.P, 1);
     const uint64_t max_tiles = std::min<uint64_t>(65536, std::max<uint64_t>(1, tu.cum_budget / pp.per_tile_bytes));
     const size_t kPartBandTiles = tu.part_band_tiles;
@@ -702,7 +745,14 @@
     std::vector<size_t> cuts;
     if (parts_on && pp.nparts >= 2 && tu.tail_bands > 0 && tu.lockstep && tu.W >= (uint32_t)tu.kc && tu.nsplit == 0 && tu.round_items > 0) {
         const uint64_t RI = tu.round_items;
-        auto dense_planes = [&](const U4 &t) -> uint64_t { return t.w - t.z - (sp_planes_job ? sparse_route(L, sp_cap, sp_planes_job, t) : 0u); };
+        auto dense_planes = [&](const U4 &t) -> uint64_t {
+            if (sided_job) {
+                uint32_t lo, hi;
+                sided_route(L, t, lo, hi);
+                return t.w - t.z - lo - hi;
+            }
+            return t.w - t.z - (sp_planes_job ? sparse_route(L, sp_cap, sp_planes_job, t) : 0u);
+        };
         uint64_t items = 0;
         for (const U4 &t : T) items += dense_planes(t);
         const uint64_t R = (items + RI - 1) / RI;
@@ -780,37 +830,64 @@
     for (auto &sv : pp.segs)
         for (auto &sg : sv) xcd_order(T, rank, sg.b, sg.e, tu.lockstep ? 2 : 1);
     pp.sp.assign(T.size(), 0);
+    pp.spb.assign(T.size(), 0);
+    pp.sided_items = pp.transposed_items = pp.table_slabs = 0;
     pp.band_sp_items.assign(pp.bands.size(), std::make_pair((size_t)0, (size_t)0));
-    if (sp_planes) {
+    if (sp_planes || sd_forced || sd_auto) {
         pp.slab_of.assign((size_t)NT * std::max<uint32_t>(L.P, 1), -1);
-        auto slab = [&](uint32_t b, uint32_t pl) -> uint32_t {
+        std::vector<uint8_t> listed;
+        auto slab = [&](uint32_t b, uint32_t pl, bool lists) -> uint32_t {
             int32_t &s = pp.slab_of[(size_t)b * L.P + pl];
             if (s < 0) {
                 s = (int32_t)pp.slabs.size();
-                pp.slabs.push_back(U2{b, pl});
-            }
+                pp.slabs.push_back(U2{b, pl | (sd_can && sided_polarity(L, b, L.pbase + 1 + (int)pl) ? kSpSlabA : 0u)});
+                listed.push_back(0);
+            }
+            if (lists) listed[(size_t)s] = 1;
             return (uint32_t)s;
         };
+        auto table_block = [&](const std::pair<size_t, size_t> &bd, const U4 &it) { return it.y & kSpItemTransposed ? T[bd.first + it.x].x : T[bd.first + it.x].y; };
         for (size_t bi = 0; bi < pp.bands.size(); ++bi) {
             const auto &bd = pp.bands[bi];
             const size_t i0 = pp.sp_items.size();
             uint64_t band_planes = 0;
             for (size_t t = bd.first; t < bd.second; ++t) band_planes += T[t].w - T[t].z;
-            if (band_planes > sp_min_planes)
+            if (sd_forced || (sd_auto && band_planes > sp_min_planes)) {
+                for (size_t t = bd.first; t < bd.second; ++t) {
+                    uint32_t below, above;
+                    sided_route(L, T[t], below, above);
+                    const uint32_t k = below + above;
+                    if (!k || pp.slabs.size() + 2 * k > tu.sparse_max_slabs) continue;
+                    pp.sp[t] = (uint8_t)above;
+                    pp.spb[t] = (uint8_t)below;
+                    for (uint32_t x = 0; x < k; ++x) {
+                        const uint32_t pl = x < above ? T[t].w - 1 - x : T[t].z + (x - above);
+                        const int v = L.pbase + 1 + (int)pl;
+                        const bool tr = T[t].x != T[t].y && sided_depth(L, T[t].y, v) > sided_depth(L, T[t].x, v);
+                        const uint32_t lb = tr ? T[t].y : T[t].x, tb = tr ? T[t].x : T[t].y;
+                        const uint32_t fl = (sided_polarity(L, lb, v) ? kSpItemListA : 0u) | (sided_polarity(L, tb, v) ? kSpItemTabA : 0u) |
+                                            (tr ? kSpItemTransposed : 0u);
+                        pp.sp_items.push_back(U4{(uint32_t)(t - bd.first), pl | fl, slab(T[t].x, pl, !tr), slab(T[t].y, pl, tr || T[t].x == T[t].y)});
+                        ++pp.sided_items;
+                        pp.transposed_items += tr;
+                    }
+                }
+            } else if (sp_planes && band_planes > sp_min_planes) {
                 for (size_t t = bd.first; t < bd.second; ++t) {
                     const uint32_t k = sparse_route(L, sp_cap, sp_planes, T[t]);
                     if (!k || pp.slabs.size() + 2 * k > tu.sparse_max_slabs) continue;
                     pp.sp[t] = (uint8_t)k;
                     for (uint32_t x = 0; x < k; ++x) {
                         const uint32_t pl = T[t].w - 1 - x;
-                        pp.sp_items.push_back(U4{(uint32_t)(t - bd.first), pl, slab(T[t].x, pl), slab(T[t].y, pl)});
+                        pp.sp_items.push_back(U4{(uint32_t)(t - bd.first), pl, slab(T[t].x, pl, true), slab(T[t].y, pl, true)});
                     }
                 }
+            }
             const size_t cnt = pp.sp_items.size() - i0;
             if (cnt > 1) {
                 constexpr size_t nx = 8;
                 std::vector<uint32_t> per_col(NT, 0), cols;
-                for (size_t k = i0; k < pp.sp_items.size(); ++k) per_col[T[bd.first + pp.sp_items[k].x].y]++;
+                for (size_t k = i0; k < pp.sp_items.size(); ++k) per_col[table_block(bd, pp.sp_items[k])]++;
                 for (uint32_t b = 0; b < NT; ++b)
                     if (per_col[b]) cols.push_back(b);
                 std::stable_sort(cols.begin(), cols.end(), [&](uint32_t a, uint32_t b) { return per_col[a] > per_col[b]; });
@@ -824,11 +901,12 @@
                     load[x] += per_col[b];
                 }
                 std::vector<U4> lists[nx];
-                for (size_t k = i0; k < pp.sp_items.size(); ++k) lists[xcd_of[T[bd.first + pp.sp_items[k].x].y]].push_back(pp.sp_items[k]);
+                for (size_t k = i0; k < pp.sp_items.size(); ++k) lists[xcd_of[table_block(bd, pp.sp_items[k])]].push_back(pp.sp_items[k]);
                 for (auto &l : lists)
                     std::stable_sort(l.begin(), l.end(), [&](const U4 &a, const U4 &b) {
                         const U4 &ta = T[bd.first + a.x], &tb = T[bd.first + b.x];
-                        return ta.y != tb.y ? ta.y < tb.y : a.y != b.y ? a.y > b.y : ta.x < tb.x;
+                        const uint32_t ca = table_block(bd, a), cb = table_block(bd, b), pa = a.y & kSpPlaneMask, pb = b.y & kSpPlaneMask;
+                        return ca != cb ? ca < cb : pa != pb ? pa > pb : ta.x + ta.y < tb.x + tb.y;
                     });
                 size_t q = i0;
                 for (size_t r = 0; q < pp.sp_items.size(); ++r)
@@ -837,13 +915,15 @@
             }
             pp.band_sp_items[bi] = std::make_pair(i0, pp.sp_items.size());
         }
+        for (size_t k = 0; k < pp.slabs.size(); ++k)
+            if (!listed[k]) pp.slabs[k].y |= kSpSlabTableOnly, ++pp.table_slabs;
     }
     const uint32_t KC = (uint32_t)tu.kc;
     const uint32_t cpp = tu.W >= KC ? tu.W / KC : 1;
     std::vector<U2> &CR = pp.chunks;
     CR.resize(T.size());
     if (tu.W >= KC) {
-        for (size_t t = 0; t < T.size(); ++t) CR[t] = U2{T[t].z * cpp, (T[t].w - pp.sp[t]) * cpp};
+        for (size_t t = 0; t < T.size(); ++t) CR[t] = U2{(T[t].z + pp.spb[t]) * cpp, (T[t].w - pp.sp[t]) * cpp};
     } else {
         for (size_t t = 0; t < T.size(); ++t)
             CR[t] = U2{(uint32_t)(((uint64_t)T[t].z * tu.W) / KC), (uint32_t)(((uint64_t)T[t].w * tu.W + KC - 1) / KC)};
diff --git a/dashing_amd/csrc/plan.h b/dashing_amd/csrc/plan.h
--- a/dashing_amd/csrc/plan.h
+++ b/dashing_amd/csrc/plan.h
@@ -79,6 +79,8 @@
     std::vector<uint32_t> perm;
     std::vector<uint8_t> blk_T, blk_lo, blk_L, blk_hi;
     std::vector<uint16_t> blk_g0, blk_g1;
+    std::vector<uint8_t> blk_vU, blk_vA;
+    uint32_t thr_cap = 0;
     int vlo = 0, vhi = 0;
     int pbase = 0;
     uint32_t P = 0;
@@ -87,7 +89,8 @@
 
 void build_layout(const uint32_t *keys, uint64_t n, int want_sorted, uint64_t rb, uint64_t re,
                   const std::vector<uint64_t> &parts, Layout &L, uint32_t rowsorted_nparts = 0,
-                  const std::vector<uint64_t> *extra = nullptr, const uint32_t *gcnt = nullptr);
+                  const std::vector<uint64_t> *extra = nullptr, const uint32_t *gcnt = nullptr, const uint32_t *thr = nullptr,
+                  uint32_t thr_cap = 0);
 
 void tile_planes(const Layout &L, uint32_t ti, uint32_t tj, int &pb, int &pe);
 
@@ -100,6 +103,10 @@
 
 constexpr uint32_t kSparseCapDefault = 1280, kSparseCapMax = 2040;
 constexpr int kSparseAutoPlanes = 2;
+constexpr bool kSparseSidedAuto = true;
+constexpr uint32_t kSpPlaneMask = 0xFFu;
+constexpr uint32_t kSpItemListA = 1u << 8, kSpItemTabA = 1u << 9, kSpItemTransposed = 1u << 10;
+constexpr uint32_t kSpSlabA = 1u << 8, kSpSlabTableOnly = 1u << 9;
 
 struct Tuning {
     uint32_t W = 0;
@@ -120,6 +127,7 @@
     int sparse_planes = 0;
     uint32_t sparse_cap = kSparseCapDefault;
     uint32_t sparse_max_slabs = 1u << 16;
+    int sparse_sided = 0;
     int p = 0;
 };
 
@@ -147,12 +155,16 @@
     std::vector<uint32_t> sort_first;
     std::vector<U4> sort_tmp;
     std::vector<uint8_t> sp;
+    std::vector<uint8_t> spb;
     std::vector<U4> sp_items;
+    uint64_t sided_items = 0, transposed_items = 0, table_slabs = 0;
     std::vector<std::pair<size_t, size_t>> band_sp_items;
     std::vector<U2> slabs;
     std::vector<int32_t> slab_of;
 };
 uint32_t sparse_bound(const Layout &L, uint32_t b, int v);
+int sided_depth(const Layout &L, uint32_t b, int v);
+int sided_polarity(const Layout &L, uint32_t b, int v);
 
 bool build_pairs(const Layout &L, const PairQuery &q, const Tuning &t, PairPlan &pp);
 bool build_tiles(const Layout &L, const PairQuery &q, const Tuning &t, PairPlan &pp);
```

Measured after the change: 4.425 billion pairs/s, median of 6. 2.7% higher.
